# voichek/kmersGWAS

Hardware: AMD Instinct MI355X
Metric: k-mers x permutations scored/sec (higher is better)
Workload: dtype fp4 x fp6/fp4 block-scaled filter + f32/f64 exact re-score

## Files before the change

### kmersgwas_amd/csrc/aux_kernels.hip

```cpp
#include "score_common.h"
#include "synth.h"

namespace kgwas {

static hipError_t ensure_dyn_lds(const void* fn, size_t bytes) {
    if (bytes > 64 * 1024) return hipFuncSetAttribute(fn, hipFuncAttributeMaxDynamicSharedMemorySize, (int)bytes);
    return hipSuccess;
}

__global__ void __launch_bounds__(256) squeeze_kernel(const uint64_t* file_rows, uint64_t file_stride_w,
                                                      uint64_t n_rows, const uint32_t* colmap, uint32_t W_m,
                                                      uint32_t W_f, uint32_t* out) {
    extern __shared__ uint32_t lds_u32[];
    const uint32_t in_dw = 2u * W_f, in_ld = in_dw + 1u;
    const uint32_t out_dw = 2u * W_m, out_ld = out_dw + 1u;
    uint32_t* lin = lds_u32;
    uint32_t* lout = lds_u32 + 64u * in_ld;
    const uint64_t row0 = (uint64_t)blockIdx.x * 64u;
    const uint32_t* fr = reinterpret_cast<const uint32_t*>(file_rows);

    for (uint32_t e = threadIdx.x; e < 64u * in_dw; e += 256u) {
        const uint32_t rr = e / in_dw, dw = e - rr * in_dw;
        const uint64_t gr = row0 + rr;
        lin[rr * in_ld + dw] = (gr < n_rows) ? fr[gr * file_stride_w * 2u + 2u + dw] : 0u;
// ... 171 lines not shown
    }
    for (int o = 32; o > 0; o >>= 1) kcnt += __shfl_xor(kcnt, o);
    if (lane == 0 && kcnt) atomicAdd(&kept_s, kcnt);
    if (__ballot(bad != 0u) && lane == 0) atomicOr(&nan_s, 1u);
    __syncthreads();
    const uint32_t kept = kept_s;
    if (p == 0 && t == 0) info[0] = kept;
    if (t == 0 && nan_s) atomicOr(&info[1], 1u);
    const unsigned long long N = topn[p];
    if (kept < N || nan_s) return;
    if (t == 0) {
        prefix_s = 0;
        need_s = N;
    }
#pragma unroll 1
    for (int byte = 7; byte >= 0; byte--) {
        if (t < 256u) hist[t] = 0;
        __syncthreads();
        const unsigned long long prefix = prefix_s;
#pragma unroll
        for (int i = 0; i < DSEL_KPT; i++) {
            const bool act = ((valid >> i) & 1u) && (byte == 7 || (key[i] >> (8 * (byte + 1))) == prefix);
            const unsigned long long m = __ballot(act);
            if (!m) continue;
            const uint32_t bin = (uint32_t)(key[i] >> (8 * byte)) & 255u;
            const int first = __ffsll((long long)m) - 1;
            const uint32_t b0 = (uint32_t)__shfl((int)bin, first);
            if (__ballot(act && bin == b0) == m) {
                if ((int)lane == first) atomicAdd(&hist[b0], (uint32_t)__popcll(m));
            } else if (act) {
                atomicAdd(&hist[bin], 1u);
            }
        }
        __syncthreads();
        if (t < 64u) pick_bin_from_top(hist, prefix, &need_s, &prefix_s);
        __syncthreads();
    }
    if (t == 0) {
        const unsigned long long k = prefix_s;
        const unsigned long long b = (k >> 63) ? (k & 0x7FFFFFFFFFFFFFFFull) : ~k;
        const double v = __longlong_as_double((long long)b);
        thr_a[p] = v;
        thr_b[p] = v;
        thr_host_copy[p] = v;
    }
}

hipError_t launch_dense_select(const double* dense, const uint32_t* n1, uint32_t n_rows, uint32_t n_pheno, uint32_t S, uint32_t min_count,
                               const uint64_t* topn, double* thr_a, double* thr_b, double* thr_host_copy, uint32_t* info, hipStream_t st) {
    hipError_t e = hipMemsetAsync(info, 0, 2 * sizeof(uint32_t), st);
    if (e != hipSuccess) return e;
    static const bool reg_ok = !(exp_int("KGWAS_DSEL_REG", 1) == 0);
    if (reg_ok && n_rows <= (uint32_t)DSEL_KPT * 1024u)
        hipLaunchKernelGGL(dense_select_reg_kernel, dim3(n_pheno), dim3(1024), 0, st, dense, n1, n_rows, S, min_count, topn, thr_a, thr_b,
                           thr_host_copy, info);
    else
        hipLaunchKernelGGL(dense_select_kernel, dim3(n_pheno), dim3(256), 0, st, dense, n1, n_rows, S, min_count, topn, thr_a, thr_b,
                           thr_host_copy, info);
    return hipGetLastError();
}

__global__ void __launch_bounds__(256) records_to_host_kernel(const unsigned long long* __restrict__ sc, const unsigned long long* __restrict__ km,
                                                              const uint32_t* __restrict__ rw, uint32_t n, unsigned long long* __restrict__ h_sc,
                                                              unsigned long long* __restrict__ h_km, uint32_t* __restrict__ h_rw) {
    const uint32_t step = gridDim.x * blockDim.x;
    for (uint32_t i = blockIdx.x * blockDim.x + threadIdx.x; i < n; i += step) {
        h_sc[i] = sc[i];
        h_km[i] = km[i];
        h_rw[i] = rw[i];
    }
}

__global__ void __launch_bounds__(256) chunk_tail_kernel(const uint32_t* __restrict__ meta, uint32_t n_meta, uint32_t* __restrict__ h_meta,
                                                         const unsigned long long* __restrict__ tested, uint32_t n_tested,
                                                         unsigned long long* __restrict__ h_tested, const double* __restrict__ thr, uint32_t n_thr,
                                                         double* __restrict__ h_thr) {
    for (uint32_t i = threadIdx.x; i < n_meta; i += 256u) h_meta[i] = meta[i];
    for (uint32_t i = threadIdx.x; i < n_tested; i += 256u) h_tested[i] = tested[i];
    for (uint32_t i = threadIdx.x; i < n_thr; i += 256u) h_thr[i] = thr[i];
}

hipError_t launch_chunk_tail(const uint32_t* meta, uint32_t n_meta, uint32_t* h_meta, const unsigned long long* tested, uint32_t n_tested,
                             unsigned long long* h_tested, const double* thr, uint32_t n_thr, double* h_thr, hipStream_t st) {
    launch_last(chunk_tail_kernel, dim3(1), dim3(256), 0, st, meta, n_meta, h_meta, tested, n_tested, h_tested, thr, n_thr, h_thr);
    return hipGetLastError();
}

__global__ void __launch_bounds__(256) thr_tail_kernel(const uint32_t* hist, const uint32_t* hist_base, uint32_t bins, const uint64_t* topn,
                                                       const double* thr_host, double* thr, const uint32_t* __restrict__ meta, uint32_t n_meta,
                                                       uint32_t* __restrict__ h_meta, const unsigned long long* __restrict__ tested, uint32_t n_tested,
                                                       unsigned long long* __restrict__ h_tested, double* __restrict__ h_thr) {
    thr_update_block(hist, hist_base, bins, topn, thr_host, thr, blockIdx.x);
    if (h_thr && threadIdx.x == 0) h_thr[blockIdx.x] = thr[blockIdx.x];
    if (blockIdx.x == 0) {
        for (uint32_t i = threadIdx.x; i < n_meta; i += 256u) h_meta[i] = meta[i];
        for (uint32_t i = threadIdx.x; i < n_tested; i += 256u) h_tested[i] = tested[i];
    }
}

hipError_t launch_thr_tail(const uint32_t* hist, const uint32_t* hist_base, uint32_t bins, const uint64_t* topn, const double* thr_host, double* thr,
                           uint32_t n_pheno, const uint32_t* meta, uint32_t n_meta, uint32_t* h_meta, const unsigned long long* tested,
                           uint32_t n_tested, unsigned long long* h_tested, double* h_thr, hipStream_t st) {
    if (n_pheno == 0 || bins % 256u) return hipErrorInvalidValue;
    launch_last(thr_tail_kernel, dim3(n_pheno), dim3(256), 0, st, hist, hist_base, bins, topn, thr_host, thr, meta, n_meta, h_meta, tested,
                n_tested, h_tested, h_thr);
    return hipGetLastError();
}

hipError_t launch_records_to_host(const double* sc, const uint64_t* km, const uint32_t* rw, uint32_t n, double* h_sc, uint64_t* h_km, uint32_t* h_rw,
                                  hipStream_t st) {
    if (!n) return hipSuccess;
    static const uint32_t max_blocks = (uint64_t)exp_int("KGWAS_RECORD_BLOCKS", 64u);
    const uint32_t blocks = std::min<uint32_t>((n + 255u) / 256u, std::max(1u, max_blocks));
    hipLaunchKernelGGL(records_to_host_kernel, dim3(blocks), dim3(256), 0, st, reinterpret_cast<const unsigned long long*>(sc),
                       reinterpret_cast<const unsigned long long*>(km), rw, n, reinterpret_cast<unsigned long long*>(h_sc),
                       reinterpret_cast<unsigned long long*>(h_km), h_rw);
    return hipGetLastError();
}

hipError_t launch_thr_update(const uint32_t* hist, const uint32_t* hist_base, uint32_t bins, const uint64_t* topn,
                             const double* thr_host, double* thr, uint32_t n_pheno, hipStream_t st) {
    if (n_pheno == 0 || bins % 256u) return hipErrorInvalidValue;
    hipLaunchKernelGGL(thr_update_kernel, dim3(n_pheno), dim3(256), 0, st, hist, hist_base, bins, topn, thr_host, thr);
    return hipGetLastError();
}

hipError_t launch_squeeze(const uint64_t* file_rows, uint64_t file_stride_w, uint64_t n_rows, const uint32_t* colmap,
                          uint32_t W_m, uint32_t W_f, uint32_t* out, hipStream_t st) {
    if (n_rows == 0) return hipSuccess;
    const size_t lds = (size_t)64u * ((2u * W_f + 1u) + (2u * W_m + 1u)) * 4u;
    if (lds > 160u * 1024u) return hipErrorInvalidValue;
    hipError_t e = ensure_dyn_lds((const void*)squeeze_kernel, lds);
    if (e != hipSuccess) return e;
    hipLaunchKernelGGL(squeeze_kernel, dim3((uint32_t)((n_rows + 63) / 64)), dim3(256), lds, st, file_rows,
                       file_stride_w, n_rows, colmap, W_m, W_f, out);
    return hipGetLastError();
}

hipError_t launch_synth(uint64_t* rows, uint64_t first_row, uint64_t n_rows, uint64_t n_acc, uint64_t seed,
                        hipStream_t st) {
    if (n_rows == 0) return hipSuccess;
    const uint64_t total = n_rows * (1 + (n_acc + 63) / 64);
    uint64_t blocks = (total + 255) / 256;
    if (blocks > 256ull * 32ull) blocks = 256ull * 32ull;
    hipLaunchKernelGGL(synth_kernel, dim3((uint32_t)blocks), dim3(256), 0, st, rows, first_row, n_rows, n_acc, seed);
    return hipGetLastError();
}

__global__ void __launch_bounds__(256) copy_to_host_kernel(const uint4* __restrict__ src, uint4* __restrict__ dst, size_t n16, uint32_t tail_words) {
    const size_t step = (size_t)gridDim.x * blockDim.x;
    for (size_t i = (size_t)blockIdx.x * blockDim.x + threadIdx.x; i < n16; i += step) dst[i] = src[i];
    if (blockIdx.x == 0 && threadIdx.x < tail_words)
        reinterpret_cast<uint32_t*>(dst + n16)[threadIdx.x] = reinterpret_cast<const uint32_t*>(src + n16)[threadIdx.x];
}

hipError_t launch_copy_to_host(const void* src, void* dst_dev, size_t bytes, hipStream_t st) {
    if (!bytes) return hipSuccess;
    if (bytes % 4 || ((uintptr_t)src | (uintptr_t)dst_dev) % 16) return hipErrorInvalidValue;
    const size_t n16 = bytes / 16;
    const uint32_t blocks = (uint32_t)std::min<size_t>(std::max<size_t>((n16 + 255) / 256, 1), 256);
    hipLaunchKernelGGL(copy_to_host_kernel, dim3(blocks), dim3(256), 0, st, reinterpret_cast<const uint4*>(src), reinterpret_cast<uint4*>(dst_dev), n16,
                       (uint32_t)((bytes % 16) / 4));
    return hipGetLastError();
}

}
```

### kmersgwas_amd/csrc/kernels.h

```cpp
#pragma once
#include <hip/hip_runtime.h>
#include <stdint.h>

#include "env.h"
#include "launch.h"

namespace kgwas {

struct Cand {
    uint64_t kmer;
    double score;
    uint64_t row;
};

struct RowSrc {
    const uint32_t* base;
    uint64_t stride_dw;
    uint32_t off_dw;
    uint32_t avail_dw;
};

constexpr uint32_t TESTED_SHARDS = 256;

struct ScoreArgs {
    RowSrc src;
    const uint32_t* dmask;
    const uint64_t* file_rows;
    uint64_t file_stride_w;
    uint64_t n_rows;
    uint64_t first_row;
    uint32_t S;
    uint32_t W_m;
    uint32_t n_pheno;
    uint32_t min_count;
    const float* Yperm;
    const float* Ymfma;
    const float* sums;
    const double* thr;
    double* dense;
    uint32_t* n1_out;
    uint64_t* kmer_out;
    Cand* cand;
    uint32_t* cand_cnt;
    uint32_t cap;
    unsigned long long* tested;
    uint32_t* hist;
    const uint32_t* hist_base;
    uint32_t hist_bins;
    double* so_score;
    uint64_t* so_kmer;
    uint32_t* so_row;
};

constexpr int HIST_SHIFT = 44;
constexpr uint32_t HIST_BINS = 16384;

hipError_t launch_copy_to_host(const void* src, void* dst_dev, size_t bytes, hipStream_t st);
hipError_t launch_chunk_tail(const uint32_t* meta, uint32_t n_meta, uint32_t* h_meta, const unsigned long long* tested, uint32_t n_tested,
                             unsigned long long* h_tested, const double* thr, uint32_t n_thr, double* h_thr, hipStream_t st);
hipError_t launch_thr_tail(const uint32_t* hist, const uint32_t* hist_base, uint32_t bins, const uint64_t* topn, const double* thr_host, double* thr,
                           uint32_t n_pheno, const uint32_t* meta, uint32_t n_meta, uint32_t* h_meta, const unsigned long long* tested,
                           uint32_t n_tested, unsigned long long* h_tested, double* h_thr, hipStream_t st);
hipError_t launch_records_to_host(const double* sc, const uint64_t* km, const uint32_t* rw, uint32_t n, double* h_sc, uint64_t* h_km, uint32_t* h_rw,
                                  hipStream_t st);
hipError_t launch_thr_update(const uint32_t* hist, const uint32_t* hist_base, uint32_t bins, const uint64_t* topn,
                             const double* thr_host, double* thr, uint32_t n_pheno, hipStream_t st);

hipError_t launch_dense_select(const double* dense, const uint32_t* n1, uint32_t n_rows, uint32_t n_pheno, uint32_t S, uint32_t min_count,
                               const uint64_t* topn, double* thr_a, double* thr_b, double* thr_host_copy, uint32_t* info, hipStream_t st);

hipError_t launch_score_valu(const ScoreArgs& a, hipStream_t st);
hipError_t launch_score_mfma(const ScoreArgs& a, uint32_t rows_per_block, uint32_t nb_full, hipStream_t st);
size_t mfma_lds_bytes(uint32_t W_m);

struct CoarseCol {
    double kalpha;
    float iu;
    int32_t pheno;
};
struct CoarseArgs {
    RowSrc src;
    uint64_t n_rows;
    uint32_t S, n_pheno, min_count;
    uint32_t n_kgroups;
    uint32_t n_lgroups;
    uint32_t n_slices;
    const int8_t* Bq;
    const CoarseCol* cols;
    const double* thr;
    unsigned long long* bitmap;
    uint64_t words_per_col;
    unsigned long long* tested;
    float eg_max, rall_max, rmax_max;
};
size_t coarse_lds_bytes(uint32_t n_kgroups, uint32_t T);
hipError_t launch_coarse(const CoarseArgs& a, uint32_t T, uint32_t rows_per_block, hipStream_t st);
struct MxArgs {
    RowSrc src;
    uint64_t n_rows;
    uint32_t S, n_pheno, min_count;
    uint32_t n_full, n_quarter;
    uint32_t n_lgroups;
    uint32_t n_slices;
    uint32_t s1_fp6;
    uint32_t scale0;
    const uint8_t* Bq;
    const CoarseCol* cols;
    const double* thr;
    unsigned long long* bitmap;
    uint64_t words_per_col;
    unsigned long long* tested;
    float eg_max, rall_max, rmax_max;
};
size_t mx_lds_bytes(uint32_t n_steps, uint32_t CT, uint32_t n_slices, uint32_t s1_fp6);
uint32_t mx_step_bytes_rt(uint32_t n_slices, uint32_t s1_fp6);
uint32_t mx_row_tiles(uint32_t CT);
hipError_t launch_mx(const MxArgs& a, uint32_t CT, uint32_t rows_per_block, hipStream_t st);
bool mxs_supported(uint32_t CT, uint32_t NG, uint32_t n_slices, uint32_t s1_fp6);
size_t mxs_lds_bytes(uint32_t CT, uint32_t NG);
hipError_t launch_mxs(const MxArgs& a, uint32_t CT, uint32_t NG, uint32_t form, uint32_t rows_per_block, hipStream_t st);
hipError_t launch_rescore(const ScoreArgs& a, const uint32_t* keys, const uint32_t* surv_off, const uint32_t* surv_cnt,
                          uint32_t row_bits, uint32_t* tile_pref, uint32_t* tile_cnt, double* tmp_score,
                          const uint32_t* key_count, uint32_t* meta, hipStream_t st);
hipError_t launch_rescore_direct(const ScoreArgs& a, const uint32_t* keys, const uint32_t* surv_off, const uint32_t* surv_cnt,
                                 uint32_t row_bits, const uint32_t* tile_pref, hipStream_t st);
struct PrepThr {
    const uint32_t* hist;
    const uint32_t* hist_base;
    uint32_t bins;
    const uint64_t* topn;
    const double* thr_host;
    double* thr;
};
hipError_t launch_chunk_prep(uint32_t* cand_cnt, uint32_t n_pheno, unsigned long long* tested, uint32_t* key_count,
                             unsigned long long* bitmap, uint64_t bitmap_words, uint32_t* seg_cnt, uint32_t n_seg_words, const PrepThr& tu,
                             hipStream_t st);

constexpr int NARROW_SLICES = 3;
constexpr uint32_t NARROW_MAX_COLS = 4;
struct NarrowCol {
    double w[NARROW_SLICES];
    double t1;
    double eg, rall, rmax;
    double pad;
    float wf[3];
    float slackf;
};
struct NarrowArgs {
    RowSrc src;
    uint64_t n_rows;
    uint32_t S, n_pheno, min_count;
    uint32_t n_kgroups;
    const uint8_t* Bn;
    const NarrowCol* cols;
    const double* thr;
    unsigned long long* bitmap;
    uint64_t words_per_col;
    unsigned long long* tested;
    uint32_t row_off;
    uint32_t* seg_cnt;
    uint32_t n_segs;
    uint64_t slack_rows;
    uint32_t pack1;
};
hipError_t launch_bitmap_keys(unsigned long long* bitmap, uint64_t words_per_col, uint64_t n_rows, uint32_t n_pheno, uint32_t* blk_scratch,
                              unsigned long long* blk_mask, uint32_t* keys_sorted, uint32_t key_cap, uint32_t row_bits, uint32_t* surv_off,
                              uint32_t* surv_cnt, uint32_t* key_count, uint32_t* tile_pref, bool nibble_transposed, hipStream_t st);
hipError_t launch_narrow_keys(const unsigned long long* bitmap, uint64_t words_per_col, uint64_t n_rows, uint32_t n_pheno, const uint32_t* seg_cnt,
                              uint32_t* keys_sorted, uint32_t key_cap, uint32_t row_bits, uint32_t* surv_off, uint32_t* surv_cnt,
                              uint32_t* key_count, uint32_t* tile_pref, uint32_t* meta, const unsigned long long* tested_shards, hipStream_t st);
size_t narrow_lds_bytes(uint32_t n_kgroups);
hipError_t launch_narrow(const NarrowArgs& a, uint32_t rows_per_block, hipStream_t st);

hipError_t launch_pattern_hash(const RowSrc& src, const uint32_t* dmask, uint64_t n_rows, uint32_t S, uint32_t W_m,
                               uint32_t min_count, uint64_t* out, unsigned long long* out_count, hipStream_t st);
hipError_t count_distinct_u64(uint64_t* keys, uint64_t n, uint64_t* result, hipStream_t st);

hipError_t launch_bed_rowinfo(const uint32_t* sq, uint64_t n_rows, uint32_t W_m, uint32_t* n1_out, uint64_t* hash_out,
                              hipStream_t st);
hipError_t launch_bed_bytes(const uint32_t* sq, uint64_t n_rows, uint32_t W_m, uint32_t bytes_per_row, uint8_t* out,
                            hipStream_t st);

hipError_t launch_snp_planes(const uint8_t* bed, uint64_t n_snps, uint32_t bytes_per_snp, const uint32_t* byte_idx,
                             const uint32_t* shift, uint32_t S, uint32_t ndw, uint32_t* planes, hipStream_t st);
hipError_t launch_snp_score(const uint32_t* planes, uint64_t n_snps, uint32_t ndw, const float* Yperm, uint32_t L, uint32_t n_pheno,
                            double mac, double* scores, hipStream_t st);

uint32_t snpkin_vals_stride(uint32_t S);
size_t snpkin_vals_bytes(uint32_t S, uint32_t chunk_snps);
size_t snpkin_params_bytes(uint32_t chunk_snps);
hipError_t launch_snpkin_prep(const uint8_t* bed, uint32_t n_snps, uint32_t bytes_per_snp, uint32_t S, void* params, void* vals,
                              unsigned long long* n_used, hipStream_t st);
hipError_t launch_snpkin_accumulate(int rows_per_wave, const uint8_t* bed, uint32_t n_snps, uint32_t bytes_per_snp, uint32_t S,
                                    const void* params, const void* vals, const uint2* tiles, uint32_t n_tiles, double* sums,
                                    hipStream_t st);

constexpr uint32_t FK_SPLITTERS = 4096;
hipError_t launch_fk_match(const uint64_t* rows, uint64_t stride, uint32_t n_rows, const uint64_t* L, uint64_t n,
                           const uint64_t* spl, uint32_t ns, uint64_t B, uint64_t carry_key, bool has_prev, uint64_t* lb,
                           uint64_t* cnt, uint32_t* head, uint32_t* first_desc, hipStream_t st);
size_t fk_scan_temp_bytes(uint32_t max_rows);
hipError_t launch_fk_select(const uint64_t* rows, uint64_t stride, uint32_t n_rows, const uint64_t* cnt, const uint32_t* head,
                            uint32_t* run_start, uint64_t carry_run, const uint32_t* first_desc, uint8_t* emit, uint32_t* sel,
                            uint32_t* n_sel, uint64_t* info, void* temp, size_t temp_bytes, hipStream_t st);
hipError_t launch_fk_keys(const uint64_t* rows, uint64_t stride, uint32_t r0, uint32_t n_rows, uint64_t* keys, hipStream_t st);
hipError_t launch_fk_gather(const uint64_t* rows, uint64_t stride, const uint32_t* sel, uint32_t m, uint64_t* out, hipStream_t st);
hipError_t launch_fk_format(const uint64_t* rows, uint64_t stride, const uint32_t* sel, uint32_t m, uint32_t k, uint32_t S_f,
                            void* text, hipStream_t st);

hipError_t launch_bt_init(uint64_t* A, uint64_t n, uint64_t stride, uint64_t* rows, hipStream_t st);
hipError_t launch_bt_match(const uint64_t* A, uint64_t n, const uint64_t* spl, uint32_t ns, uint64_t B, const uint64_t* slice,
                           uint32_t m, uint64_t carry_key, bool has_prev, uint64_t* rows, uint64_t stride, uint64_t accession,
                           uint32_t* descends, hipStream_t st);

constexpr uint32_t LL_MAX_SLOTS = 4096;
constexpr uint32_t LL_NEED_NONE = 0xFFFFFFFFu;
struct ListArgs {
    const uint64_t* words;
    const uint32_t* seg_off;
    const uint32_t* seg_len;
    uint32_t n_seg;
    const uint64_t* sample;
    uint32_t m, nb, slots;
    uint64_t N, mac;
    const uint32_t* need;
    uint64_t* stage_pass;
    uint64_t* stage_np_key;
    uint64_t* stage_np_cnt;
    uint32_t* bk_base;
    uint32_t* bk_pass;
    uint32_t* bk_np;
    unsigned long long* stats;
    uint32_t* flags;
    unsigned long long* err_key;
};
hipError_t launch_ll_check(const uint64_t* words, uint32_t m, uint64_t carry_key, bool has_prev, uint32_t file, uint32_t* flags,
                           hipStream_t st);
size_t ll_temp_bytes(uint32_t max_sample, uint32_t max_buckets);
hipError_t launch_ll_splitters(const uint64_t* words, uint64_t total, uint32_t m, uint64_t* sample_raw, uint64_t* sample, void* temp,
                               size_t temp_bytes, hipStream_t st);
size_t ll_count_lds_bytes(uint32_t slots);
hipError_t launch_ll_count(const ListArgs& a, hipStream_t st);
hipError_t launch_ll_gather(const ListArgs& a, uint32_t* off_pass, uint32_t* off_np, uint64_t* out_pass, uint64_t* out_np_key,
                            uint64_t* out_np_cnt, void* temp, size_t temp_bytes, hipStream_t st);
hipError_t launch_ll_commit(unsigned long long* total, unsigned long long* piece, uint64_t n, hipStream_t st);

constexpr uint64_t CK_MAX_PASS_WORDS = 1ull << 30;
uint32_t ck_blocks(uint64_t max_words);
size_t ck_temp_bytes(uint64_t max_words, uint32_t max_sample, uint32_t kmer_len);
// ... 28 lines not shown
```

### kmersgwas_amd/csrc/launch.h

```cpp
#pragma once
#include <hip/hip_runtime.h>

#include <tuple>
#include <utility>

extern "C" hipError_t hipExtLaunchKernel(const void* function_address, dim3 numBlocks, dim3 dimBlocks, void** args, size_t sharedMemBytes,
                                         hipStream_t stream, hipEvent_t startEvent, hipEvent_t stopEvent, int flags);

namespace kgwas {

extern thread_local hipEvent_t g_bound_stop;

template <class... KA, size_t... I>
inline hipError_t launch_bound_impl(void (*kernel)(KA...), dim3 grid, dim3 block, size_t lds, hipStream_t st, hipEvent_t stop, std::tuple<KA...>& vals,
                                    std::index_sequence<I...>) {
    void* ptrs[] = {const_cast<void*>(static_cast<const void*>(&std::get<I>(vals)))..., nullptr};
    return hipExtLaunchKernel(reinterpret_cast<const void*>(kernel), grid, block, ptrs, lds, st, nullptr, stop, 0);
}

template <class... KA, class... A>
inline void launch_last(void (*kernel)(KA...), dim3 grid, dim3 block, size_t lds, hipStream_t st, A&&... args) {
    static_assert(sizeof...(KA) == sizeof...(A), "one argument per kernel parameter");
    const hipEvent_t stop = g_bound_stop;
    g_bound_stop = nullptr;
    if (!stop) {
        hipLaunchKernelGGL(kernel, grid, block, lds, st, static_cast<KA>(args)...);
        return;
    }
    std::tuple<KA...> vals(static_cast<KA>(args)...);
    (void)launch_bound_impl(kernel, grid, block, lds, st, stop, vals, std::index_sequence_for<KA...>{});
}

template <class F>
inline hipError_t bind_stop(hipEvent_t ev, hipStream_t st, F&& launcher) {
    g_bound_stop = ev;
    const hipError_t e = launcher();
    if (g_bound_stop) {
        g_bound_stop = nullptr;
        if (e == hipSuccess) return hipEventRecord(ev, st);
    }
    return e;
}

}
```

### kmersgwas_amd/csrc/scan_create.cpp

```cpp
#include "scan_internal.h"
#include <chrono>

struct CreateTrace {
    const bool on = opt_set("KGWAS_TRACE");
    const std::chrono::steady_clock::time_point t0 = std::chrono::steady_clock::now();
    void operator()(const char* what) const {
        if (on)
            fprintf(stderr, "[kgwas] scan_create +%.1f ms: %s\n", std::chrono::duration<double, std::milli>(std::chrono::steady_clock::now() - t0).count(), what);
    }
};

static std::unique_ptr<kgwas_scan> new_session(const kgwas_scan_params* p, ScanShape& sh) {
    if (p->struct_size != sizeof(kgwas_scan_params)) throw Error(KGWAS_ERR_ARG, "kgwas_scan_params: size mismatch");
    if (!p->col || !p->Y || !p->topn || p->n_acc == 0 || p->n_pheno == 0 || p->n_acc_file == 0)
        throw Error(KGWAS_ERR_ARG, "kgwas_scan_create: empty problem");
    if (p->n_acc > p->n_acc_file) throw Error(KGWAS_ERR_ARG, "more phenotyped accessions than table columns");
    if (p->n_acc_file >= (1ull << 31)) throw Error(KGWAS_ERR_ARG, "too many accessions");
    require_heap_emulation();
    check_device(p->device);
    KGWAS_HIP(hipSetDevice(p->device));
    std::unique_ptr<kgwas_scan> s(new kgwas_scan);
    s->device = p->device;
    s->S_f = p->n_acc_file;
    s->S = p->n_acc;
// ... 74 lines not shown
    KGWAS_HIP(hipStreamSynchronize(nullptr));
    s->d_topn.alloc(P);
    s->d_sel.alloc(P);
    s->h_sel.alloc(P);
    s->d_sel_info.alloc(2);
    s->h_sel_info.alloc(2);
    KGWAS_HIP(hipMemcpy(s->d_topn.p, s->topn.data(), P * 8, hipMemcpyHostToDevice));
    KGWAS_HIP(hipMemcpy(s->d_dmask.p, ex.dmask.data(), ex.dmask.size() * 4, hipMemcpyHostToDevice));
    KGWAS_HIP(hipMemcpy(s->d_colmap.p, ex.colmap.data(), ex.colmap.size() * 4, hipMemcpyHostToDevice));
    KGWAS_HIP(hipMemcpy(s->d_sums.p, ex.sums.data(), P * 4, hipMemcpyHostToDevice));
    if (s->kernel_used == KGWAS_KERNEL_MFMA) {
        s->d_Ymfma.alloc(ex.Ymfma.size());
        KGWAS_HIP(hipMemcpy(s->d_Ymfma.p, ex.Ymfma.data(), ex.Ymfma.size() * 4, hipMemcpyHostToDevice));
    }
    if (s->kernel_used != KGWAS_KERNEL_MFMA || s->coarse) {
        s->d_Yperm.alloc(ex.Yperm.size());
        KGWAS_HIP(hipMemcpy(s->d_Yperm.p, ex.Yperm.data(), ex.Yperm.size() * 4, hipMemcpyHostToDevice));
    }
    tcreate("small device buffers allocated and uploaded");
    return std::move(ex.sums);
}

static void upload_filters(kgwas_scan* s, const ScanPlan& pl, const ScanShape& sh, const std::vector<float>& sums) {
    if (pl.narrow) {
        const NarrowOperands op = narrow_operands(sh, pl, s->Y, sums, s->dbg_keep_resid ? s->dbg_resid[2].data() : nullptr);
        s->d_Bn.alloc(op.Bn.size());
        s->d_ncols.alloc(sh.P);
        KGWAS_HIP(hipMemcpy(s->d_Bn.p, op.Bn.data(), op.Bn.size(), hipMemcpyHostToDevice));
        KGWAS_HIP(hipMemcpy(s->d_ncols.p, op.ncols.data(), sh.P * sizeof(NarrowCol), hipMemcpyHostToDevice));
    }
    for (int mi = 0; mi < 2; mi++) {
        const FilterSet& fs = pl.set[mi];
        if (!fs.slices) continue;
        kgwas_scan::CoarseMode& M = s->cmode[mi];
        M.mx = fs.mx;
        M.mx_full = fs.n_full;
        M.mx_quarter = fs.n_quarter;
        M.mx_s1_fp6 = fs.s1_fp6;
        if (fs.mx) M.mx_scale0 = 0x01010101u * (uint32_t)(0x7F + (fs.slices == 1 ? 0 : 5));
        M.slices = fs.slices;
        M.n_parts = (uint32_t)fs.parts.size();
        M.tile_slices = fs.tile_slices;
        M.tile_slices_eq = fs.tile_slices_eq;
        uint32_t groups_all = 0;
        for (size_t pi = 0; pi < fs.parts.size(); pi++) {
            const FilterPart& fp = fs.parts[pi];
            kgwas_scan::CoarsePart& Pt = M.part[pi];
            Pt.T = fp.T;
            Pt.n_lgroups = (uint32_t)(fp.groups / fp.ng);
            Pt.stream = fp.stream;
            Pt.ng = fp.ng;
            if (fp.stream) s->st.coarse_mx_stream = fp.stream;
            groups_all += Pt.n_lgroups;
            double* resid = s->dbg_keep_resid ? s->dbg_resid[mi].data() : nullptr;
            const PartOperands op = fs.mx ? block_scaled_operands(sh, fs, fp, s->Y, sums, resid)
                                          : int8_operands(sh, pl.n_kgroups, fs, fp, s->Y, sums, resid);
            M.eg_max = std::max(M.eg_max, op.eg_max);
            M.rall_max = std::max(M.rall_max, op.rall_max);
            M.rmax_max = std::max(M.rmax_max, op.rmax_max);
            Pt.d_Bq.alloc(op.Bq.size());
            Pt.d_cols.alloc(op.cols.size());
            KGWAS_HIP(hipMemcpy(Pt.d_Bq.p, op.Bq.data(), op.Bq.size(), hipMemcpyHostToDevice));
            KGWAS_HIP(hipMemcpy(Pt.d_cols.p, op.cols.data(), op.cols.size() * sizeof(CoarseCol), hipMemcpyHostToDevice));
        }
        s->st.coarse_mode_tiles[mi] = M.part[0].T;
        s->st.coarse_mode_lgroups[mi] = groups_all;
        s->st.coarse_mode_tile_slices[mi] = M.tile_slices;
        if (fs.mx) {
            if (pl.use_mx) s->st.coarse_mx = 1;
            s->st.coarse_mx_s1_fp6 = fs.s1_fp6;
            s->st.coarse_mx_steps = fs.n_steps;
        }
        M.ready = true;
    }
}

static void alloc_filter_buffers(kgwas_scan* s) {
    const uint64_t P = s->n_pheno;
    s->key_slots = (uint32_t)std::min<uint64_t>((uint64_t)s->cap * P, 0x7FFFFFFFull);
    s->d_surv_sorted.alloc(s->key_slots);
    s->bitmap_words = (s->chunk_max + 63) / 64;
    s->d_bitmap.alloc(P * s->bitmap_words);
    s->d_bm_blocks.alloc(P * ((s->bitmap_words + 1023) / 1024 + 1) + 4);
    if (!s->narrow) s->d_bm_mask.alloc(P * ((s->bitmap_words + 1023) / 1024) * 4 + 4);
    s->bitmap_clean = false;
    s->d_surv_cnt.alloc(P);
    s->d_surv_off.alloc(P);
    s->d_key_count.alloc(2);
    s->d_tile_pref.alloc(P + 1);
    s->d_tile_cnt.alloc((size_t)s->key_slots / 256 + P + 2);
    s->d_tmp_score.alloc(s->key_slots);
    int least = 0, greatest = 0;
    KGWAS_HIP(hipDeviceGetStreamPriorityRange(&least, &greatest));
    const bool hi = !(exp_int("KGWAS_COPY_PRIO", 1) == 0);
    KGWAS_HIP(hipStreamCreateWithPriority(&s->copy_stream, hipStreamNonBlocking, hi ? greatest : least));
    s->row_key_bits = 1;
    while (s->row_key_bits < 32 && (1ull << s->row_key_bits) < s->chunk_max) s->row_key_bits++;
}

static void alloc_slots(kgwas_scan* s, const CreateTrace& tcreate) {
    const uint64_t P = s->n_pheno;
    if (!s->direct) s->d_sq.alloc(s->chunk_max * 2 * s->W_m);
    if (s->coarse) {
        const uint64_t slot_bytes = (uint64_t)s->key_slots * 20;
        s->n_slots = (int)std::min<uint64_t>(MAX_SLOTS, std::max<uint64_t>(4, (4ull << 30) / std::max<uint64_t>(slot_bytes, 1)));
        s->ring_size = (size_t)std::max<uint64_t>(std::min<uint64_t>(1ull << 30, std::min<uint64_t>((uint64_t)s->n_slots * slot_bytes, std::max<uint64_t>(64ull << 20, 8 * slot_bytes))),
                                                  2 * slot_bytes + 4096);
        if (opt_str("KGWAS_RING_BYTES"))
            s->ring_size = (size_t)std::max<uint64_t>(strtoull(opt_str("KGWAS_RING_BYTES"), nullptr, 10), slot_bytes + 4096);
        tcreate("device buffers and slots allocated");
        s->ring.alloc(s->ring_size);
        s->ring_dev = s->ring.dev();
        tcreate("pinned record ring allocated");
    } else {
        const uint64_t slot_bytes = (uint64_t)s->cap * P * sizeof(Cand);
        s->n_slots = (int)std::min<uint64_t>(16, std::max<uint64_t>(4, (1ull << 30) / std::max<uint64_t>(slot_bytes, 1)));
    }
    for (int si = 0; si < s->n_slots + (s->coarse ? 1 : 0); si++) {
        const bool is_redo = si == s->n_slots;
        Slot& sl = is_redo ? s->redo : s->slot[si];
        if (s->coarse && !is_redo) {
            sl.d_so_score.alloc(s->key_slots);
            sl.d_so_kmer.alloc(s->key_slots);
            sl.d_so_row.alloc(s->key_slots);
            sl.d_meta.alloc(2 * P + 4);
            sl.h_meta.alloc(2 * P + 4);
            sl.h_thr.alloc(P);
            memset(sl.h_thr.p, 0, P * sizeof(double));
            memset(sl.h_meta.p, 0, (2 * P + 4) * sizeof(uint32_t));
            sl.h_meta_dev = sl.h_meta.dev();
            sl.h_thr_dev = sl.h_thr.dev();
            KGWAS_HIP(hipEventCreateWithFlags(&sl.ev_counts, hipEventBlockingSync));
        } else {
            sl.cand.alloc((uint64_t)s->cap * P);
            sl.d_cand = sl.cand.dev();
        }
        sl.d_cnt.alloc(P);
        sl.h_cnt.alloc(P);
        sl.d_tested.alloc(TESTED_SHARDS);
        sl.h_tested.alloc(TESTED_SHARDS);
        sl.h_tested_dev = sl.h_tested.dev();
        KGWAS_HIP(hipEventCreate(&sl.ev_sq0));
        KGWAS_HIP(hipEventCreate(&sl.ev_k0));
        KGWAS_HIP(hipEventCreate(&sl.ev_k1));
        KGWAS_HIP(hipEventCreateWithFlags(&sl.ev_done, hipEventBlockingSync));
        KGWAS_HIP(hipEventCreate(&sl.ev_mid));
    }
    s->d_dense.alloc(P * s->dense_rows);
    s->h_dense.alloc(P * s->dense_rows);
    s->d_n1.alloc(s->dense_rows);
    s->h_n1.alloc(s->dense_rows);
    s->d_kmer.alloc(s->dense_rows);
    s->h_kmer.alloc(s->dense_rows);
    s->h_dense_dev = s->h_dense.dev();
    s->h_n1_dev = s->h_n1.dev();
    s->h_kmer_dev = s->h_kmer.dev();
    s->d_tested_dense.alloc(TESTED_SHARDS);
}

static void make_heaps_and_select(kgwas_scan* s) {
    make_heaps(s);
    const char* fr = opt_str("KGWAS_FULL_REPLAY");
    s->lazy_enabled = s->coarse && !s->record_history && !(fr && atoi(fr) != 0);
    s->lazy_log_mode = s->lazy_enabled && s->history_ring != 0;
    lazy_reset(s);
    s->hist.resize(s->n_pheno);
    s->keys.resize(s->n_pheno);
// ... 104 lines not shown
```

### kmersgwas_amd/csrc/scan_gpu.cpp

```cpp
#include "scan_internal.h"

namespace kgwas {


void fill_args(kgwas_scan* s, ScoreArgs& a, const uint64_t* d_rows, uint64_t n_rows, uint64_t first_row,
               bool squeezed) {
    memset(&a, 0, sizeof(a));
    if (squeezed) {
        a.src.base = s->d_sq.p;
        a.src.stride_dw = 2 * s->W_m;
        a.src.off_dw = 0;
        a.src.avail_dw = (uint32_t)(2 * s->W_m);
    } else {
        a.src.base = reinterpret_cast<const uint32_t*>(d_rows);
        a.src.stride_dw = 2 * (1 + s->W_f);
        a.src.off_dw = 2;
        a.src.avail_dw = (uint32_t)(2 * s->W_f);
    }
    a.dmask = s->d_dmask.p;
    a.file_rows = d_rows;
    a.file_stride_w = 1 + s->W_f;
    a.n_rows = n_rows;
    a.first_row = first_row;
    a.S = (uint32_t)s->S;
// ... 228 lines not shown
    if (!s->cmode[1].ready) return 0;
    const double cand_row = (double)s->sum_topn / (double)std::max<uint64_t>(s->rows_submitted, 1);
    auto eq = [](const kgwas_scan::CoarseMode& M) { return M.tile_slices_eq > 0 ? M.tile_slices_eq : (double)M.tile_slices; };
    const double tiles0 = eq(s->cmode[0]), tiles1 = eq(s->cmode[1]);
    return cand_row * std::max(0.0, s->infl_obs[0] - s->infl_obs[1]) < s->mode_k * (tiles1 - tiles0) ? 0 : 1;
}

static void dbg_log_thresholds(kgwas_scan* s, const double* d_thr, uint64_t n_rows, uint64_t first_row, uint32_t set) {
    kgwas_scan::DbgChunk ch;
    ch.first_row = first_row;
    ch.n_rows = n_rows;
    ch.set = set;
    ch.thr.resize(s->n_pheno);
    KGWAS_HIP(hipMemcpyAsync(ch.thr.data(), d_thr, s->n_pheno * sizeof(double), hipMemcpyDeviceToHost, s->stream));
    KGWAS_HIP(hipStreamSynchronize(s->stream));
    s->dbg_chunks.push_back(std::move(ch));
}

static void dbg_log_survivors(kgwas_scan* s) {
    kgwas_scan::DbgChunk& ch = s->dbg_chunks.back();
    const uint64_t P = s->n_pheno;
    std::vector<uint32_t> off(P), cnt(P);
    uint32_t total = 0;
    KGWAS_HIP(hipMemcpyAsync(off.data(), s->d_surv_off.p, P * sizeof(uint32_t), hipMemcpyDeviceToHost, s->stream));
    KGWAS_HIP(hipMemcpyAsync(cnt.data(), s->d_surv_cnt.p, P * sizeof(uint32_t), hipMemcpyDeviceToHost, s->stream));
    KGWAS_HIP(hipMemcpyAsync(&total, s->d_key_count.p, sizeof(uint32_t), hipMemcpyDeviceToHost, s->stream));
    KGWAS_HIP(hipStreamSynchronize(s->stream));
    ch.overflow = total > s->key_slots ? 1u : 0u;
    if (ch.overflow || !total) return;
    std::vector<uint32_t> keys(total);
    KGWAS_HIP(hipMemcpyAsync(keys.data(), s->d_surv_sorted.p, (size_t)total * sizeof(uint32_t), hipMemcpyDeviceToHost, s->stream));
    KGWAS_HIP(hipStreamSynchronize(s->stream));
    const uint32_t row_mask = s->row_key_bits >= 32 ? 0xFFFFFFFFu : (1u << s->row_key_bits) - 1u;
    for (uint64_t p = 0; p < P; p++) {
        if ((uint64_t)off[p] + cnt[p] > total) throw Error(KGWAS_ERR_STATE, "survivor log: a column's key range leaves the list");
        for (uint32_t i = 0; i < cnt[p]; i++) {
            const uint32_t key = keys[off[p] + i];
            ch.pairs.push_back(s->row_key_bits >= 32 ? 0u : key >> s->row_key_bits);
            ch.pairs.push_back(key & row_mask);
        }
    }
}

void submit_sparse(kgwas_scan* s, Slot& sl, const uint64_t* d_rows, uint64_t n_rows, uint64_t first_row,
                   bool count_hist) {
    ScoreArgs a;
    fill_args(s, a, d_rows, n_rows, first_row, !s->direct);
    a.cand = sl.d_cand;
    a.cand_cnt = sl.d_cnt.p;
    a.cap = s->cap;
    a.tested = sl.d_tested.p;
    if (count_hist) {
        if (!s->hist_ready) start_histograms(s);
        a.hist = s->d_hist.p;
        a.hist_base = s->d_hist_base.p;
        a.hist_bins = HIST_BINS;
    } else {
        for (uint64_t j = 0; j < s->n_pheno; j++) s->h_thr_redo.p[j] = s->lazy[j].on ? s->lazy[j].bound() : s->heaps[j].lowest();
        KGWAS_HIP(hipMemcpyAsync(s->d_thr_redo.p, s->h_thr_redo.p, s->n_pheno * sizeof(double), hipMemcpyHostToDevice,
                                 s->stream));
        a.thr = s->d_thr_redo.p;
    }
    const bool use_coarse = s->coarse && count_hist;
    if (!s->direct) {
        KGWAS_HIP(hipEventRecord(sl.ev_sq0, s->stream));
        maybe_squeeze(s, d_rows, n_rows);
        KGWAS_HIP(hipEventRecord(sl.ev_k0, s->stream));
    }
    {
        const uint64_t n_words = (n_rows + 63) / 64;
        const uint32_t n_segs = (uint32_t)((n_words + 1023) / 1024);
        PrepThr tu;
        memset(&tu, 0, sizeof(tu));
        if (use_coarse && s->narrow && s->hist_ready) {
            tu.hist = s->d_hist.p;
            tu.hist_base = s->d_hist_base.p;
            tu.bins = HIST_BINS;
            tu.topn = s->d_topn.p;
            tu.thr_host = s->d_thr_host.p;
            tu.thr = s->d_thr.p;
        }
        const bool zero_bitmap = use_coarse && (s->narrow || !s->bitmap_clean);
        const uint64_t zero_words = !zero_bitmap ? 0 : (s->narrow ? s->n_pheno * n_words : s->d_bitmap.n);
        const auto prep = [&] {
            return launch_chunk_prep(sl.d_cnt.p, (uint32_t)s->n_pheno, sl.d_tested.p, use_coarse ? s->d_key_count.p : nullptr,
                                     zero_bitmap ? s->d_bitmap.p : nullptr, zero_words,
                                     (use_coarse && s->narrow) ? s->d_bm_blocks.p : nullptr, (use_coarse && s->narrow) ? (uint32_t)s->n_pheno * n_segs : 0u,
                                     tu, s->stream);
        };
        if (s->direct) KGWAS_HIP(bind_stop(sl.ev_k0, s->stream, prep));
        else KGWAS_HIP(prep());
    }
    sl.used_coarse = use_coarse;
    if (use_coarse) {
        CoarseArgs c;
        memset(&c, 0, sizeof(c));
        c.src = a.src;
        c.n_rows = n_rows;
        c.S = a.S;
        c.n_pheno = a.n_pheno;
        c.min_count = a.min_count;
        c.n_kgroups = s->n_kgroups;
        const int cm = s->narrow ? 0 : pick_coarse_mode(s);
        if (s->dbg_keep_surv) dbg_log_thresholds(s, a.thr, n_rows, first_row, s->narrow ? 2u : (uint32_t)cm);
        const kgwas_scan::CoarseMode& M = s->cmode[cm];
        sl.coarse_mode = cm;
        sl.cand_est = (double)s->sum_topn * (double)n_rows / (double)std::max<uint64_t>(s->rows_submitted, 1);
        c.n_slices = M.slices;
        c.eg_max = M.eg_max;
        c.rall_max = M.rall_max;
        c.rmax_max = M.rmax_max;
        c.thr = a.thr;
        c.tested = a.tested;
        static const uint32_t rpb_env = (uint64_t)exp_int("KGWAS_COARSE_RPB", 0u);
        const uint64_t n_words = (n_rows + 63) / 64;
        if (s->narrow) {
            NarrowArgs na;
            memset(&na, 0, sizeof(na));
            na.src = a.src;
            na.n_rows = n_rows;
            na.S = a.S;
            na.n_pheno = a.n_pheno;
            na.min_count = a.min_count;
            na.n_kgroups = s->n_kgroups;
            na.Bn = s->d_Bn.p;
            na.cols = s->d_ncols.p;
            na.thr = a.thr;
            na.bitmap = s->d_bitmap.p;
            na.words_per_col = n_words;
            na.tested = a.tested;
            na.pack1 = s->narrow_pack1 ? 1u : 0u;
            na.seg_cnt = s->d_bm_blocks.p;
            na.n_segs = (uint32_t)((n_words + 1023) / 1024);
            na.slack_rows = s->direct ? s->slack_rows : 0;
            KGWAS_HIP(bind_stop(sl.ev_mid, s->stream, [&] { return launch_narrow(na, rpb_env ? rpb_env : (n_rows >= (1u << 24) ? 1280u : n_rows >= (1u << 18) ? 768u : 256u), s->stream); }));
        } else {
            s->bitmap_clean = false;
            c.bitmap = s->d_bitmap.p;
            c.words_per_col = n_words;
            for (uint32_t pi = 0; pi < M.n_parts; pi++) {
                const kgwas_scan::CoarsePart& Pt = M.part[pi];
                c.n_lgroups = Pt.n_lgroups;
                c.Bq = Pt.d_Bq.p;
                c.cols = Pt.d_cols.p;
                c.tested = pi == 0 ? a.tested : nullptr;
                const bool last_part = pi + 1u == M.n_parts;
                const uint32_t rpb = rpb_env ? rpb_env : (n_rows >= (1u << 22) ? 4096u : n_rows >= (1u << 20) ? 2048u : 512u);
                if (M.mx) {
                    MxArgs x;
                    memset(&x, 0, sizeof(x));
                    x.src = c.src;
                    x.n_rows = n_rows;
                    x.S = c.S;
                    x.n_pheno = c.n_pheno;
                    x.min_count = c.min_count;
                    x.n_full = M.mx_full;
                    x.n_quarter = M.mx_quarter;
                    x.n_lgroups = Pt.n_lgroups;
                    x.n_slices = M.slices;
                    x.s1_fp6 = M.mx_s1_fp6;
                    x.scale0 = M.mx_scale0;
                    x.Bq = reinterpret_cast<const uint8_t*>(Pt.d_Bq.p);
                    x.cols = Pt.d_cols.p;
                    x.thr = c.thr;
                    x.bitmap = c.bitmap;
                    x.words_per_col = c.words_per_col;
                    x.tested = c.tested;
                    x.eg_max = c.eg_max;
                    x.rall_max = c.rall_max;
                    x.rmax_max = c.rmax_max;
                    const auto filt = [&] {
                        return Pt.stream ? launch_mxs(x, Pt.T, Pt.ng, Pt.stream - 1u, rpb, s->stream) : launch_mx(x, Pt.T, rpb, s->stream);
                    };
                    if (last_part) KGWAS_HIP(bind_stop(sl.ev_mid, s->stream, filt));
                    else KGWAS_HIP(filt());
                } else {
                    const auto filt = [&] { return launch_coarse(c, Pt.T, rpb, s->stream); };
                    if (last_part) KGWAS_HIP(bind_stop(sl.ev_mid, s->stream, filt));
                    else KGWAS_HIP(filt());
                }
            }
            if (!M.n_parts) KGWAS_HIP(hipEventRecord(sl.ev_mid, s->stream));
        }
        a.tested = nullptr;
        a.so_score = sl.d_so_score.p;
        a.so_kmer = sl.d_so_kmer.p;
        a.so_row = sl.d_so_row.p;
        if (s->narrow) {
            KGWAS_HIP(launch_narrow_keys(s->d_bitmap.p, n_words, n_rows, (uint32_t)s->n_pheno, s->d_bm_blocks.p, s->d_surv_sorted.p, s->key_slots,
                                         s->row_key_bits, s->d_surv_off.p, s->d_surv_cnt.p, s->d_key_count.p, s->d_tile_pref.p, sl.d_meta.p, sl.d_tested.p, s->stream));
            if (s->dbg_keep_surv) dbg_log_survivors(s);
            KGWAS_HIP(bind_stop(sl.ev_k1, s->stream, [&] { return launch_rescore_direct(a, s->d_surv_sorted.p, s->d_surv_off.p, s->d_surv_cnt.p, s->row_key_bits, s->d_tile_pref.p, s->stream); }));
        } else {
        KGWAS_HIP(launch_bitmap_keys(s->d_bitmap.p, n_words, n_rows, (uint32_t)s->n_pheno, s->d_bm_blocks.p, s->d_bm_mask.p, s->d_surv_sorted.p, s->key_slots,
                                     s->row_key_bits, s->d_surv_off.p, s->d_surv_cnt.p, s->d_key_count.p, s->d_tile_pref.p, !s->narrow, s->stream));
        s->bitmap_clean = true;
        if (s->dbg_keep_surv) dbg_log_survivors(s);
        a.so_score = sl.d_so_score.p;
        a.so_kmer = sl.d_so_kmer.p;
        a.so_row = sl.d_so_row.p;
        KGWAS_HIP(bind_stop(sl.ev_k1, s->stream, [&] {
            return launch_rescore(a, s->d_surv_sorted.p, s->d_surv_off.p, s->d_surv_cnt.p, s->row_key_bits, s->d_tile_pref.p,
                                  s->d_tile_cnt.p, s->d_tmp_score.p, s->d_key_count.p, sl.d_meta.p, s->stream);
        }));
        }
        s->st.score_launches++;
    } else {
        if (s->direct) KGWAS_HIP(hipEventRecord(sl.ev_k0, s->stream));
        launch_score(s, a);
        KGWAS_HIP(hipEventRecord(sl.ev_k1, s->stream));
    }
    const bool fused_tail = use_coarse && s->narrow;
    static const bool tail_kernel = !(exp_int("KGWAS_TAIL_KERNEL", 1) == 0);
    const bool one_launch = use_coarse && tail_kernel && sl.h_meta_dev;
    const bool thr_and_tail = one_launch && s->hist_ready && !fused_tail;
    if (s->hist_ready && !fused_tail && !thr_and_tail)
        KGWAS_HIP(launch_thr_update(s->d_hist.p, s->d_hist_base.p, HIST_BINS, s->d_topn.p, s->d_thr_host.p, s->d_thr.p,
                                    (uint32_t)s->n_pheno, s->stream));
    if (!fused_tail && !one_launch)
        KGWAS_HIP(hipMemcpyAsync(sl.h_tested.p, sl.d_tested.p, TESTED_SHARDS * sizeof(unsigned long long), hipMemcpyDeviceToHost,
                                 s->stream));
    sl.tested_in_meta = fused_tail;
    if (thr_and_tail) {
        const bool thr_too = s->lazy_any.load(std::memory_order_relaxed);
        KGWAS_HIP(bind_stop(sl.ev_counts, s->stream, [&] {
            return launch_thr_tail(s->d_hist.p, s->d_hist_base.p, HIST_BINS, s->d_topn.p, s->d_thr_host.p, s->d_thr.p, (uint32_t)s->n_pheno, sl.d_meta.p,
                                   (uint32_t)(2 * s->n_pheno + 4), sl.h_meta_dev, sl.d_tested.p, (uint32_t)TESTED_SHARDS, sl.h_tested_dev,
                                   thr_too ? sl.h_thr_dev : nullptr, s->stream);
        }));
    } else if (one_launch) {
        const bool thr_too = s->lazy_any.load(std::memory_order_relaxed);
        KGWAS_HIP(bind_stop(sl.ev_counts, s->stream, [&] {
            return launch_chunk_tail(sl.d_meta.p, (uint32_t)(2 * s->n_pheno + 4), sl.h_meta_dev, sl.d_tested.p, fused_tail ? 0u : (uint32_t)TESTED_SHARDS,
                                     sl.h_tested_dev, s->d_thr.p, thr_too ? (uint32_t)s->n_pheno : 0u, sl.h_thr_dev, s->stream);
        }));
    } else if (use_coarse) {
        KGWAS_HIP(hipMemcpyAsync(sl.h_meta.p, sl.d_meta.p, (2 * s->n_pheno + 4) * sizeof(uint32_t), hipMemcpyDeviceToHost, s->stream));
        if (s->lazy_any.load(std::memory_order_relaxed))
            KGWAS_HIP(hipMemcpyAsync(sl.h_thr.p, s->d_thr.p, s->n_pheno * sizeof(double), hipMemcpyDeviceToHost, s->stream));
        KGWAS_HIP(hipEventRecord(sl.ev_counts, s->stream));
    } else {
        KGWAS_HIP(hipMemcpyAsync(sl.h_cnt.p, sl.d_cnt.p, s->n_pheno * sizeof(uint32_t), hipMemcpyDeviceToHost, s->stream));
        KGWAS_HIP(hipEventRecord(sl.ev_done, s->stream));
    }
    sl.rows = d_rows;
    sl.first_row = first_row;
    sl.n_rows = n_rows;
    sl.busy = true;
    s->st.chunks++;
}

bool chunk_complete(kgwas_scan* s, Slot& sl) {
    sl.busy = false;
    float ms = 0;
    KGWAS_HIP(hipEventElapsedTime(&ms, sl.ev_k0, sl.ev_k1));
    s->st.score_kernel_ms += ms;
    if (sl.used_coarse) {
        float mc = 0;
        KGWAS_HIP(hipEventElapsedTime(&mc, sl.ev_k0, sl.ev_mid));
        s->st.coarse_kernel_ms += mc;
        s->st.coarse_launches++;
        s->st.coarse_mode_ms[sl.coarse_mode] += mc;
        s->st.coarse_mode_launches[sl.coarse_mode]++;
        s->st.coarse_mode_rows[sl.coarse_mode] += sl.n_rows;
    }
    if (!s->direct) {
        float mq = 0;
        KGWAS_HIP(hipEventElapsedTime(&mq, sl.ev_sq0, sl.ev_k0));
        s->st.squeeze_kernel_ms += mq;
    }
    bool over = false;
    if (sl.used_coarse) {
        over = sl.h_meta.p[2 * s->n_pheno + 1] > s->key_slots;
    } else {
        for (uint64_t j = 0; j < s->n_pheno && !over; j++) over = sl.h_cnt.p[j] > s->cap;
    }
    if (s->trace) {
        uint64_t tot = 0, mx = 0;
        for (uint64_t q = 0; q < s->n_pheno; q++) {
            const uint64_t v = sl.used_coarse ? sl.h_meta.p[q] : sl.h_cnt.p[q];
            tot += v;
            mx = std::max<uint64_t>(mx, v);
        }
        fprintf(stderr, "[kgwas] chunk rows=%llu first=%llu kernel=%.3fms records %llu (max per column %llu)%s%s\n",
                (unsigned long long)sl.n_rows, (unsigned long long)sl.first_row, ms, (unsigned long long)tot,
                (unsigned long long)mx, sl.used_coarse ? (" survivors " + std::to_string(sl.h_meta.p[2 * s->n_pheno + 1])).c_str() : "",
                over ? " OVERFLOW" : "");
    }
    if (over) return false;
    if (sl.tested_in_meta)
        s->st.rows_tested += (uint64_t)sl.h_meta.p[2 * s->n_pheno + 2] | ((uint64_t)sl.h_meta.p[2 * s->n_pheno + 3] << 32);
    else
        for (uint32_t i = 0; i < TESTED_SHARDS; i++) s->st.rows_tested += sl.h_tested.p[i];
    return true;
}

uint64_t next_sparse_chunk(const kgwas_scan* s) {
    const double m = (double)std::max<uint64_t>(s->rows_submitted, 1);
    static const double fill_env = exp_num("KGWAS_FILL", 0.0);
    const double fill = fill_env > 0.0 ? fill_env : (s->narrow ? (s->lazy_any.load(std::memory_order_relaxed) ? 0.15 : 0.05) : 0.4);
    double c;
    if (s->coarse) {
        const double infl = s->narrow ? 1.0 : std::max(1.0, s->infl_obs[pick_coarse_mode(s)]);
        c = fill * m * (double)s->key_slots / (infl * (double)std::max<uint64_t>(s->sum_topn, 1));
    } else {
        c = m * (double)s->cap / (3.0 * (double)std::max<uint64_t>(s->max_topn, 1));
    }
    uint64_t ci = (uint64_t)std::min<double>(c, (double)s->chunk_max);
    ci = std::max<uint64_t>(ci, std::min<uint64_t>(s->dense_rows, s->chunk_max));
    ci = std::min<uint64_t>(ci, s->chunk_max);
    return (ci + 127) / 128 * 128;
}

void wait_event(kgwas_scan* s, hipEvent_t ev) {
    auto w0 = std::chrono::steady_clock::now();
    bool done = false;
    static const int polls = (int)exp_int("KGWAS_WAIT_POLLS", 400);
    for (int i = 0; i < polls && !done; i++) {
        const hipError_t q = hipEventQuery(ev);
        if (q == hipSuccess) done = true;
        else if (q != hipErrorNotReady) KGWAS_HIP(q);
        else
            for (int k = 0; k < 20; k++) __builtin_ia32_pause();
    }
    if (!done) KGWAS_HIP(hipEventSynchronize(ev));
    s->st.gpu_wait_ms += std::chrono::duration<double, std::milli>(std::chrono::steady_clock::now() - w0).count();
}

void ring_to_recycling(kgwas_scan* s, uint64_t replayed) {
    for (uint64_t j = 0; j < s->n_pheno; j++)
        if (s->lazy[j].on) s->lazy[j].detach();
    s->ring_keep.store(false, std::memory_order_release);
    s->ring_tail = replayed ? s->slot[(size_t)((replayed - 1) % (uint64_t)s->n_slots)].ring_end : s->ring_feed_start;
    s->ring_freed = replayed;
    if (s->trace) fprintf(stderr, "[kgwas t=%.3f] record ring full: logs detached, ring recycles from %zu (head %zu of %zu)\n", s->t_ms(), s->ring_tail, s->ring_head, s->ring_size);
}

bool fetch_records(kgwas_scan* s, Slot& sl, uint64_t seq) {
// ... 60 lines not shown
```

### kmersgwas_amd/csrc/scan_host.cpp

```cpp
#include "scan_internal.h"
#include <sched.h>

namespace kgwas {

thread_local hipEvent_t g_bound_stop = nullptr;


std::vector<int> parse_cpulist(const char* path) {
    std::vector<int> out;
    FILE* f = fopen(path, "r");
    if (!f) return out;
    char buf[4096];
    if (fgets(buf, sizeof(buf), f)) {
        for (char* tok = strtok(buf, ",\n"); tok; tok = strtok(nullptr, ",\n")) {
            int a = 0, b = 0;
            const int k = sscanf(tok, "%d-%d", &a, &b);
            if (k == 1) b = a;
            if (k >= 1)
                for (int c = a; c <= b; c++) out.push_back(c);
        }
    }
    fclose(f);
    return out;
}

std::vector<std::vector<int>> pick_replay_cpus(unsigned n, int device) {
    std::vector<std::vector<int>> none;
    int mode = 1;
    const char* e = opt_str("KGWAS_PIN_THREADS");
    if (e) mode = atoi(e);
    if (mode == 0) return none;
    cpu_set_t allowed;
    CPU_ZERO(&allowed);
    if (sched_getaffinity(0, sizeof(allowed), &allowed) != 0) return none;
    if (!e && usable_cpus() < (unsigned)CPU_COUNT(&allowed)) {
        if (opt_str("KGWAS_TRACE")) fprintf(stderr, "[kgwas] replay workers not pinned: a quota of %u CPUs on a set of %d\n", usable_cpus(), CPU_COUNT(&allowed));
        return none;
    }
    int node = -1;
    char bus[64] = {0};
    if (hipDeviceGetPCIBusId(bus, (int)sizeof(bus), device) == hipSuccess) {
        for (char* c = bus; *c; c++) *c = (char)tolower(*c);
        char path[256];
        snprintf(path, sizeof(path), "/sys/bus/pci/devices/%s/numa_node", bus);
        if (FILE* f = fopen(path, "r")) {
            if (fscanf(f, "%d", &node) != 1) node = -1;
            fclose(f);
        }
    }
    std::vector<int> cand;
    if (node >= 0) {
        char path[256];
        snprintf(path, sizeof(path), "/sys/devices/system/node/node%d/cpulist", node);
        cand = parse_cpulist(path);
    }
    if (cand.empty())
        for (int c = 0; c < CPU_SETSIZE; c++)
            if (CPU_ISSET(c, &allowed)) cand.push_back(c);
    std::vector<int> cores;
    for (int c : cand) {
        if (c < 0 || c >= CPU_SETSIZE || !CPU_ISSET(c, &allowed)) continue;
        char path[256];
        snprintf(path, sizeof(path), "/sys/devices/system/cpu/cpu%d/topology/thread_siblings_list", c);
        const std::vector<int> sib = parse_cpulist(path);
        if (sib.empty() || sib[0] == c) cores.push_back(c);
    }
    size_t n_gpus = 1, ordinal = 0;
    if (node >= 0 && bus[0]) {
        std::vector<std::string> gpus;
        if (DIR* d = opendir("/sys/bus/pci/devices")) {
            while (struct dirent* de = readdir(d)) {
                if (de->d_name[0] == '.') continue;
                char path[512];
                unsigned vendor = 0, cls = 0;
                int nn = -2;
                snprintf(path, sizeof(path), "/sys/bus/pci/devices/%s/vendor", de->d_name);
                if (FILE* f = fopen(path, "r")) {
                    if (fscanf(f, "%x", &vendor) != 1) vendor = 0;
                    fclose(f);
                }
                if (vendor != 0x1002) continue;
                snprintf(path, sizeof(path), "/sys/bus/pci/devices/%s/class", de->d_name);
                if (FILE* f = fopen(path, "r")) {
                    if (fscanf(f, "%x", &cls) != 1) cls = 0;
                    fclose(f);
                }
                if ((cls >> 8) != 0x0380 && (cls >> 8) != 0x1200 && (cls >> 8) != 0x0300) continue;
                snprintf(path, sizeof(path), "/sys/bus/pci/devices/%s/numa_node", de->d_name);
// ... 133 lines not shown
```

### kmersgwas_amd/csrc/scan_internal.h

```cpp
#pragma once
#include <algorithm>
#include <atomic>
#include <chrono>
#include <cmath>
#include <condition_variable>
#include <deque>
#include <limits>
#include <cstdio>
#include <cstdlib>
#include <cstring>
#include <functional>
#include <memory>
#include <mutex>
#include <string>
#include <thread>
#include <vector>

#include <dirent.h>
#include <immintrin.h>
#include <pthread.h>
#include <sched.h>
#include <sys/mman.h>

#include "common.h"
// ... 240 lines not shown
        }
        return *this;
    }
    ~LazyCol() { release_log(); }
    void release_log() {
        free(l_sc);
        free(l_km);
        free(l_rw);
        l_sc = nullptr, l_km = nullptr, l_rw = nullptr;
        l_n = l_cap = 0;
        segs.clear();
        scan_seg = 0, scan_off = 0, unscanned = 0;
    }
    void reserve_log(size_t need);
    void reset(bool enable, uint64_t topn_);
    void compact();
    void prune(uint64_t thr_bits);
    bool select(std::vector<uint64_t>& kmer, std::vector<double>& score, std::vector<uint64_t>& row);
    bool ties_now();
    void take_chunk(const double* sc, const uint64_t* km, const uint32_t* rw, uint32_t n, uint64_t row0, uint64_t thr_bits, bool by_ref);
    inline bool full() const { return n_logged >= topn; }
    inline double bound() const {
        double v = 0.0;
        if (have_bound) memcpy(&v, &bound_bits, 8);
        return v;
    }
    inline void add(uint64_t kmer, double score, uint64_t row) {
        uint64_t b;
        memcpy(&b, &score, 8);
        if (b == NEG_INF) return;
        if (l_n == l_cap) reserve_log(l_n + 1);
        l_sc[l_n] = score;
        l_km[l_n] = kmer;
        l_rw[l_n] = row;
        l_n++;
        owned_appended(1);
        n_logged++;
        if (++unscanned >= 4 * topn + 1024) scan_pending();
    }
    void scan_pending();
    size_t scan_seg = 0;
    uint32_t scan_off = 0;
    uint64_t unscanned = 0;
};

inline size_t ring_size(size_t forced, uint64_t topn) {
    if (forced > 1) return forced;
    const double r = 16.0 * std::sqrt(2.0 * (double)topn);
    return (size_t)std::min<double>(std::max<double>(r, 256.0), 1048576.0);
}

constexpr int MAX_SLOTS = 48;

struct ReplayAcc {
    uint64_t pushes = 0, cands = 0, busy_ns = 0, units = 0;
};

struct Slot {
    PinBuf<Cand> cand;
    Cand* d_cand = nullptr;
    DevBuf<uint32_t> d_cnt;
    PinBuf<uint32_t> h_cnt;
    bool copies_ordered = false;
    double* so_score = nullptr;
    uint64_t* so_kmer = nullptr;
    uint32_t* so_row = nullptr;
    size_t ring_end = 0;
    DevBuf<double> d_so_score;
    DevBuf<uint64_t> d_so_kmer;
    DevBuf<uint32_t> d_so_row;
    DevBuf<uint32_t> d_meta;
    PinBuf<uint32_t> h_meta;
    uint32_t* h_meta_dev = nullptr;
    double* h_thr_dev = nullptr;
    unsigned long long* h_tested_dev = nullptr;
    PinBuf<double> h_thr;
    bool tie_check = false;
    bool tested_in_meta = false;
    hipEvent_t ev_counts = nullptr;
    DevBuf<unsigned long long> d_tested;
    PinBuf<unsigned long long> h_tested;
    hipEvent_t ev_sq0 = nullptr, ev_k0 = nullptr, ev_k1 = nullptr, ev_done = nullptr, ev_mid = nullptr;
    bool used_coarse = false;
    int coarse_mode = 0;
    double cand_est = 0;
    const uint64_t* rows = nullptr;
    uint64_t first_row = 0, n_rows = 0;
    bool squeezed = false, busy = false;
};

}

using namespace kgwas;

struct kgwas_scan {
    int device = 0;
    uint64_t S_f = 0, S = 0, W_f = 0, W_m = 0, L = 0, n_pheno = 0, min_count = 0;
    std::vector<uint64_t> col, topn;
    std::vector<float> Y;
    bool direct = false;
    uint32_t kernel_used = 0;
    bool record_history = false;
    size_t history_ring = 0;
    uint64_t chunk_max = 0, dense_rows = 0, dense_chunk = 0;
    uint32_t cap = 0;
    uint64_t max_topn = 0;
    uint32_t nb_full = 0;

    hipStream_t stream = nullptr, copy_stream = nullptr;
    hipEvent_t ev_user = nullptr, ev_ds = nullptr, ev_d0 = nullptr, ev_d1 = nullptr;
    hipEvent_t ev_dcopy = nullptr;
    bool dense_copy_pending = false;
    DevBuf<uint32_t> d_dmask, d_colmap, d_sq;
    DevBuf<float> d_Yperm, d_Ymfma, d_sums;
    DevBuf<double> d_thr;
    PinBuf<double> h_thr;
    uint32_t thr_flip = 0;
    DevBuf<uint32_t> d_hist, d_hist_base;
    PinBuf<uint32_t> h_hist_base;
    DevBuf<uint64_t> d_topn;
    DevBuf<double> d_thr_host, d_thr_redo;
    PinBuf<double> h_thr_redo;
    bool hist_ready = false;
    uint64_t rows_submitted = 0;
    bool coarse = false;
    uint32_t n_kgroups = 0;
    struct CoarsePart {
        uint32_t T = 0, n_lgroups = 0;
        uint32_t stream = 0;
        uint32_t ng = 1;
        DevBuf<int8_t> d_Bq;
        DevBuf<CoarseCol> d_cols;
    };
    struct CoarseMode {
        bool ready = false;
        bool mx = false;
        uint32_t mx_full = 0, mx_quarter = 0, mx_s1_fp6 = 0, mx_scale0 = 0;
        uint32_t slices = 0, n_parts = 0;
        uint32_t tile_slices = 0;
        double tile_slices_eq = 0;
        float eg_max = 0, rall_max = 0, rmax_max = 0;
        CoarsePart part[2];
    } cmode[2];
    DevBuf<double> d_sel;
    PinBuf<double> h_sel;
    DevBuf<uint32_t> d_sel_info;
    PinBuf<uint32_t> h_sel_info;
    bool sel_valid = false;
    double infl_obs[2] = {4.0, 1.1};
    double mode_k = 0;
    std::chrono::steady_clock::time_point t_feed0;
    double t_ms() const { return std::chrono::duration<double, std::milli>(std::chrono::steady_clock::now() - t_feed0).count(); }
    uint64_t sum_topn = 0;
    bool narrow = false;
    bool narrow_pack1 = false;
    DevBuf<uint8_t> d_Bn;
    DevBuf<NarrowCol> d_ncols;
    DevBuf<unsigned long long> d_bitmap;
    uint64_t bitmap_words = 0;
    DevBuf<uint32_t> d_bm_blocks;
    DevBuf<unsigned long long> d_bm_mask;
    bool bitmap_clean = false;
    uint64_t slack_rows = 0;
    DevBuf<uint32_t> d_surv_sorted, d_surv_cnt, d_surv_off, d_key_count;
    DevBuf<uint32_t> d_tile_pref, d_tile_cnt;
    DevBuf<double> d_tmp_score;
    uint32_t key_slots = 0;
    uint32_t row_key_bits = 32;
    bool count_patterns = false;
    DevBuf<uint64_t> d_pat;
    DevBuf<unsigned long long> d_pat_cnt;
    uint64_t pat_upper = 0;
    Slot slot[MAX_SLOTS];
    PinBuf<uint8_t> ring;
    uint8_t* ring_dev = nullptr;
    bool streamed_feed = false;
    double* h_dense_dev = nullptr;
    uint32_t* h_n1_dev = nullptr;
    uint64_t* h_kmer_dev = nullptr;
    size_t ring_size = 0, ring_head = 0, ring_tail = 0;
    std::atomic<bool> ring_keep{false};
    size_t ring_feed_start = 0;
    uint64_t ring_freed = 0;
    Slot redo;
    int n_slots = MAX_SLOTS;
    DevBuf<double> d_dense;
    DevBuf<uint32_t> d_n1;
    DevBuf<uint64_t> d_kmer;
    PinBuf<double> h_dense;
    PinBuf<uint32_t> h_n1;
    PinBuf<uint64_t> h_kmer;
    DevBuf<unsigned long long> d_tested_dense;
    DevBuf<uint64_t> d_stage;
    Ingest ingest;

    struct HugeArena {
        void* p = nullptr;
        size_t bytes = 0;
        ~HugeArena() { free(p); }
    } heap_arena;
    std::unique_ptr<std::pmr::monotonic_buffer_resource> heap_mr;
    std::vector<BestHeap> heaps;
    bool lazy_enabled = false;
    bool dbg_keep_resid = false;
    std::vector<double> dbg_resid[3];
    struct DbgChunk {
        uint64_t first_row = 0, n_rows = 0;
        uint32_t set = 0, overflow = 0;
        std::vector<double> thr;
        std::vector<uint32_t> pairs;
    };
    bool dbg_keep_surv = false;
    std::vector<DbgChunk> dbg_chunks;
    bool lazy_log_mode = false;
    std::vector<LazyCol> lazy;
    std::atomic<bool> lazy_any{false};
    std::atomic<uint64_t> n_selected{0}, n_unselected{0}, lazy_pushes{0};
    uint64_t tie_check_rows = 0;
    std::vector<History> hist;
    std::vector<uint64_t> exp_kmer, exp_row;
    std::vector<double> exp_score;
    std::vector<std::vector<uint64_t>> keys;
    bool trace = false;
    std::vector<double> col_ms;
    bool all_full = false;
    uint64_t rows_done = 0;
    std::unique_ptr<Pool> pool;
    struct alignas(64) GroupState {
        std::atomic<uint64_t> done{0};
        std::atomic<uint32_t> busy{0};
    };
    std::atomic<size_t> n_groups{1};
    size_t n_groups0 = 1;
    std::vector<std::vector<uint32_t>> grp_cols;
    std::vector<std::vector<uint32_t>> grp_cols0;
    std::vector<int> grp_home;
    std::unique_ptr<std::atomic<int>[]> grp_owner;
    std::unique_ptr<GroupState[]> gstate;
    std::unique_ptr<std::atomic<uint32_t>[]> slot_left;
    std::atomic<int> rp_hungry{0};
    std::atomic<bool> rp_all_published{false};
    std::atomic<uint64_t> rp_final_pub{0};
    std::atomic<bool> final_feed{false};
    bool final_feed_next = false;
// ... 140 lines not shown
```

### kmersgwas_amd/csrc/score_coarse.hip

```cpp
#include <algorithm>
#include <type_traits>

#include "score_common.h"

#ifndef KGWAS_COARSE_PHASES
#define KGWAS_COARSE_PHASES 1
#endif
#ifndef KGWAS_COARSE_ABLATE
#define KGWAS_COARSE_ABLATE 0
#endif
#ifndef KGWAS_RESCORE_HALVES
#define KGWAS_RESCORE_HALVES 0
#endif
#ifndef KGWAS_RESCORE_FMA
#define KGWAS_RESCORE_FMA 1
#endif

namespace kgwas {

typedef int i32x4 __attribute__((ext_vector_type(4)));

#ifdef KGWAS_COARSE_TIMELINE
__device__ unsigned long long g_coarse_tl[2 * 16 * 64];
#define TL_STAMP(idx)                                                                       \
// ... 156 lines not shown
                }
                __builtin_amdgcn_wave_barrier();
                const uint32_t n1r = (uint32_t)n1s[lane];
                const uint64_t left = a.n_rows - rbase;
                const uint32_t rows_here = left < 64u ? (uint32_t)left : 64u;
                const bool mac_any = a.S >= 2u * a.min_count;
                const uint32_t span = a.S - 2u * a.min_count;
                const bool ok = mac_any & ((m >> 2) * 16u + kg * 4u + (m & 3u) < rows_here) & ((n1r - a.min_count) <= span);
                if (lg == 0) tested_local += ok ? 1u : 0u;
                const float f = (float)n1r;
                const float sq = __builtin_amdgcn_sqrtf(f * (Nf - f)) * 0.99999905f;
                float2 tm;
                tm.x = ok ? sq : __builtin_huge_valf();
                tm.y = (a.eg_max + fminf(a.rall_max, f * a.rmax_max)) * 1.000001f;
                if (KGWAS_COARSE_ABLATE & 16) tm = make_float2(1000.0f + m, 1.0f);
                trm[lane] = tm;
                __builtin_amdgcn_wave_barrier();
#pragma unroll
                for (int i = 0; i < RT * 4; i += 2) {
                    const float4 v = *reinterpret_cast<const float4*>(trm + kg * 16u + i);
                    sqd[i] = v.x;
                    er[i] = v.y;
                    sqd[i + 1] = v.z;
                    er[i + 1] = v.w;
                }
                __builtin_amdgcn_wave_barrier();
            }
            TL_STAMP(51);
            auto pair_margin = [&](int i, int g, float al) {
                int dc = acc[i >> 2][NS * g][i & 3];
                if (NS == 2) dc = __mul24(dc, 254) + acc[i >> 2][NS * g + NS - 1][i & 3];
                return fmaf(-al, sqd[i], fabsf((float)dc));
            };
            float alc[PG];
#pragma unroll
            for (int g = 0; g < PG; g++) alc[g] = colc[g * 16 + m];
            uint64_t hit[RT * 4];
            if (!(KGWAS_COARSE_ABLATE & 1)) {
                float mx[RT * 4];
#pragma unroll
                for (int i = 0; i < RT * 4; i++) mx[i] = -__builtin_huge_valf();
#pragma unroll
                for (int g = 0; g < PG; g++)
#pragma unroll
                    for (int i = 0; i < RT * 4; i++) mx[i] = fmaxf(mx[i], pair_margin(i, g, alc[g]));
#pragma unroll
                for (int i = 0; i < RT * 4; i++) hit[i] = __ballot(mx[i] + er[i] >= 0.0f);
            } else {
#pragma unroll
                for (int i = 0; i < RT * 4; i++) hit[i] = 0;
                int x = 0;
#pragma unroll
                for (int i = 0; i < RT * 4; i++)
#pragma unroll
                    for (int t = 0; t < T; t++) x ^= acc[i >> 2][t][i & 3];
                hit[0] = __ballot(x == 0x7fffffff);
            }
            TL_STAMP(52);
            uint64_t hit_any = 0;
#pragma unroll
            for (int i = 0; i < RT * 4; i++) hit_any |= hit[i];
            if ((KGWAS_COARSE_ABLATE & 32) && hit_any) {
                if (lane == 0) atomicAdd(&a.tested[0], 0ull);
                hit_any = 0;
            }
            uint32_t mb[PG];
#pragma unroll
            for (int g = 0; g < PG; g++) mb[g] = 0;
            if (hit_any) {
#pragma unroll
                for (int i = 0; i < RT * 4; i++) {
                    if (hit[i]) {
#pragma unroll
                        for (int g = 0; g < PG; g++) {
                            float al = alc[g];
                            asm volatile("" : "+v"(al));
                            mb[g] |= (pair_margin(i, g, al) + er[i] >= 0.0f) ? (1u << i) : 0u;
                        }
                    }
                }
            }
            if (hit_any) {
                unsigned short* bm16 = reinterpret_cast<unsigned short*>(a.bitmap) + (rbase >> 6) * 4u + kg;
#pragma unroll
                for (int g = 0; g < PG; g++)
                    if (mb[g]) bm16[(uint64_t)colp[g * 16 + m] * a.words_per_col * 4u] = (unsigned short)mb[g];
            }
            TL_STAMP(53);
        }
    }
    if (a.tested) {
        uint32_t v = tested_local;
#pragma unroll
        for (int d = 1; d < 64; d <<= 1) v += __shfl_xor(v, d);
        if (lane == 0u && v) atomicAdd(&a.tested[blockIdx.x % TESTED_SHARDS], (unsigned long long)v);
    }
}

__device__ __forceinline__ uint32_t tile_column(const uint32_t* tile_pref, uint32_t n_pheno, uint32_t t) {
    uint32_t lo = 0, hi = n_pheno;
    while (hi - lo > 1u) {
        const uint32_t mid = (lo + hi) >> 1;
        if (tile_pref[mid] <= t) lo = mid; else hi = mid;
    }
    return lo;
}

typedef __attribute__((address_space(4))) const float* kconst_f32p;
template <bool YLDS, int NS = 1>
__device__ __forceinline__ void rescore_block(const uint32_t (&w)[NS][4], const float* yb, float (&acc)[NS][4]) {
    kconst_f32p yc = (kconst_f32p)yb;
    const float4* yl = reinterpret_cast<const float4*>(yb);
    (void)yc;
    (void)yl;
#if KGWAS_RESCORE_FMA
    typedef float f32x2 __attribute__((ext_vector_type(2)));
#if KGWAS_RESCORE_HALVES
    if (NS == 1 && YLDS) {
        const float2* yh = reinterpret_cast<const float2*>(yb);
#pragma unroll
        for (int half = 0; half < 2; half++) {
            uint32_t eh[2][8];
#pragma unroll
            for (int l = 0; l < 2; l++)
#pragma unroll
                for (int j = 0; j < 8; j++) eh[l][j] = (w[0][2 * half + l] >> j) & 0x01010101u;
            f32x2 ah = {acc[0][2 * half], acc[0][2 * half + 1]};
#pragma unroll
            for (int s = 0; s < 32; s++) {
                const int b = 31 - s, j = b & 7, k = b >> 3;
                const float2 yv = yh[2 * s + half];
                const f32x2 yy = {yv.x, yv.y};
                auto byte_f32 = [&](uint32_t x) {
                    float f;
                    if (k == 0) asm("v_cvt_f32_ubyte0 %0, %1" : "=v"(f) : "v"(x));
                    if (k == 1) asm("v_cvt_f32_ubyte1 %0, %1" : "=v"(f) : "v"(x));
                    if (k == 2) asm("v_cvt_f32_ubyte2 %0, %1" : "=v"(f) : "v"(x));
                    if (k == 3) asm("v_cvt_f32_ubyte3 %0, %1" : "=v"(f) : "v"(x));
                    return f;
                };
                const f32x2 g = {byte_f32(eh[0][j]), byte_f32(eh[1][j])};
                ah = __builtin_elementwise_fma(g, yy, ah);
            }
            acc[0][2 * half] = ah.x;
            acc[0][2 * half + 1] = ah.y;
        }
        return;
    }
#endif
    uint32_t e[NS][4][8];
#pragma unroll
    for (int v = 0; v < NS; v++)
#pragma unroll
        for (int l = 0; l < 4; l++)
#pragma unroll
            for (int j = 0; j < 8; j++) e[v][l][j] = (w[v][l] >> j) & 0x01010101u;
    f32x2 a01[NS], a23[NS];
#pragma unroll
    for (int v = 0; v < NS; v++) {
        a01[v] = (f32x2){acc[v][0], acc[v][1]};
        a23[v] = (f32x2){acc[v][2], acc[v][3]};
    }
#pragma unroll
    for (int s = 0; s < 32; s++) {
        const int b = 31 - s, j = b & 7, k = b >> 3;
        f32x2 y01, y23;
        if (YLDS) {
            const float4 yv = yl[s];
            y01 = (f32x2){yv.x, yv.y};
// ... 98 lines not shown
        }
        if (YLDS) {
            const float4* ysrc = reinterpret_cast<const float4*>(a.Yperm + (size_t)p * L);
            for (uint32_t k = threadIdx.x; k < L / 4u; k += 256u) ytile[k] = ysrc[k];
            __syncthreads();
        }
        uint2 nx[NS][2];
        auto fetch = [&](uint32_t b) {
#pragma unroll
            for (int v = 0; v < NS; v++)
#pragma unroll
                for (int h = 0; h < 2; h++) {
                    nx[v][h] = make_uint2(0u, 0u);
                    if (4u * b + 2u * h + 1u < a.src.avail_dw) nx[v][h] = *reinterpret_cast<const uint2*>(rp[v] + 4u * b + 2u * h);
                }
        };
        if (nblk) fetch(0);
        for (uint32_t b = 0; b < nblk; b++) {
            uint32_t w[NS][4];
#pragma unroll
            for (int v = 0; v < NS; v++) {
#pragma unroll
                for (int h = 0; h < 2; h++) {
                    w[v][2 * h] = nx[v][h].x & a.dmask[4 * b + 2 * h];
                    w[v][2 * h + 1] = nx[v][h].y & a.dmask[4 * b + 2 * h + 1];
                }
                n1[v] += __popc(w[v][0]) + __popc(w[v][1]) + __popc(w[v][2]) + __popc(w[v][3]);
            }
            if (b + 1u < nblk) fetch(b + 1u);
            if (YLDS)
                rescore_block<true, NS>(w, reinterpret_cast<const float*>(ytile) + 128u * b, acc);
            else
                rescore_block<false, NS>(w, a.Yperm + (size_t)p * L + 128u * b, acc);
        }
        if (DIRECT) {
#pragma unroll
            for (int v = 0; v < NS; v++) {
                const float yf = ((acc[v][0] + acc[v][1]) + acc[v][2]) + acc[v][3];
                double q, d, sc, out = -__builtin_huge_val();
                score_terms(a, yf, n1[v], a.sums[p], q, d);
                if (valid[v] && mac_pass(a, n1[v]) && candidate_score(a, p, q, d, a.thr[p], sc)) out = sc;
                if (valid[v]) {
                    a.so_score[gi[v]] = out;
                    a.so_kmer[gi[v]] = a.file_rows[r[v] * a.file_stride_w];
                    a.so_row[gi[v]] = (uint32_t)r[v];
                }
            }
            if (YLDS) __syncthreads();
        } else {
#pragma unroll
            for (int v = 0; v < NS; v++)
                if ((uint32_t)v < nv) rescore_finish(a, p, valid[v], gi[v], acc[v], n1[v], tmp_score, tile_cnt, t0 + (uint32_t)v, wcnt);
        }
    };
    for (uint32_t t = (uint32_t)NS * blockIdx.x;; t += (uint32_t)NS * gridDim.x) {
        if (ticket) {
            if (threadIdx.x == 0) next_tile = atomicAdd(ticket, (uint32_t)NS);
            __syncthreads();
            t = next_tile;
            __syncthreads();
        }
        if (t >= n_tiles) break;
        const uint32_t p = __builtin_amdgcn_readfirstlane(tile_column(tile_pref, a.n_pheno, t));
        if (NS == 1) {
            run(t, p, 1u);
        } else {
            const bool two = t + 1u < n_tiles && t + 1u < tile_pref[p + 1u];
            run(t, p, two ? 2u : 1u);
            if (!two && t + 1u < n_tiles) run(t + 1u, __builtin_amdgcn_readfirstlane(tile_column(tile_pref, a.n_pheno, t + 1u)), 1u);
        }
    }
}

__device__ __forceinline__ uint32_t block_sum_256(uint32_t v, uint32_t* red) {
    const uint32_t lane = threadIdx.x & 63u, wave = threadIdx.x >> 6;
#pragma unroll
    for (int d = 1; d < 64; d <<= 1) v += __shfl_xor(v, d);
    __syncthreads();
    if (lane == 0u) red[wave] = v;
    __syncthreads();
    return red[0] + red[1] + red[2] + red[3];
}

__global__ void __launch_bounds__(256) compact_kernel(ScoreArgs a, const uint32_t* keys, const uint32_t* surv_off,
                                                      const uint32_t* surv_cnt, const uint32_t* tile_pref, uint32_t row_mask,
                                                      const double* tmp_score, const uint32_t* tile_cnt, const uint32_t* key_count,
                                                      uint32_t* meta) {
    __shared__ uint32_t wcnt[4];
    __shared__ uint32_t red[4];
    __shared__ uint32_t cpre[257];
    const uint32_t n_tiles = tile_pref[a.n_pheno];
    const uint32_t lane = threadIdx.x & 63u, wave = threadIdx.x >> 6;
    const uint32_t n_workers = gridDim.x - 1u;
    if (blockIdx.x == n_workers) {
        const uint32_t per = (n_tiles + 255u) / 256u;
        const uint32_t lo = threadIdx.x * per < n_tiles ? threadIdx.x * per : n_tiles;
        const uint32_t hi = lo + per < n_tiles ? lo + per : n_tiles;
        uint32_t sm = 0;
        for (uint32_t i = lo; i < hi; i++) sm += tile_cnt[i];
        cpre[threadIdx.x + 1u] = sm;
        if (threadIdx.x == 0u) cpre[0] = 0u;
        __syncthreads();
        for (uint32_t d = 1; d < 256u; d <<= 1) {
            const uint32_t x = threadIdx.x + 1u > d ? cpre[threadIdx.x + 1u - d] : 0u;
            __syncthreads();
            cpre[threadIdx.x + 1u] += x;
            __syncthreads();
        }
        auto prefix_at = [&](uint32_t x) {
            if (x >= n_tiles) return cpre[256];
            const uint32_t seg = per ? x / per : 0u;
            uint32_t v = cpre[seg];
            for (uint32_t i = seg * per; i < x; i++) v += tile_cnt[i];
            return v;
        };
        for (uint32_t p = threadIdx.x; p < a.n_pheno; p += 256u) {
            const uint32_t o0 = prefix_at(tile_pref[p]), o1 = prefix_at(tile_pref[p + 1u]);
            meta[p] = o1 - o0;
            meta[a.n_pheno + p] = o0;
        }
        if (threadIdx.x == 0u) {
            meta[2u * a.n_pheno] = cpre[256];
            meta[2u * a.n_pheno + 1u] = *key_count;
        }
        return;
    }
    uint32_t base = 0, done = 0;
    for (uint32_t t = blockIdx.x; t < n_tiles; t += n_workers) {
        uint32_t part = 0;
        for (uint32_t i = done + threadIdx.x; i < t; i += 256u) part += tile_cnt[i];
        base += block_sum_256(part, red);
        done = t;
        if (tile_cnt[t] == 0u) continue;
        const uint32_t p = __builtin_amdgcn_readfirstlane(tile_column(tile_pref, a.n_pheno, t));
        const uint32_t i = (t - tile_pref[p]) * 256u + threadIdx.x;
        const bool valid = i < surv_cnt[p];
        const uint32_t gi = surv_off[p] + (valid ? i : 0u);
        const double sc = valid ? tmp_score[gi] : -__builtin_huge_val();
        const bool is_cand = sc != -__builtin_huge_val();
        const unsigned long long bal = __ballot(is_cand);
        if (lane == 0) wcnt[wave] = __popcll(bal);
        __syncthreads();
        uint32_t before = __popcll(bal & ((1ull << lane) - 1ull));
        for (uint32_t w = 0; w < wave; w++) before += wcnt[w];
        if (is_cand) {
            const uint32_t r = keys[gi] & row_mask;
            const uint32_t o = base + before;
            a.so_score[o] = sc;
            a.so_kmer[o] = a.file_rows[(uint64_t)r * a.file_stride_w];
            a.so_row[o] = r;
        }
        __syncthreads();
    }
}

__global__ void __launch_bounds__(256) chunk_prep_kernel(uint32_t* cand_cnt, uint32_t n_pheno, unsigned long long* tested, uint32_t* key_count,
                                                         unsigned long long* bitmap, uint64_t bitmap_words, uint32_t* seg_cnt, uint32_t n_seg_words,
                                                         PrepThr tu) {
    const uint32_t i = blockIdx.x * blockDim.x + threadIdx.x;
    if (i < n_pheno) cand_cnt[i] = 0u;
    if (i < TESTED_SHARDS) tested[i] = 0ull;
    if (i == 0 && key_count) key_count[0] = 0u, key_count[1] = 0u;
    if (i < n_seg_words) seg_cnt[i] = 0u;
    ulonglong2* b2 = reinterpret_cast<ulonglong2*>(bitmap);
    const uint64_t pairs = bitmap_words / 2u;
    for (uint64_t k = i; k < pairs; k += (uint64_t)gridDim.x * blockDim.x) b2[k] = make_ulonglong2(0ull, 0ull);
    if (i == 0 && (bitmap_words & 1u)) bitmap[bitmap_words - 1u] = 0ull;
    if (tu.hist)
        for (uint32_t p = blockIdx.x; p < n_pheno; p += gridDim.x) thr_update_block(tu.hist, tu.hist_base, tu.bins, tu.topn, tu.thr_host, tu.thr, p);
}

hipError_t launch_chunk_prep(uint32_t* cand_cnt, uint32_t n_pheno, unsigned long long* tested, uint32_t* key_count,
                             unsigned long long* bitmap, uint64_t bitmap_words, uint32_t* seg_cnt, uint32_t n_seg_words, const PrepThr& tu,
                             hipStream_t st) {
    uint64_t n = n_pheno > TESTED_SHARDS ? n_pheno : TESTED_SHARDS;
    if (n_seg_words > n) n = n_seg_words;
    if (bitmap_words / 8u > n) n = bitmap_words / 8u;
    const uint64_t blocks = std::min<uint64_t>((n + 255u) / 256u, 8192u);
    if (blocks * 256u < std::max<uint64_t>(std::max<uint64_t>(n_pheno, TESTED_SHARDS), n_seg_words)) return hipErrorInvalidValue;
    if (tu.hist && (tu.bins % 1024u || tu.bins / 256u > 64u)) return hipErrorInvalidValue;
    launch_last(chunk_prep_kernel, dim3((uint32_t)blocks), dim3(256), 0, st, cand_cnt, n_pheno, tested, key_count, bitmap, bitmap_words,
                       seg_cnt, n_seg_words, tu);
    return hipGetLastError();
}

size_t coarse_lds_bytes(uint32_t n_kgroups, uint32_t T) { return (size_t)n_kgroups * 8u * T * 1024u + 1536u + 8u * 768u; }

template <int T, int NS, int TH = 512>
static hipError_t launch_coarse_t(const CoarseArgs& a, uint32_t rows_per_block, uint32_t n_rowblocks, size_t lds,
                                  hipStream_t st) {
    lds += (size_t)(TH / 64 - 8) * 768u;
    if (lds > 64 * 1024) {
        hipError_t e = hipFuncSetAttribute((const void*)coarse_kernel<T, NS, TH>, hipFuncAttributeMaxDynamicSharedMemorySize,
                                           (int)lds);
        if (e != hipSuccess) return e;
    }
    static const int grid_env = (int)exp_int("KGWAS_COARSE_GRIDLG", -1);
    const uint32_t grid_lg = (grid_env >= 0 ? grid_env != 0 : true) && a.n_lgroups > 1 ? 1u : 0u;
    const uint32_t grid = grid_lg ? (n_rowblocks + 7u) / 8u * 8u * a.n_lgroups : n_rowblocks;
    launch_last(coarse_kernel<T, NS, TH>, dim3(grid), dim3(TH), lds, st, a, rows_per_block, n_rowblocks, grid_lg);
    return hipGetLastError();
}

hipError_t launch_coarse(const CoarseArgs& a, uint32_t T, uint32_t rows_per_block, hipStream_t st) {
    if (a.n_rows == 0) return hipSuccess;
    const size_t lds = coarse_lds_bytes(a.n_kgroups, T);
    if (lds > 160u * 1024u) return hipErrorInvalidValue;
    static const int th_env = (int)exp_int("KGWAS_COARSE_TH", 768);
    const bool wide_block = th_env == 768 && a.n_slices == 1 && T <= 4 && lds + 4u * 768u <= 160u * 1024u;
    const uint32_t threads = wide_block ? 768 : 512;
    if ((a.n_rows * a.src.stride_dw + a.src.off_dw + a.src.avail_dw) * 4ull >= (1ull << 32)) return hipErrorInvalidValue;
    const uint32_t rpp = (threads >> 6) * 64u;
    rows_per_block = (rows_per_block + rpp - 1) / rpp * rpp;
    const uint32_t n_rowblocks = (uint32_t)((a.n_rows + rows_per_block - 1) / rows_per_block);
#ifdef KGWAS_COARSE_BENCH_ONLY
    if (a.n_slices == 1 && T == 7) return launch_coarse_t<7, 1>(a, rows_per_block, n_rowblocks, lds, st);
    if (a.n_slices == 2 && T == 8) return launch_coarse_t<8, 2>(a, rows_per_block, n_rowblocks, lds, st);
    return hipErrorInvalidValue;
#else
    if (wide_block) {
        switch (T) {
            case 1: return launch_coarse_t<1, 1, 768>(a, rows_per_block, n_rowblocks, lds, st);
            case 2: return launch_coarse_t<2, 1, 768>(a, rows_per_block, n_rowblocks, lds, st);
            case 3: return launch_coarse_t<3, 1, 768>(a, rows_per_block, n_rowblocks, lds, st);
            case 4: return launch_coarse_t<4, 1, 768>(a, rows_per_block, n_rowblocks, lds, st);
        }
    }
    if (a.n_slices == 1) {
        switch (T) {
            case 1: return launch_coarse_t<1, 1>(a, rows_per_block, n_rowblocks, lds, st);
            case 2: return launch_coarse_t<2, 1>(a, rows_per_block, n_rowblocks, lds, st);
            case 3: return launch_coarse_t<3, 1>(a, rows_per_block, n_rowblocks, lds, st);
            case 4: return launch_coarse_t<4, 1>(a, rows_per_block, n_rowblocks, lds, st);
            case 5: return launch_coarse_t<5, 1>(a, rows_per_block, n_rowblocks, lds, st);
            case 6: return launch_coarse_t<6, 1>(a, rows_per_block, n_rowblocks, lds, st);
            case 7: return launch_coarse_t<7, 1>(a, rows_per_block, n_rowblocks, lds, st);
            case 8: return launch_coarse_t<8, 1>(a, rows_per_block, n_rowblocks, lds, st);
        }
    } else if (a.n_slices == 2) {
        switch (T) {
            case 2: return launch_coarse_t<2, 2>(a, rows_per_block, n_rowblocks, lds, st);
            case 4: return launch_coarse_t<4, 2>(a, rows_per_block, n_rowblocks, lds, st);
            case 6: return launch_coarse_t<6, 2>(a, rows_per_block, n_rowblocks, lds, st);
            case 8: return launch_coarse_t<8, 2>(a, rows_per_block, n_rowblocks, lds, st);
        }
    }
    return hipErrorInvalidValue;
#endif
}

#ifdef KGWAS_COARSE_TIMELINE
extern "C" int kgwas_debug_coarse_timeline(unsigned long long* out, unsigned long long n) {
    if (n > 2 * 16 * 64) n = 2 * 16 * 64;
    return (int)hipMemcpyFromSymbol(out, HIP_SYMBOL(g_coarse_tl), n * sizeof(unsigned long long), 0, hipMemcpyDeviceToHost);
}
#endif

hipError_t launch_rescore(const ScoreArgs& a, const uint32_t* keys, const uint32_t* surv_off, const uint32_t* surv_cnt,
                          uint32_t row_bits, uint32_t* tile_pref, uint32_t* tile_cnt, double* tmp_score,
                          const uint32_t* key_count, uint32_t* meta, hipStream_t st) {
    if (a.n_pheno == 0) return hipSuccess;
    const uint32_t row_mask = row_bits >= 32 ? 0xFFFFFFFFu : ((1u << row_bits) - 1u);
    const size_t ybytes = 64u * (size_t)a.W_m * sizeof(float);
    static const bool ylds_ok = exp_str("KGWAS_RESCORE_YLDS") ? atoi(exp_str("KGWAS_RESCORE_YLDS")) != 0 : true;
    [[maybe_unused]] static const int ns_env = (int)exp_int("KGWAS_RESCORE_NS", 1);
    static const bool dyn = exp_int("KGWAS_RESCORE_DYN", 0) != 0;
    static const uint32_t grid = (uint64_t)exp_int("KGWAS_RESCORE_GRID", 2048u);
    uint32_t* ticket = dyn ? const_cast<uint32_t*>(key_count) + 1 : nullptr;
#ifdef KGWAS_EXPERIMENTS
    if (ylds_ok && ybytes <= 16384u && ns_env == 2)
        hipLaunchKernelGGL((rescore_kernel<true, false, 2>), dim3(grid), dim3(256), ybytes, st, a, keys, surv_off, surv_cnt, tile_pref, row_mask,
                           tmp_score, tile_cnt, ticket);
    else
#endif
    if (ylds_ok && ybytes <= 16384u)
        hipLaunchKernelGGL(rescore_kernel<true>, dim3(grid), dim3(256), ybytes, st, a, keys, surv_off, surv_cnt, tile_pref, row_mask,
                           tmp_score, tile_cnt, ticket);
    else
        hipLaunchKernelGGL(rescore_kernel<false>, dim3(grid), dim3(256), 0, st, a, keys, surv_off, surv_cnt, tile_pref, row_mask,
                           tmp_score, tile_cnt, ticket);
    launch_last(compact_kernel, dim3(2048 + 1), dim3(256), 0, st, a, keys, surv_off, surv_cnt, tile_pref, row_mask, tmp_score,
                       tile_cnt, key_count, meta);
    return hipGetLastError();
}

hipError_t launch_rescore_direct(const ScoreArgs& a, const uint32_t* keys, const uint32_t* surv_off, const uint32_t* surv_cnt,
                                 uint32_t row_bits, const uint32_t* tile_pref, hipStream_t st) {
    if (a.n_pheno == 0) return hipSuccess;
    const uint32_t row_mask = row_bits >= 32 ? 0xFFFFFFFFu : ((1u << row_bits) - 1u);
    const size_t ybytes = 64u * (size_t)a.W_m * sizeof(float);
    if (ybytes <= 16384u)
        launch_last(rescore_kernel<true, true>, dim3(512), dim3(256), ybytes, st, a, keys, surv_off, surv_cnt, tile_pref, row_mask,
                           (double*)nullptr, (uint32_t*)nullptr, (uint32_t*)nullptr);
    else
        launch_last(rescore_kernel<false, true>, dim3(512), dim3(256), 0, st, a, keys, surv_off, surv_cnt, tile_pref, row_mask,
                           (double*)nullptr, (uint32_t*)nullptr, (uint32_t*)nullptr);
    return hipGetLastError();
}

}
```

### kmersgwas_amd/csrc/score_mx.hip

```cpp
#include <stdlib.h>

#include <algorithm>

#include "score_common.h"

#ifndef KGWAS_MX_ABLATE
#define KGWAS_MX_ABLATE 0
#endif

#ifndef KGWAS_MX_NT
#define KGWAS_MX_NT 0
#endif

#ifndef KGWAS_MX_WARM
#define KGWAS_MX_WARM 0
#endif
#ifndef KGWAS_MX_PERSIST
#define KGWAS_MX_PERSIST 1
#endif

namespace kgwas {

typedef int mxv8i __attribute__((ext_vector_type(8)));
typedef float mxv4f __attribute__((ext_vector_type(4)));
// ... 301 lines not shown
                    const float sq = __builtin_amdgcn_sqrtf(f * (Nf - f)) * 0.99999905f;
                    float2 tm;
                    tm.x = ok ? sq : __builtin_huge_valf();
                    tm.y = (a.eg_max + fminf(a.rall_max, f * a.rmax_max)) * 1.000001f;
                    trm[e] = tm;
                }
                __builtin_amdgcn_wave_barrier();
            }

            float alc[CT];
            float al_min = __builtin_huge_valf();
#pragma unroll
            for (int t = 0; t < CT; t++) {
                alc[t] = colc[t * 16 + m];
                al_min = fminf(al_min, alc[t]);
            }
            const bool ones_lane = m == 15u;
#pragma unroll
            for (int w = 0; w < NW; w++) {
                float sqd[16], er[16];
#pragma unroll
                for (int i = 0; i < 16; i += 2) {
                    const float4 v = *reinterpret_cast<const float4*>(trm + kb * (RT * 4u) + 16 * w + i);
                    sqd[i] = v.x;
                    er[i] = v.y;
                    sqd[i + 1] = v.z;
                    er[i + 1] = v.w;
                }
                auto pair_margin = [&](int i, int t, float al) {
                    const int gi = 16 * w + i;
                    return fmaf(-al, sqd[i], fabsf(acc[gi >> 2][t][gi & 3]));
                };
                uint64_t hit[16];
                if (!(KGWAS_MX_ABLATE & 1)) {
                    float mx[16];
#pragma unroll
                    for (int i = 0; i < 16; i++) {
                        const int gi = 16 * w + i;
                        const float v = acc[gi >> 2][CT - 1][gi & 3];
                        mx[i] = ones_lane ? 0.0f : fabsf(v);
                    }
#pragma unroll
                    for (int t = 0; t + 1 < CT; t++)
#pragma unroll
                        for (int i = 0; i < 16; i++) {
                            const int gi = 16 * w + i;
                            mx[i] = fmaxf(mx[i], fabsf(acc[gi >> 2][t][gi & 3]));
                        }
#pragma unroll
                    for (int i = 0; i < 16; i++) hit[i] = __ballot(fmaf(-al_min, sqd[i], mx[i]) + er[i] >= 0.0f);
                } else {
#pragma unroll
                    for (int i = 0; i < 16; i++) hit[i] = 0;
                    int x = 0;
#pragma unroll
                    for (int i = 0; i < 16; i++)
#pragma unroll
                        for (int t = 0; t < CT; t++) x ^= __float_as_int(acc[(16 * w + i) >> 2][t][i & 3]);
                    hit[0] = __ballot(x == 0x7fffffff);
                }
                uint64_t hit_any = 0;
#pragma unroll
                for (int i = 0; i < 16; i++) hit_any |= hit[i];
                if ((KGWAS_MX_ABLATE & 32) && hit_any) {
                    if (lane == 0) atomicAdd(&a.tested[0], 0ull);
                    hit_any = 0;
                }
                if (hit_any) {
                    uint32_t mb[CT];
#pragma unroll
                    for (int t = 0; t < CT; t++) mb[t] = 0;
#pragma unroll
                    for (int i = 0; i < 16; i++) {
                        if (hit[i]) {
#pragma unroll
                            for (int t = 0; t < CT; t++) {
                                float al = alc[t];
                                asm volatile("" : "+v"(al));
                                mb[t] |= (pair_margin(i, t, al) + er[i] >= 0.0f) ? (1u << i) : 0u;
                            }
                        }
                    }
                    unsigned short* bm16 = reinterpret_cast<unsigned short*>(a.bitmap) + ((rbase >> 6) + w) * 4u + kb;
#pragma unroll
                    for (int t = 0; t < CT; t++)
                        if (mb[t]) bm16[(uint64_t)colp[t * 16 + m] * a.words_per_col * 4u] = (unsigned short)mb[t];
                }
            }
            __builtin_amdgcn_wave_barrier();
#pragma unroll
            for (int rt = 0; rt < RT; rt++) ro[rt] = ro_next[rt];
        }
    }
#if KGWAS_MX_WARM
    asm volatile("s_waitcnt vmcnt(0)" ::: "memory");
#endif
    if (a.tested) {
        uint32_t v = tested_local;
#pragma unroll
        for (int d = 1; d < 64; d <<= 1) v += __shfl_xor(v, d);
        if (lane == 0u && v) atomicAdd(&a.tested[blockIdx.x % TESTED_SHARDS], (unsigned long long)v);
    }
}

size_t mx_lds_bytes(uint32_t n_steps, uint32_t CT, uint32_t n_slices, uint32_t s1_fp6) {
    const uint32_t sb = n_slices == 1 ? MX_PART0 : (s1_fp6 ? 2u * MX_PART0 : MX_PART0 + 1024u);
    return (size_t)n_steps * CT * sb + 3u * 112u * 4u + 12u * 768u + 256u;
}
uint32_t mx_step_bytes_rt(uint32_t n_slices, uint32_t s1_fp6) { return n_slices == 1 ? MX_PART0 : (s1_fp6 ? 2u * MX_PART0 : MX_PART0 + 1024u); }
uint32_t mx_row_tiles(uint32_t CT) { return 4u; }

template <int CT, int RT, int NS, int S1F, int TH = 512>
static hipError_t launch_mx_t(const MxArgs& a, uint32_t rows_per_block, size_t lds, hipStream_t st) {
    const uint32_t rpp = (TH / 64) * RT * 16u;
    rows_per_block = (rows_per_block + rpp - 1) / rpp * rpp;
    const uint32_t n_rowblocks = (uint32_t)((a.n_rows + rows_per_block - 1) / rows_per_block);
    if (lds > 64 * 1024) {
        hipError_t e = hipFuncSetAttribute((const void*)mx_kernel<CT, RT, NS, S1F, TH>, hipFuncAttributeMaxDynamicSharedMemorySize, (int)lds);
        if (e != hipSuccess) return e;
    }
    const uint32_t grid_lg = a.n_lgroups > 1 ? 1u : 0u;
    uint32_t grid = grid_lg ? (n_rowblocks + 7u) / 8u * 8u * a.n_lgroups : n_rowblocks;
    if (KGWAS_MX_PERSIST && !grid_lg) {
        static int n_cu = 0;
        if (!n_cu) {
            int dev = 0;
            hipDeviceProp_t pr;
            n_cu = (hipGetDevice(&dev) == hipSuccess && hipGetDeviceProperties(&pr, dev) == hipSuccess && pr.multiProcessorCount > 0) ? pr.multiProcessorCount : 256;
        }
        const uint64_t n_pass = (a.n_rows + rpp - 1) / rpp;
        grid = (uint32_t)std::min<uint64_t>(n_pass, (uint64_t)n_cu);
    }
    launch_last(mx_kernel<CT, RT, NS, S1F, TH>, dim3(grid), dim3(TH), lds, st, a, rows_per_block, n_rowblocks, grid_lg);
    return hipGetLastError();
}

template <int NS, int S1F>
static hipError_t launch_mx_ct(const MxArgs& a, uint32_t CT, uint32_t rows_per_block, size_t lds, hipStream_t st) {
    switch (CT) {
        case 1: return launch_mx_t<1, 4, NS, S1F, 768>(a, rows_per_block, lds, st);
        case 2: return launch_mx_t<2, 4, NS, S1F, 768>(a, rows_per_block, lds, st);
        case 3: return launch_mx_t<3, 4, NS, S1F, 768>(a, rows_per_block, lds, st);
        case 4: return launch_mx_t<4, 4, NS, S1F>(a, rows_per_block, lds, st);
        case 5: return launch_mx_t<5, 4, NS, S1F>(a, rows_per_block, lds, st);
        case 6: return launch_mx_t<6, 4, NS, S1F>(a, rows_per_block, lds, st);
        case 7: return launch_mx_t<7, 4, NS, S1F>(a, rows_per_block, lds, st);
    }
    return hipErrorInvalidValue;
}

hipError_t launch_mx(const MxArgs& a, uint32_t CT, uint32_t rows_per_block, hipStream_t st) {
    if (a.n_rows == 0) return hipSuccess;
    const size_t lds = mx_lds_bytes(4u * a.n_full + a.n_quarter, CT, a.n_slices, a.s1_fp6);
    if (lds > 160u * 1024u) return hipErrorInvalidValue;
    if ((a.n_rows * a.src.stride_dw + a.src.off_dw + a.src.avail_dw) * 4ull >= (1ull << 32)) return hipErrorInvalidValue;
#ifdef KGWAS_MX_BENCH_ONLY
    if (a.n_slices == 2 && !a.s1_fp6 && CT == 7) return launch_mx_t<7, 4, 2, 4>(a, rows_per_block, lds, st);
    return hipErrorInvalidValue;
#else
    if (a.n_slices == 1) return launch_mx_ct<1, 4>(a, CT, rows_per_block, lds, st);
    if (a.n_slices == 2 && !a.s1_fp6) return launch_mx_ct<2, 4>(a, CT, rows_per_block, lds, st);
    if (a.n_slices == 2 && a.s1_fp6) return launch_mx_ct<2, 2>(a, CT, rows_per_block, lds, st);
    return hipErrorInvalidValue;
#endif
}

}
```

### kmersgwas_amd/csrc/score_mxs.hip

```cpp
#include <stdlib.h>

#include <algorithm>
#include <type_traits>

#include "score_common.h"

#ifndef KGWAS_MXS_DEPHASE
#define KGWAS_MXS_DEPHASE 0
#endif
#ifndef KGWAS_MXS_ROWS_NT
#define KGWAS_MXS_ROWS_NT 0
#endif
#ifndef KGWAS_MXS_ABLATE
#define KGWAS_MXS_ABLATE 0
#endif

#ifndef KGWAS_MXS_PROF
#define KGWAS_MXS_PROF 0
#endif

namespace kgwas {

#if KGWAS_MXS_PROF
__device__ unsigned long long mxs_prof[8];
// ... 332 lines not shown
                for (int rt = 0; rt < RT; rt++) *reinterpret_cast<mxsv4f*>(n1s + kb * NSL + rt * 4) = acc[rt][CT - 1];
            }
            __builtin_amdgcn_wave_barrier();
            const uint64_t left = rbase < a.n_rows ? a.n_rows - rbase : 0;
            const uint32_t rows_here = left < RT * 16u ? (uint32_t)left : RT * 16u;
            const bool mac_any = a.S >= 2u * a.min_count;
            const uint32_t span = a.S - 2u * a.min_count;
            if (lane < RT * 16u) {
                const uint32_t e = lane;
                const uint32_t kbe = e / NSL, ie = e % NSL;
                const uint32_t row = 16u * (ie >> 2) + 4u * kbe + (ie & 3u);
                const float f = n1s[e];
                const uint32_t n1r = (uint32_t)f;
                const bool ok = mac_any & (row < rows_here) & ((n1r - a.min_count) <= span);
                if (lg == 0 && grp == 0) tested_local += ok ? 1u : 0u;
                const float sq = __builtin_amdgcn_sqrtf(f * (Nf - f)) * 0.99999905f;
                float2 tm;
                tm.x = ok ? sq : __builtin_huge_valf();
                tm.y = (a.eg_max + fminf(a.rall_max, f * a.rmax_max)) * 1.000001f;
                trm[e] = tm;
            }
            __builtin_amdgcn_wave_barrier();
        }
        float alc[CT];
        float al_min = __builtin_huge_valf();
#pragma unroll
        for (int t = 0; t < CT; t++) {
            alc[t] = colc[grp * SLOTS + t * 16 + m];
            al_min = fminf(al_min, alc[t]);
        }
        const bool ones_lane = m == 15u;
        {
            float sqd[NSL], er[NSL];
#pragma unroll
            for (int i = 0; i < NSL; i += 2) {
                const float4 v = *reinterpret_cast<const float4*>(trm + kb * NSL + i);
                sqd[i] = v.x;
                er[i] = v.y;
                sqd[i + 1] = v.z;
                er[i + 1] = v.w;
            }
            uint64_t hit[NSL];
            if (!(KGWAS_MXS_ABLATE & 1)) {
                float mx[NSL];
#pragma unroll
                for (int i = 0; i < NSL; i++) {
                    const float v = acc[i >> 2][CT - 1][i & 3];
                    mx[i] = ones_lane ? 0.0f : fabsf(v);
                }
#pragma unroll
                for (int t = 0; t + 1 < CT; t++)
#pragma unroll
                    for (int i = 0; i < NSL; i++) mx[i] = fmaxf(mx[i], fabsf(acc[i >> 2][t][i & 3]));
#pragma unroll
                for (int i = 0; i < NSL; i++) hit[i] = __ballot(fmaf(-al_min, sqd[i], mx[i]) + er[i] >= 0.0f);
            } else {
#pragma unroll
                for (int i = 0; i < NSL; i++) hit[i] = 0;
                int x = 0;
#pragma unroll
                for (int i = 0; i < NSL; i++)
#pragma unroll
                    for (int t = 0; t < CT; t++) x ^= __float_as_int(acc[i >> 2][t][i & 3]);
                hit[0] = __ballot(x == 0x7fffffff);
            }
            uint64_t hit_any = 0;
#pragma unroll
            for (int i = 0; i < NSL; i++) hit_any |= hit[i];
            if (hit_any) {
                uint32_t mb[CT];
#pragma unroll
                for (int t = 0; t < CT; t++) mb[t] = 0;
#pragma unroll
                for (int i = 0; i < NSL; i++) {
                    if (hit[i]) {
#pragma unroll
                        for (int t = 0; t < CT; t++) {
                            float al = alc[t];
                            asm volatile("" : "+v"(al));
                            mb[t] |= (fmaf(-al, sqd[i], fabsf(acc[i >> 2][t][i & 3])) + er[i] >= 0.0f) ? (1u << i) : 0u;
                        }
                    }
                }
                if (RT == 4) {
                    unsigned short* bm16 = reinterpret_cast<unsigned short*>(a.bitmap) + (rbase >> 6) * 4u + kb;
#pragma unroll
                    for (int t = 0; t < CT; t++)
                        if (mb[t]) bm16[(uint64_t)colp[t * 16 + m] * a.words_per_col * 4u] = (unsigned short)mb[t];
                } else {
                    unsigned char* bm8 = reinterpret_cast<unsigned char*>(a.bitmap) + (rbase >> 6) * 8u + kb * 2u + ((rbase >> 5) & 1u);
#pragma unroll
                    for (int t = 0; t < CT; t++)
                        if (mb[t]) bm8[(uint64_t)colp[t * 16 + m] * a.words_per_col * 8u] = (unsigned char)mb[t];
                }
            }
        }
        __builtin_amdgcn_wave_barrier();
#if KGWAS_MXS_PROF
        pf_epi += __builtin_readcyclecounter() - te0;
#endif
    }
    if (!late)
        for (uint32_t i = 0; i < n_dummy; i++) dummy_step();
#if KGWAS_MXS_PROF
    if (threadIdx.x == 0) {
        atomicAdd(&mxs_prof[0], pf_sync);
        atomicAdd(&mxs_prof[1], pf_step);
        atomicAdd(&mxs_prof[2], pf_epi);
        atomicAdd(&mxs_prof[3], pf_nstep);
        atomicAdd(&mxs_prof[4], (unsigned long long)n_passes);
        atomicAdd(&mxs_prof[5], __builtin_readcyclecounter() - pf_k0);
        atomicAdd(&mxs_prof[6], pf_bar);
        atomicAdd(&mxs_prof[7], pf_issue);
    }
#endif
    asm volatile("s_waitcnt vmcnt(0)" ::: "memory");
    if (a.tested) {
        uint32_t v = tested_local;
#pragma unroll
        for (int d = 1; d < 64; d <<= 1) v += __shfl_xor(v, d);
        if (lane == 0u && v) atomicAdd(&a.tested[blockIdx.x % TESTED_SHARDS], (unsigned long long)v);
    }
}

static size_t mxs_lds_bytes_t(uint32_t cta, uint32_t rt, uint32_t ng, uint32_t th, uint32_t ring) {
    const uint32_t waves = th / 64u;
    return (size_t)ring * ((cta * MXS_SB + 1023u) / 1024u * 1024u) + 3u * cta * 16u * 4u + waves * (rt * 192u) + waves * 256u + (KGWAS_MXS_DEPHASE ? waves : waves / ng) * (rt * 1024u);
}

template <int CT, int RT, int NG, int TH>
static hipError_t launch_mxs_t(const MxArgs& a, uint32_t rows_per_block, hipStream_t st) {
    const uint32_t rpp = (TH / 64 / NG) * RT * 16u;
    rows_per_block = (rows_per_block + rpp - 1) / rpp * rpp;
    const uint32_t n_rowblocks = (uint32_t)((a.n_rows + rows_per_block - 1) / rows_per_block);
    const bool ring4 = mxs_lds_bytes_t(CT * NG, RT, NG, TH, 4) <= 160u * 1024u;
    const size_t lds = mxs_lds_bytes_t(CT * NG, RT, NG, TH, ring4 ? 4 : 3);
    if (lds > 160u * 1024u) return hipErrorInvalidValue;
    const void* fn = ring4 ? (const void*)mxs_kernel<CT, RT, NG, TH, 4> : (const void*)mxs_kernel<CT, RT, NG, TH, 3>;
    if (lds > 64 * 1024) {
        hipError_t e = hipFuncSetAttribute(fn, hipFuncAttributeMaxDynamicSharedMemorySize, (int)lds);
        if (e != hipSuccess) return e;
    }
    const uint32_t grid = a.n_lgroups > 1 ? (n_rowblocks + 7u) / 8u * 8u * a.n_lgroups : n_rowblocks;
    if (ring4)
        launch_last(mxs_kernel<CT, RT, NG, TH, 4>, dim3(grid), dim3(TH), lds, st, a, rows_per_block, n_rowblocks);
    else
        launch_last(mxs_kernel<CT, RT, NG, TH, 3>, dim3(grid), dim3(TH), lds, st, a, rows_per_block, n_rowblocks);
    return hipGetLastError();
}

bool mxs_supported(uint32_t CT, uint32_t NG, uint32_t n_slices, uint32_t s1_fp6) {
    return n_slices == 2 && !s1_fp6 && ((NG == 1 && CT >= 3 && CT <= 13) || (NG == 2 && CT >= 4 && CT <= 7));
}
size_t mxs_lds_bytes(uint32_t CT, uint32_t NG) {
    const uint32_t rt = (NG == 1 && CT > 7) ? 2u : 4u;
    const size_t b4 = mxs_lds_bytes_t(CT * NG, rt, NG, 512, 4);
    return b4 <= 160u * 1024u ? b4 : mxs_lds_bytes_t(CT * NG, rt, NG, 512, 3);
}

hipError_t launch_mxs(const MxArgs& a, uint32_t CT, uint32_t NG, uint32_t form, uint32_t rows_per_block, hipStream_t st) {
    if (a.n_rows == 0) return hipSuccess;
    if (!mxs_supported(CT, NG, a.n_slices, a.s1_fp6)) return hipErrorInvalidValue;
    if ((a.n_rows * a.src.stride_dw + a.src.off_dw + a.src.avail_dw) * 4ull >= (1ull << 32)) return hipErrorInvalidValue;
#ifdef KGWAS_MXS_BENCH_ONLY
    if (NG == 2 && CT == 7) return launch_mxs_t<7, 4, 2, 512>(a, rows_per_block, st);
    if (NG == 1 && CT == 13) return form == 2 ? launch_mxs_t<13, 4, 1, 256>(a, rows_per_block, st) : launch_mxs_t<13, 2, 1, 512>(a, rows_per_block, st);
    if (NG == 1 && CT == 7) return launch_mxs_t<7, 4, 1, 512>(a, rows_per_block, st);
    return hipErrorInvalidValue;
#else
    if (NG == 2) switch (CT) {
            case 4: return launch_mxs_t<4, 4, 2, 512>(a, rows_per_block, st);
            case 5: return launch_mxs_t<5, 4, 2, 512>(a, rows_per_block, st);
            case 6: return launch_mxs_t<6, 4, 2, 512>(a, rows_per_block, st);
            case 7: return launch_mxs_t<7, 4, 2, 512>(a, rows_per_block, st);
        }
    else switch (CT) {
            case 3: return launch_mxs_t<3, 4, 1, 512>(a, rows_per_block, st);
            case 4: return launch_mxs_t<4, 4, 1, 512>(a, rows_per_block, st);
            case 5: return launch_mxs_t<5, 4, 1, 512>(a, rows_per_block, st);
            case 6: return launch_mxs_t<6, 4, 1, 512>(a, rows_per_block, st);
            case 7: return launch_mxs_t<7, 4, 1, 512>(a, rows_per_block, st);
            case 8: return form == 2 ? launch_mxs_t<8, 4, 1, 256>(a, rows_per_block, st) : launch_mxs_t<8, 2, 1, 512>(a, rows_per_block, st);
            case 9: return form == 2 ? launch_mxs_t<9, 4, 1, 256>(a, rows_per_block, st) : launch_mxs_t<9, 2, 1, 512>(a, rows_per_block, st);
            case 10: return form == 2 ? launch_mxs_t<10, 4, 1, 256>(a, rows_per_block, st) : launch_mxs_t<10, 2, 1, 512>(a, rows_per_block, st);
            case 11: return form == 2 ? launch_mxs_t<11, 4, 1, 256>(a, rows_per_block, st) : launch_mxs_t<11, 2, 1, 512>(a, rows_per_block, st);
            case 12: return form == 2 ? launch_mxs_t<12, 4, 1, 256>(a, rows_per_block, st) : launch_mxs_t<12, 2, 1, 512>(a, rows_per_block, st);
            case 13: return form == 2 ? launch_mxs_t<13, 4, 1, 256>(a, rows_per_block, st) : launch_mxs_t<13, 2, 1, 512>(a, rows_per_block, st);
        }
    return hipErrorInvalidValue;
#endif
}

}
```

### kmersgwas_amd/csrc/score_narrow.hip

```cpp
#include <stdlib.h>

#include <algorithm>

#include "score_common.h"

#ifndef KGWAS_NARROW_ABLATE
#define KGWAS_NARROW_ABLATE 0
#endif

namespace kgwas {

typedef int nv8i __attribute__((ext_vector_type(8)));
typedef float nv4f __attribute__((ext_vector_type(4)));

namespace {
constexpr int NRT = 4;
}

__device__ __forceinline__ void narrow_group(const uint32_t (&piece)[NRT][4], const uint4* sg, nv4f (&acc)[NRT]) {
#pragma unroll
    for (int j = 0; j < 4; j++) {
        uint4 s0, s1;
        if (KGWAS_NARROW_ABLATE & 16) {
            s0 = make_uint4(j, 1, 2, 3);
// ... 268 lines not shown
        const char* fetch_ptr = rows_base + fb + 16u * lane;                                      \
        if (fb < total_b && ((q) * 4u + wave) * 64u < rows_per_block) {             \
            EACH(NARROW_LOAD)                                                                     \
        }                                                                                         \
    }
    NARROW_FETCH(NARROW_EACH, 0u)
#if KGWAS_NARROW_DEPTH == 2
    NARROW_FETCH(NARROW_EACH2, 1u)
#endif
    uint32_t pofs[NRT];
#pragma unroll
    for (int rt = 0; rt < NRT; rt++) pofs[rt] = (rt * 16u + m) * stride_b + off_b;
    auto process = [&](uint64_t rbase) {
        __builtin_amdgcn_wave_barrier();
        nv4f acc[NRT];
#pragma unroll
        for (int rt = 0; rt < NRT; rt++) acc[rt] = (nv4f){0.0f, 0.0f, 0.0f, 0.0f};
        for (uint32_t g = 0; g < a.n_kgroups; g++) {
            uint32_t b0 = 64u * g + 16u * kb, b1 = b0 + 8u;
            b0 = b0 + 8u <= avail_b ? b0 : avail_b - 8u;
            b1 = b1 + 8u <= avail_b ? b1 : avail_b - 8u;
            uint32_t piece[NRT][4];
#pragma unroll
            for (int rt = 0; rt < NRT; rt++) {
                const char* rp = stage + pofs[rt];
                uint2 lo, hi;
                if (KGWAS_NARROW_ABLATE & 8) {
                    lo = make_uint2(lane * 2654435761u + g, rt + b0);
                    hi = make_uint2(lane + b1, lane * 40503u);
                } else {
                    lo = *reinterpret_cast<const uint2*>(rp + b0);
                    hi = *reinterpret_cast<const uint2*>(rp + b1);
                }
                piece[rt][0] = lo.x;
                piece[rt][1] = lo.y;
                piece[rt][2] = hi.x;
                piece[rt][3] = hi.y;
            }
            narrow_group(piece, nlds + (size_t)g * 4u * 128u + lane * 2u, acc);
        }
        if (KGWAS_NARROW_ABLATE & 4) {
            float x = 0;
#pragma unroll
            for (int rt = 0; rt < NRT; rt++) x += acc[rt][0] + acc[rt][1] + acc[rt][2] + acc[rt][3];
            if (x == 12345.678f) tested_local++;
        } else {
            narrow_test(a, lcols, L, acc, lane, rbase, mac_any, span, tested_local);
        }
        __builtin_amdgcn_wave_barrier();
    };
#define NARROW_PASS(EACH, ps)                                                                                     \
    {                                                                                                             \
        EACH(NARROW_PUT)    \
        NARROW_FETCH(EACH, (ps) + KGWAS_NARROW_DEPTH)                                                             \
        process(pass_row0(ps));                                                                                   \
    }
#if KGWAS_NARROW_DEPTH == 2
    for (uint32_t ps = 0;; ps += 2u) {
        if (!pass_exists(ps)) break;
        NARROW_PASS(NARROW_EACH, ps)
        if (!pass_exists(ps + 1u)) break;
        NARROW_PASS(NARROW_EACH2, ps + 1u)
    }
#undef NARROW_EACH2
#else
    for (uint32_t ps = 0; pass_exists(ps); ps++) NARROW_PASS(NARROW_EACH, ps)
#endif
#undef NARROW_PASS
#undef NARROW_FETCH
#undef NARROW_EACH
#undef NARROW_LOAD
#undef NARROW_PUT
    __syncthreads();
    narrow_flush_counts(a, L);
    if (a.tested) {
        uint32_t v = tested_local;
#pragma unroll
        for (int dd = 1; dd < 64; dd <<= 1) v += __shfl_xor(v, dd);
        if (lane == 0u && v) atomicAdd(&a.tested[blockIdx.x % TESTED_SHARDS], (unsigned long long)v);
    }
}

constexpr uint32_t BM_WORDS = 1024;

__global__ void __launch_bounds__(256) bitmap_count_kernel(const unsigned long long* bm, uint64_t words_per_col, uint32_t n_words,
                                                           uint32_t n_blocks, uint32_t* blk_cnt, unsigned long long* blk_mask) {
    __shared__ uint32_t part[4];
    const uint32_t p = blockIdx.y, b = blockIdx.x;
    const unsigned long long* w = bm + (uint64_t)p * words_per_col;
    uint32_t c = 0;
#pragma unroll
    for (int i = 0; i < 4; i++) {
        const uint32_t x = b * BM_WORDS + threadIdx.x * 4u + i;
        if (x < n_words) c += __popcll(w[x]);
    }
    const unsigned long long m = __ballot(c != 0u);
    if ((threadIdx.x & 63u) == 0u) blk_mask[((uint64_t)p * n_blocks + b) * 4u + (threadIdx.x >> 6)] = m;
#pragma unroll
    for (int d = 1; d < 64; d <<= 1) c += __shfl_xor(c, d);
    if ((threadIdx.x & 63u) == 0u) part[threadIdx.x >> 6] = c;
    __syncthreads();
    if (threadIdx.x == 0) blk_cnt[p * n_blocks + b] = part[0] + part[1] + part[2] + part[3];
}

__global__ void __launch_bounds__(256) bitmap_scan_kernel(uint32_t* blk_cnt, uint32_t n_blocks, uint32_t* col_total) {
    __shared__ uint32_t part[256];
    __shared__ uint32_t carry;
    const uint32_t p = blockIdx.x;
    if (threadIdx.x == 0) carry = 0;
    __syncthreads();
    for (uint32_t b0 = 0; b0 < n_blocks; b0 += 256u) {
        const uint32_t b = b0 + threadIdx.x;
        const uint32_t v = b < n_blocks ? blk_cnt[p * n_blocks + b] : 0u;
        part[threadIdx.x] = v;
        __syncthreads();
        for (uint32_t d = 1; d < 256u; d <<= 1) {
            const uint32_t x = threadIdx.x >= d ? part[threadIdx.x - d] : 0u;
            __syncthreads();
            part[threadIdx.x] += x;
            __syncthreads();
        }
        if (b < n_blocks) blk_cnt[p * n_blocks + b] = carry + part[threadIdx.x] - v;
        __syncthreads();
        if (threadIdx.x == 255u) carry += part[255];
        __syncthreads();
    }
    if (threadIdx.x == 0) col_total[p] = carry;
}

__device__ __forceinline__ void bitmap_bases_block(const uint32_t* col_total, uint32_t n_pheno, uint32_t key_cap, uint32_t* surv_off,
                                                   uint32_t* surv_cnt, uint32_t* key_count, uint32_t* tile_pref) {
    __shared__ uint32_t part[256];
    __shared__ uint32_t carry;
    if (threadIdx.x == 0) carry = 0;
    __syncthreads();
    for (uint32_t p0 = 0; p0 < n_pheno; p0 += 256u) {
        const uint32_t p = p0 + threadIdx.x;
        const uint32_t v = p < n_pheno ? col_total[p] : 0u;
        part[threadIdx.x] = v;
        __syncthreads();
        for (uint32_t d = 1; d < 256u; d <<= 1) {
            const uint32_t x = threadIdx.x >= d ? part[threadIdx.x - d] : 0u;
            __syncthreads();
            part[threadIdx.x] += x;
            __syncthreads();
        }
        if (p < n_pheno) {
            surv_off[p] = carry + part[threadIdx.x] - v;
            surv_cnt[p] = v;
        }
        __syncthreads();
        if (threadIdx.x == 255u) carry += part[255];
        __syncthreads();
    }
    if (threadIdx.x == 0) *key_count = carry;
    const bool over = carry > key_cap;
    __syncthreads();
    if (over)
        for (uint32_t p = threadIdx.x; p < n_pheno; p += 256u) surv_cnt[p] = 0u;
    if (threadIdx.x == 0) carry = 0;
    __syncthreads();
    for (uint32_t p0 = 0; p0 < n_pheno; p0 += 256u) {
        const uint32_t p = p0 + threadIdx.x;
        const uint32_t v = (p < n_pheno && !over) ? (col_total[p] + 255u) / 256u : 0u;
        part[threadIdx.x] = v;
        __syncthreads();
        for (uint32_t d = 1; d < 256u; d <<= 1) {
            const uint32_t x = threadIdx.x >= d ? part[threadIdx.x - d] : 0u;
            __syncthreads();
            part[threadIdx.x] += x;
            __syncthreads();
        }
        if (p < n_pheno) tile_pref[p] = carry + part[threadIdx.x] - v;
        __syncthreads();
        if (threadIdx.x == 255u) carry += part[255];
        __syncthreads();
    }
    if (threadIdx.x == 0) tile_pref[n_pheno] = carry;
    __syncthreads();
}

__global__ void __launch_bounds__(256) bitmap_scatter_kernel(unsigned long long* bm, uint64_t words_per_col, uint32_t n_words,
                                                             uint32_t n_blocks, const uint32_t* blk_off, const uint32_t* col_total,
                                                             const unsigned long long* blk_mask, uint32_t n_pheno, uint32_t* surv_off,
                                                             uint32_t* surv_cnt, uint32_t* key_count, uint32_t* tile_pref, uint32_t* keys,
                                                             uint32_t key_cap, uint32_t row_bits, bool nibble_transposed) {
    __shared__ uint32_t part[4];
    __shared__ uint32_t basep[4];
    const uint32_t p = blockIdx.y, b = blockIdx.x;
    if (p == 0u && b == 0u) bitmap_bases_block(col_total, n_pheno, key_cap, surv_off, surv_cnt, key_count, tile_pref);
    const uint32_t my_off = blk_off[p * n_blocks + b];
    const uint32_t next_off = b + 1u < n_blocks ? blk_off[p * n_blocks + b + 1u] : col_total[p];
    if (next_off == my_off) return;
    const uint32_t lane = threadIdx.x & 63u, wave = threadIdx.x >> 6;
    uint32_t col_base;
    {
        uint32_t v = 0;
        for (uint32_t q = threadIdx.x; q < p; q += 256u) v += col_total[q];
#pragma unroll
        for (int d = 1; d < 64; d <<= 1) v += __shfl_xor(v, d);
        if (lane == 0u) basep[wave] = v;
        __syncthreads();
        col_base = basep[0] + basep[1] + basep[2] + basep[3];
    }
    const bool mine = (blk_mask[((uint64_t)p * n_blocks + b) * 4u + wave] >> lane) & 1ull;
    unsigned long long* w = bm + (uint64_t)p * words_per_col;
    unsigned long long x[4] = {0ull, 0ull, 0ull, 0ull};
    uint32_t c = 0;
    if (mine) {
#pragma unroll
        for (int i = 0; i < 4; i++) {
            const uint32_t idx = b * BM_WORDS + threadIdx.x * 4u + i;
            if (idx < n_words) {
                x[i] = w[idx];
                if (x[i]) w[idx] = 0ull;
            }
            c += __popcll(x[i]);
        }
        if (nibble_transposed) {
#pragma unroll
            for (int i = 0; i < 4; i++) {
                if (!x[i]) continue;
                unsigned long long y = 0;
#pragma unroll
                for (int kg = 0; kg < 4; kg++)
#pragma unroll
                    for (int rt = 0; rt < 4; rt++) y |= ((x[i] >> (4 * (4 * kg + rt))) & 0xFull) << (4 * (4 * rt + kg));
                x[i] = y;
            }
        }
    }
    uint32_t incl = c;
#pragma unroll
    for (int d = 1; d < 64; d <<= 1) {
        const uint32_t t = __shfl_up(incl, d);
        if ((int)lane >= d) incl += t;
    }
    if (lane == 63u) part[wave] = incl;
    __syncthreads();
    uint32_t o = col_base + my_off + incl - c;
    for (uint32_t k = 0; k < wave; k++) o += part[k];
#pragma unroll
    for (int i = 0; i < 4; i++) {
        unsigned long long v = x[i];
        const uint32_t row0 = (b * BM_WORDS + threadIdx.x * 4u + i) * 64u;
        while (v) {
            const uint32_t bit = __ffsll((long long)v) - 1u;
            v &= v - 1ull;
            if (o < key_cap) keys[o] = (p << row_bits) | (row0 + bit);
            o++;
        }
    }
}

hipError_t launch_bitmap_keys(unsigned long long* bitmap, uint64_t words_per_col, uint64_t n_rows, uint32_t n_pheno, uint32_t* blk_scratch,
                              unsigned long long* blk_mask, uint32_t* keys_sorted, uint32_t key_cap, uint32_t row_bits, uint32_t* surv_off,
                              uint32_t* surv_cnt, uint32_t* key_count, uint32_t* tile_pref, bool nibble_transposed, hipStream_t st) {
    const uint32_t n_words = (uint32_t)((n_rows + 63) / 64);
    const uint32_t n_blocks = (n_words + BM_WORDS - 1) / BM_WORDS;
    hipLaunchKernelGGL(bitmap_count_kernel, dim3(n_blocks, n_pheno), dim3(256), 0, st, bitmap, words_per_col, n_words, n_blocks, blk_scratch, blk_mask);
    uint32_t* col_total = blk_scratch + (size_t)n_pheno * n_blocks;
    hipLaunchKernelGGL(bitmap_scan_kernel, dim3(n_pheno), dim3(256), 0, st, blk_scratch, n_blocks, col_total);
    hipLaunchKernelGGL(bitmap_scatter_kernel, dim3(n_blocks, n_pheno), dim3(256), 0, st, bitmap, words_per_col, n_words, n_blocks, blk_scratch,
                       col_total, blk_mask, n_pheno, surv_off, surv_cnt, key_count, tile_pref, keys_sorted, key_cap, row_bits, nibble_transposed);
    return hipGetLastError();
}

__global__ void __launch_bounds__(256) narrow_keys_kernel(const unsigned long long* bm, uint64_t words_per_col, uint32_t n_words, uint32_t n_segs,
                                                          uint32_t n_pheno, const uint32_t* seg_cnt, uint32_t* keys, uint32_t key_cap,
                                                          uint32_t row_bits, uint32_t* surv_off, uint32_t* surv_cnt, uint32_t* key_count,
                                                          uint32_t* tile_pref, uint32_t* meta, const unsigned long long* tested_shards) {
    __shared__ uint32_t red[4][NARROW_MAX_COLS + 1];
    __shared__ uint32_t tot[NARROW_MAX_COLS + 1];
    __shared__ uint32_t part[4];
    const uint32_t p = blockIdx.y, b = blockIdx.x;
    const uint32_t lane = threadIdx.x & 63u, wave = threadIdx.x >> 6;
    uint32_t cs[NARROW_MAX_COLS] = {0u, 0u, 0u, 0u}, mine = 0;
    for (uint32_t q = 0; q < n_pheno; q++)
        for (uint32_t k = threadIdx.x; k < n_segs; k += 256u) {
            const uint32_t v = seg_cnt[q * n_segs + k];
            cs[q] += v;
            if (q == p && k < b) mine += v;
        }
#pragma unroll
    for (int d = 1; d < 64; d <<= 1) {
        mine += __shfl_xor(mine, d);
#pragma unroll
        for (int q = 0; q < (int)NARROW_MAX_COLS; q++) cs[q] += __shfl_xor(cs[q], d);
    }
    if (lane == 0u) {
#pragma unroll
        for (int q = 0; q < (int)NARROW_MAX_COLS; q++) red[wave][q] = cs[q];
        red[wave][NARROW_MAX_COLS] = mine;
    }
    __syncthreads();
    if (threadIdx.x <= NARROW_MAX_COLS) tot[threadIdx.x] = red[0][threadIdx.x] + red[1][threadIdx.x] + red[2][threadIdx.x] + red[3][threadIdx.x];
    __syncthreads();
    uint32_t total = 0, off_p = 0;
    for (uint32_t q = 0; q < n_pheno; q++) {
        if (q < p) off_p += tot[q];
        total += tot[q];
    }
    const bool over = total > key_cap;
    if (b == 0u && p == 0u) {
        __shared__ unsigned long long tsum[4];
        unsigned long long v = tested_shards[threadIdx.x];
#pragma unroll
        for (int d = 1; d < 64; d <<= 1) v += __shfl_xor(v, d);
        if (lane == 0u) tsum[wave] = v;
        __syncthreads();
        if (threadIdx.x == 0u) {
            const unsigned long long tt = tsum[0] + tsum[1] + tsum[2] + tsum[3];
            meta[2u * n_pheno + 2u] = (uint32_t)tt;
            meta[2u * n_pheno + 3u] = (uint32_t)(tt >> 32);
        }
    }
    if (b == 0u && p == 0u && threadIdx.x == 0u) {
        uint32_t o = 0, t = 0;
        for (uint32_t q = 0; q < n_pheno; q++) {
            const uint32_t c = over ? 0u : tot[q];
            surv_off[q] = o;
            surv_cnt[q] = c;
            tile_pref[q] = t;
            meta[q] = c;
            meta[n_pheno + q] = o;
            o += tot[q];
            t += (c + 255u) / 256u;
        }
        tile_pref[n_pheno] = t;
        *key_count = total;
        meta[2u * n_pheno] = over ? 0u : total;
        meta[2u * n_pheno + 1u] = total;
    }
    if (over || seg_cnt[p * n_segs + b] == 0u) return;
    const unsigned long long* w = bm + (uint64_t)p * words_per_col;
    unsigned long long x[4];
    uint32_t c = 0;
#pragma unroll
    for (int i = 0; i < 4; i++) {
        const uint32_t idx = b * BM_WORDS + threadIdx.x * 4u + i;
        x[i] = idx < n_words ? w[idx] : 0ull;
        c += __popcll(x[i]);
    }
    uint32_t incl = c;
#pragma unroll
    for (int d = 1; d < 64; d <<= 1) {
        const uint32_t t = __shfl_up(incl, d);
        if ((int)lane >= d) incl += t;
    }
    if (lane == 63u) part[wave] = incl;
    __syncthreads();
    uint32_t o = off_p + tot[NARROW_MAX_COLS] + incl - c;
    for (uint32_t k = 0; k < wave; k++) o += part[k];
#pragma unroll
    for (int i = 0; i < 4; i++) {
        unsigned long long v = x[i];
        const uint32_t row0 = (b * BM_WORDS + threadIdx.x * 4u + i) * 64u;
        while (v) {
            const uint32_t bit = __ffsll((long long)v) - 1u;
            v &= v - 1ull;
            if (o < key_cap) keys[o] = (p << row_bits) | (row0 + bit);
            o++;
        }
    }
}

hipError_t launch_narrow_keys(const unsigned long long* bitmap, uint64_t words_per_col, uint64_t n_rows, uint32_t n_pheno, const uint32_t* seg_cnt,
                              uint32_t* keys_sorted, uint32_t key_cap, uint32_t row_bits, uint32_t* surv_off, uint32_t* surv_cnt,
                              uint32_t* key_count, uint32_t* tile_pref, uint32_t* meta, const unsigned long long* tested_shards, hipStream_t st) {
    static_assert(TESTED_SHARDS == 256, "block (0, 0) sums one counter per thread");
    if (n_pheno < 1 || n_pheno > NARROW_MAX_COLS) return hipErrorInvalidValue;
    const uint32_t n_words = (uint32_t)((n_rows + 63) / 64);
    const uint32_t n_segs = (n_words + BM_WORDS - 1) / BM_WORDS;
    hipLaunchKernelGGL(narrow_keys_kernel, dim3(n_segs, n_pheno), dim3(256), 0, st, bitmap, words_per_col, n_words, n_segs, n_pheno, seg_cnt,
                       keys_sorted, key_cap, row_bits, surv_off, surv_cnt, key_count, tile_pref, meta, tested_shards);
    return hipGetLastError();
}

size_t narrow_lds_bytes(uint32_t n_kgroups) { return (size_t)n_kgroups * 4u * 2048u + 4u * sizeof(NarrowCol); }

template <int NP>
static hipError_t launch_staged_t(const NarrowArgs& a, uint32_t rows_per_block, uint32_t n_blocks, uint32_t stage_bytes, size_t lds,
                                  hipStream_t st, bool last) {
    if (lds > 64 * 1024) {
        hipError_t e = hipFuncSetAttribute((const void*)narrow_staged_kernel<NP>, hipFuncAttributeMaxDynamicSharedMemorySize, (int)lds);
        if (e != hipSuccess) return e;
    }
    if (last)
        launch_last(narrow_staged_kernel<NP>, dim3(n_blocks), dim3(256), lds, st, a, rows_per_block, stage_bytes);
    else
        hipLaunchKernelGGL((narrow_staged_kernel<NP>), dim3(n_blocks), dim3(256), lds, st, a, rows_per_block, stage_bytes);
    return hipGetLastError();
}

hipError_t launch_narrow(const NarrowArgs& a, uint32_t rows_per_block, hipStream_t st) {
    if (a.n_rows == 0) return hipSuccess;
    if (a.n_pheno < 1 || a.n_pheno > NARROW_MAX_COLS) return hipErrorInvalidValue;
    rows_per_block = (rows_per_block + 255u) / 256u * 256u;
    const uint32_t stride_b = (uint32_t)a.src.stride_dw * 4u;
    const int np = (int)((64u * stride_b + 1023u) / 1024u);
    const uint32_t stage_bytes = (uint32_t)np * 1024u;
    const size_t lds_staged = narrow_lds_bytes(a.n_kgroups) + 4u * (size_t)stage_bytes;
    static const bool no_stage = exp_int("KGWAS_NARROW_STAGED", 1) == 0;
    uint64_t n_staged = 0;
    if (!no_stage && lds_staged <= 53u * 1024u && np <= 12 && (reinterpret_cast<uintptr_t>(a.src.base) & 15u) == 0) {
        const uint64_t readable_b = (a.n_rows + a.slack_rows) * (uint64_t)stride_b;
        const uint64_t total_b = a.n_rows * (uint64_t)stride_b, over = (uint64_t)np * 1024u - 64ull * stride_b;
        if ((a.n_rows - 1u) / 64u * 64u * stride_b + (uint64_t)np * 1024u <= readable_b)
            n_staged = a.n_rows;
        else if (total_b > over)
            n_staged = (total_b - over) / (64ull * stride_b) * 64ull;
    }
    if (n_staged) {
        NarrowArgs s1 = a;
        s1.n_rows = n_staged;
        const uint32_t nb = (uint32_t)((n_staged + rows_per_block - 1) / rows_per_block);
        hipError_t e = hipSuccess;
        switch (np) {
            case 1: e = launch_staged_t<1>(s1, rows_per_block, nb, stage_bytes, lds_staged, st, n_staged == a.n_rows); break;
            case 2: e = launch_staged_t<2>(s1, rows_per_block, nb, stage_bytes, lds_staged, st, n_staged == a.n_rows); break;
            case 3: e = launch_staged_t<3>(s1, rows_per_block, nb, stage_bytes, lds_staged, st, n_staged == a.n_rows); break;
            case 4: e = launch_staged_t<4>(s1, rows_per_block, nb, stage_bytes, lds_staged, st, n_staged == a.n_rows); break;
            case 5: e = launch_staged_t<5>(s1, rows_per_block, nb, stage_bytes, lds_staged, st, n_staged == a.n_rows); break;
            case 6: e = launch_staged_t<6>(s1, rows_per_block, nb, stage_bytes, lds_staged, st, n_staged == a.n_rows); break;
            case 7: e = launch_staged_t<7>(s1, rows_per_block, nb, stage_bytes, lds_staged, st, n_staged == a.n_rows); break;
            case 8: e = launch_staged_t<8>(s1, rows_per_block, nb, stage_bytes, lds_staged, st, n_staged == a.n_rows); break;
            case 9: e = launch_staged_t<9>(s1, rows_per_block, nb, stage_bytes, lds_staged, st, n_staged == a.n_rows); break;
            case 10: e = launch_staged_t<10>(s1, rows_per_block, nb, stage_bytes, lds_staged, st, n_staged == a.n_rows); break;
            case 11: e = launch_staged_t<11>(s1, rows_per_block, nb, stage_bytes, lds_staged, st, n_staged == a.n_rows); break;
            default: e = launch_staged_t<12>(s1, rows_per_block, nb, stage_bytes, lds_staged, st, n_staged == a.n_rows); break;
        }
        if (e != hipSuccess || n_staged == a.n_rows) return e;
    }
    NarrowArgs a2 = a;
    a2.src.base = a.src.base + n_staged * a.src.stride_dw;
    a2.n_rows = a.n_rows - n_staged;
    a2.row_off = (uint32_t)n_staged;
    const uint32_t n_blocks2 = (uint32_t)((a2.n_rows + rows_per_block - 1) / rows_per_block);
    const size_t lds = narrow_lds_bytes(a.n_kgroups);
    if (lds > 160u * 1024u) return hipErrorInvalidValue;
    if (lds > 64 * 1024) {
        hipError_t e = hipFuncSetAttribute((const void*)narrow_kernel, hipFuncAttributeMaxDynamicSharedMemorySize, (int)lds);
        if (e != hipSuccess) return e;
    }
    launch_last(narrow_kernel, dim3(n_blocks2), dim3(256), lds, st, a2, rows_per_block);
    return hipGetLastError();
}

}
```

Before: 530.1 billion.

## Track dirty bitmap groups with byte marks and fuse chunk tail into rescore

Filter kernels now record a byte mark per group of bitmap words they set, so the count and scatter kernels only popcount and clear marked regions instead of scanning the whole bitmap. The count kernel handles several blocks per workgroup, and the scatter kernel clears marks and reads words before its early exit. The threshold-update and meta/tested host copy tail is folded into the rescore launch through a new ChunkEnd argument, which saves a kernel launch per chunk. Launch bookkeeping counters are added to check that the stop event binds to the last launch. The cost is extra mark writes in the filter kernels and more complex cross-kernel invariants.

```diff
diff --git a/kmersgwas_amd/csrc/aux_kernels.hip b/kmersgwas_amd/csrc/aux_kernels.hip
--- a/kmersgwas_amd/csrc/aux_kernels.hip
+++ b/kmersgwas_amd/csrc/aux_kernels.hip
@@ -277,8 +277,7 @@
 
 hipError_t launch_chunk_tail(const uint32_t* meta, uint32_t n_meta, uint32_t* h_meta, const unsigned long long* tested, uint32_t n_tested,
                              unsigned long long* h_tested, const double* thr, uint32_t n_thr, double* h_thr, hipStream_t st) {
-    launch_last(chunk_tail_kernel, dim3(1), dim3(256), 0, st, meta, n_meta, h_meta, tested, n_tested, h_tested, thr, n_thr, h_thr);
-    return hipGetLastError();
+    return launch_last(chunk_tail_kernel, dim3(1), dim3(256), 0, st, meta, n_meta, h_meta, tested, n_tested, h_tested, thr, n_thr, h_thr);
 }
 
 __global__ void __launch_bounds__(256) thr_tail_kernel(const uint32_t* hist, const uint32_t* hist_base, uint32_t bins, const uint64_t* topn,
@@ -297,9 +296,8 @@
                            uint32_t n_pheno, const uint32_t* meta, uint32_t n_meta, uint32_t* h_meta, const unsigned long long* tested,
                            uint32_t n_tested, unsigned long long* h_tested, double* h_thr, hipStream_t st) {
     if (n_pheno == 0 || bins % 256u) return hipErrorInvalidValue;
-    launch_last(thr_tail_kernel, dim3(n_pheno), dim3(256), 0, st, hist, hist_base, bins, topn, thr_host, thr, meta, n_meta, h_meta, tested,
-                n_tested, h_tested, h_thr);
-    return hipGetLastError();
+    return launch_last(thr_tail_kernel, dim3(n_pheno), dim3(256), 0, st, hist, hist_base, bins, topn, thr_host, thr, meta, n_meta, h_meta, tested,
+                       n_tested, h_tested, h_thr);
 }
 
 hipError_t launch_records_to_host(const double* sc, const uint64_t* km, const uint32_t* rw, uint32_t n, double* h_sc, uint64_t* h_km, uint32_t* h_rw,
diff --git a/kmersgwas_amd/csrc/kernels.h b/kmersgwas_amd/csrc/kernels.h
--- a/kmersgwas_amd/csrc/kernels.h
+++ b/kmersgwas_amd/csrc/kernels.h
@@ -90,6 +90,8 @@
     const double* thr;
     unsigned long long* bitmap;
     uint64_t words_per_col;
+    unsigned char* marks;
+    uint64_t marks_per_col;
     unsigned long long* tested;
     float eg_max, rall_max, rmax_max;
 };
@@ -109,6 +111,8 @@
     const double* thr;
     unsigned long long* bitmap;
     uint64_t words_per_col;
+    unsigned char* marks;
+    uint64_t marks_per_col;
     unsigned long long* tested;
     float eg_max, rall_max, rmax_max;
 };
@@ -119,9 +123,22 @@
 bool mxs_supported(uint32_t CT, uint32_t NG, uint32_t n_slices, uint32_t s1_fp6);
 size_t mxs_lds_bytes(uint32_t CT, uint32_t NG);
 hipError_t launch_mxs(const MxArgs& a, uint32_t CT, uint32_t NG, uint32_t form, uint32_t rows_per_block, hipStream_t st);
+struct ChunkEnd {
+    const uint32_t* hist;
+    const uint32_t* hist_base;
+    uint32_t bins;
+    const uint64_t* topn;
+    const double* thr_host;
+    double* thr;
+    uint32_t* h_meta;
+    const unsigned long long* tested;
+    uint32_t n_tested;
+    unsigned long long* h_tested;
+    double* h_thr;
+};
 hipError_t launch_rescore(const ScoreArgs& a, const uint32_t* keys, const uint32_t* surv_off, const uint32_t* surv_cnt,
                           uint32_t row_bits, uint32_t* tile_pref, uint32_t* tile_cnt, double* tmp_score,
-                          const uint32_t* key_count, uint32_t* meta, hipStream_t st);
+                          const uint32_t* key_count, uint32_t* meta, const ChunkEnd* end, hipStream_t st);
 hipError_t launch_rescore_direct(const ScoreArgs& a, const uint32_t* keys, const uint32_t* surv_off, const uint32_t* surv_cnt,
                                  uint32_t row_bits, const uint32_t* tile_pref, hipStream_t st);
 struct PrepThr {
@@ -133,8 +150,8 @@
     double* thr;
 };
 hipError_t launch_chunk_prep(uint32_t* cand_cnt, uint32_t n_pheno, unsigned long long* tested, uint32_t* key_count,
-                             unsigned long long* bitmap, uint64_t bitmap_words, uint32_t* seg_cnt, uint32_t n_seg_words, const PrepThr& tu,
-                             hipStream_t st);
+                             unsigned long long* bitmap, uint64_t bitmap_words, unsigned char* marks, uint64_t mark_bytes, uint32_t* seg_cnt,
+                             uint32_t n_seg_words, const PrepThr& tu, hipStream_t st);
 
 constexpr int NARROW_SLICES = 3;
 constexpr uint32_t NARROW_MAX_COLS = 4;
@@ -163,8 +180,9 @@
     uint64_t slack_rows;
     uint32_t pack1;
 };
+constexpr uint64_t bitmap_marks_per_col(uint64_t words_per_col) { return ((words_per_col + 3u) / 4u + 3u) / 4u * 4u; }
 hipError_t launch_bitmap_keys(unsigned long long* bitmap, uint64_t words_per_col, uint64_t n_rows, uint32_t n_pheno, uint32_t* blk_scratch,
-                              unsigned long long* blk_mask, uint32_t* keys_sorted, uint32_t key_cap, uint32_t row_bits, uint32_t* surv_off,
+                              unsigned char* marks, uint32_t* keys_sorted, uint32_t key_cap, uint32_t row_bits, uint32_t* surv_off,
                               uint32_t* surv_cnt, uint32_t* key_count, uint32_t* tile_pref, bool nibble_transposed, hipStream_t st);
 hipError_t launch_narrow_keys(const unsigned long long* bitmap, uint64_t words_per_col, uint64_t n_rows, uint32_t n_pheno, const uint32_t* seg_cnt,
                               uint32_t* keys_sorted, uint32_t key_cap, uint32_t row_bits, uint32_t* surv_off, uint32_t* surv_cnt,
diff --git a/kmersgwas_amd/csrc/launch.h b/kmersgwas_amd/csrc/launch.h
--- a/kmersgwas_amd/csrc/launch.h
+++ b/kmersgwas_amd/csrc/launch.h
@@ -10,6 +10,8 @@
 namespace kgwas {
 
 extern thread_local hipEvent_t g_bound_stop;
+extern thread_local unsigned long long g_launches;
+extern thread_local unsigned long long g_bound_taken;
 
 template <class... KA, size_t... I>
 inline hipError_t launch_bound_impl(void (*kernel)(KA...), dim3 grid, dim3 block, size_t lds, hipStream_t st, hipEvent_t stop, std::tuple<KA...>& vals,
@@ -19,16 +21,27 @@
 }
 
 template <class... KA, class... A>
-inline void launch_last(void (*kernel)(KA...), dim3 grid, dim3 block, size_t lds, hipStream_t st, A&&... args) {
+inline void launch_mid(void (*kernel)(KA...), dim3 grid, dim3 block, size_t lds, hipStream_t st, A&&... args) {
+    static_assert(sizeof...(KA) == sizeof...(A), "one argument per kernel parameter");
+    g_launches++;
+    hipLaunchKernelGGL(kernel, grid, block, lds, st, static_cast<KA>(args)...);
+}
+
+template <class... KA, class... A>
+inline hipError_t launch_last(void (*kernel)(KA...), dim3 grid, dim3 block, size_t lds, hipStream_t st, A&&... args) {
     static_assert(sizeof...(KA) == sizeof...(A), "one argument per kernel parameter");
     const hipEvent_t stop = g_bound_stop;
     g_bound_stop = nullptr;
+    g_launches++;
     if (!stop) {
         hipLaunchKernelGGL(kernel, grid, block, lds, st, static_cast<KA>(args)...);
-        return;
+        return hipGetLastError();
     }
+    g_bound_taken = g_launches;
     std::tuple<KA...> vals(static_cast<KA>(args)...);
-    (void)launch_bound_impl(kernel, grid, block, lds, st, stop, vals, std::index_sequence_for<KA...>{});
+    const hipError_t e = launch_bound_impl(kernel, grid, block, lds, st, stop, vals, std::index_sequence_for<KA...>{});
+    const hipError_t earlier = hipGetLastError();
+    return e != hipSuccess ? e : earlier;
 }
 
 template <class F>
@@ -38,6 +51,8 @@
     if (g_bound_stop) {
         g_bound_stop = nullptr;
         if (e == hipSuccess) return hipEventRecord(ev, st);
+    } else if (e == hipSuccess && g_launches != g_bound_taken) {
+        return hipErrorInvalidValue;
     }
     return e;
 }
diff --git a/kmersgwas_amd/csrc/scan_create.cpp b/kmersgwas_amd/csrc/scan_create.cpp
--- a/kmersgwas_amd/csrc/scan_create.cpp
+++ b/kmersgwas_amd/csrc/scan_create.cpp
@@ -180,7 +180,7 @@
     s->bitmap_words = (s->chunk_max + 63) / 64;
     s->d_bitmap.alloc(P * s->bitmap_words);
     s->d_bm_blocks.alloc(P * ((s->bitmap_words + 1023) / 1024 + 1) + 4);
-    if (!s->narrow) s->d_bm_mask.alloc(P * ((s->bitmap_words + 1023) / 1024) * 4 + 4);
+    if (!s->narrow) s->d_bm_marks.alloc(P * bitmap_marks_per_col(s->bitmap_words));
     s->bitmap_clean = false;
     s->d_surv_cnt.alloc(P);
     s->d_surv_off.alloc(P);
diff --git a/kmersgwas_amd/csrc/scan_gpu.cpp b/kmersgwas_amd/csrc/scan_gpu.cpp
--- a/kmersgwas_amd/csrc/scan_gpu.cpp
+++ b/kmersgwas_amd/csrc/scan_gpu.cpp
@@ -334,9 +334,11 @@
         }
         const bool zero_bitmap = use_coarse && (s->narrow || !s->bitmap_clean);
         const uint64_t zero_words = !zero_bitmap ? 0 : (s->narrow ? s->n_pheno * n_words : s->d_bitmap.n);
+        const bool zero_marks = zero_bitmap && !s->narrow;
         const auto prep = [&] {
             return launch_chunk_prep(sl.d_cnt.p, (uint32_t)s->n_pheno, sl.d_tested.p, use_coarse ? s->d_key_count.p : nullptr,
-                                     zero_bitmap ? s->d_bitmap.p : nullptr, zero_words,
+                                     zero_bitmap ? s->d_bitmap.p : nullptr, zero_words, zero_marks ? s->d_bm_marks.p : nullptr,
+                                     zero_marks ? s->d_bm_marks.n : 0,
                                      (use_coarse && s->narrow) ? s->d_bm_blocks.p : nullptr, (use_coarse && s->narrow) ? (uint32_t)s->n_pheno * n_segs : 0u,
                                      tu, s->stream);
         };
@@ -344,6 +346,9 @@
         else KGWAS_HIP(prep());
     }
     sl.used_coarse = use_coarse;
+    static const bool tail_kernel = !(exp_int("KGWAS_TAIL_KERNEL", 1) == 0);
+    static const bool chunk_end_ok = !(exp_int("KGWAS_CHUNK_END", 1) == 0);
+    bool ended = false;
     if (use_coarse) {
         CoarseArgs c;
         memset(&c, 0, sizeof(c));
@@ -390,6 +395,8 @@
             s->bitmap_clean = false;
             c.bitmap = s->d_bitmap.p;
             c.words_per_col = n_words;
+            c.marks = s->d_bm_marks.p;
+            c.marks_per_col = bitmap_marks_per_col(n_words);
             for (uint32_t pi = 0; pi < M.n_parts; pi++) {
                 const kgwas_scan::CoarsePart& Pt = M.part[pi];
                 c.n_lgroups = Pt.n_lgroups;
@@ -417,6 +424,8 @@
                     x.thr = c.thr;
                     x.bitmap = c.bitmap;
                     x.words_per_col = c.words_per_col;
+                    x.marks = c.marks;
+                    x.marks_per_col = c.marks_per_col;
                     x.tested = c.tested;
                     x.eg_max = c.eg_max;
                     x.rall_max = c.rall_max;
@@ -444,16 +453,32 @@
             if (s->dbg_keep_surv) dbg_log_survivors(s);
             KGWAS_HIP(bind_stop(sl.ev_k1, s->stream, [&] { return launch_rescore_direct(a, s->d_surv_sorted.p, s->d_surv_off.p, s->d_surv_cnt.p, s->row_key_bits, s->d_tile_pref.p, s->stream); }));
         } else {
-        KGWAS_HIP(launch_bitmap_keys(s->d_bitmap.p, n_words, n_rows, (uint32_t)s->n_pheno, s->d_bm_blocks.p, s->d_bm_mask.p, s->d_surv_sorted.p, s->key_slots,
+        KGWAS_HIP(launch_bitmap_keys(s->d_bitmap.p, n_words, n_rows, (uint32_t)s->n_pheno, s->d_bm_blocks.p, s->d_bm_marks.p, s->d_surv_sorted.p, s->key_slots,
                                      s->row_key_bits, s->d_surv_off.p, s->d_surv_cnt.p, s->d_key_count.p, s->d_tile_pref.p, !s->narrow, s->stream));
         s->bitmap_clean = true;
         if (s->dbg_keep_surv) dbg_log_survivors(s);
         a.so_score = sl.d_so_score.p;
         a.so_kmer = sl.d_so_kmer.p;
         a.so_row = sl.d_so_row.p;
-        KGWAS_HIP(bind_stop(sl.ev_k1, s->stream, [&] {
+        ChunkEnd ce;
+        memset(&ce, 0, sizeof(ce));
+        if (chunk_end_ok && tail_kernel && sl.h_meta_dev && s->hist_ready) {
+            ce.hist = s->d_hist.p;
+            ce.hist_base = s->d_hist_base.p;
+            ce.bins = HIST_BINS;
+            ce.topn = s->d_topn.p;
+            ce.thr_host = s->d_thr_host.p;
+            ce.thr = s->d_thr.p;
+            ce.h_meta = sl.h_meta_dev;
+            ce.tested = sl.d_tested.p;
+            ce.n_tested = (uint32_t)TESTED_SHARDS;
+            ce.h_tested = sl.h_tested_dev;
+            ce.h_thr = s->lazy_any.load(std::memory_order_relaxed) ? sl.h_thr_dev : nullptr;
+            ended = true;
+        }
+        KGWAS_HIP(bind_stop(ended ? sl.ev_counts : sl.ev_k1, s->stream, [&] {
             return launch_rescore(a, s->d_surv_sorted.p, s->d_surv_off.p, s->d_surv_cnt.p, s->row_key_bits, s->d_tile_pref.p,
-                                  s->d_tile_cnt.p, s->d_tmp_score.p, s->d_key_count.p, sl.d_meta.p, s->stream);
+                                  s->d_tile_cnt.p, s->d_tmp_score.p, s->d_key_count.p, sl.d_meta.p, ended ? &ce : nullptr, s->stream);
         }));
         }
         s->st.score_launches++;
@@ -463,37 +488,39 @@
         KGWAS_HIP(hipEventRecord(sl.ev_k1, s->stream));
     }
     const bool fused_tail = use_coarse && s->narrow;
-    static const bool tail_kernel = !(exp_int("KGWAS_TAIL_KERNEL", 1) == 0);
-    const bool one_launch = use_coarse && tail_kernel && sl.h_meta_dev;
-    const bool thr_and_tail = one_launch && s->hist_ready && !fused_tail;
-    if (s->hist_ready && !fused_tail && !thr_and_tail)
-        KGWAS_HIP(launch_thr_update(s->d_hist.p, s->d_hist_base.p, HIST_BINS, s->d_topn.p, s->d_thr_host.p, s->d_thr.p,
-                                    (uint32_t)s->n_pheno, s->stream));
-    if (!fused_tail && !one_launch)
-        KGWAS_HIP(hipMemcpyAsync(sl.h_tested.p, sl.d_tested.p, TESTED_SHARDS * sizeof(unsigned long long), hipMemcpyDeviceToHost,
-                                 s->stream));
+    sl.k1_is_counts = ended;
     sl.tested_in_meta = fused_tail;
-    if (thr_and_tail) {
-        const bool thr_too = s->lazy_any.load(std::memory_order_relaxed);
-        KGWAS_HIP(bind_stop(sl.ev_counts, s->stream, [&] {
-            return launch_thr_tail(s->d_hist.p, s->d_hist_base.p, HIST_BINS, s->d_topn.p, s->d_thr_host.p, s->d_thr.p, (uint32_t)s->n_pheno, sl.d_meta.p,
-                                   (uint32_t)(2 * s->n_pheno + 4), sl.h_meta_dev, sl.d_tested.p, (uint32_t)TESTED_SHARDS, sl.h_tested_dev,
-                                   thr_too ? sl.h_thr_dev : nullptr, s->stream);
-        }));
-    } else if (one_launch) {
-        const bool thr_too = s->lazy_any.load(std::memory_order_relaxed);
-        KGWAS_HIP(bind_stop(sl.ev_counts, s->stream, [&] {
-            return launch_chunk_tail(sl.d_meta.p, (uint32_t)(2 * s->n_pheno + 4), sl.h_meta_dev, sl.d_tested.p, fused_tail ? 0u : (uint32_t)TESTED_SHARDS,
-                                     sl.h_tested_dev, s->d_thr.p, thr_too ? (uint32_t)s->n_pheno : 0u, sl.h_thr_dev, s->stream);
-        }));
-    } else if (use_coarse) {
-        KGWAS_HIP(hipMemcpyAsync(sl.h_meta.p, sl.d_meta.p, (2 * s->n_pheno + 4) * sizeof(uint32_t), hipMemcpyDeviceToHost, s->stream));
-        if (s->lazy_any.load(std::memory_order_relaxed))
-            KGWAS_HIP(hipMemcpyAsync(sl.h_thr.p, s->d_thr.p, s->n_pheno * sizeof(double), hipMemcpyDeviceToHost, s->stream));
-        KGWAS_HIP(hipEventRecord(sl.ev_counts, s->stream));
-    } else {
-        KGWAS_HIP(hipMemcpyAsync(sl.h_cnt.p, sl.d_cnt.p, s->n_pheno * sizeof(uint32_t), hipMemcpyDeviceToHost, s->stream));
-        KGWAS_HIP(hipEventRecord(sl.ev_done, s->stream));
+    if (!ended) {
+        const bool one_launch = use_coarse && tail_kernel && sl.h_meta_dev;
+        const bool thr_and_tail = one_launch && s->hist_ready && !fused_tail;
+        if (s->hist_ready && !fused_tail && !thr_and_tail)
+            KGWAS_HIP(launch_thr_update(s->d_hist.p, s->d_hist_base.p, HIST_BINS, s->d_topn.p, s->d_thr_host.p, s->d_thr.p,
+                                        (uint32_t)s->n_pheno, s->stream));
+        if (!fused_tail && !one_launch)
+            KGWAS_HIP(hipMemcpyAsync(sl.h_tested.p, sl.d_tested.p, TESTED_SHARDS * sizeof(unsigned long long), hipMemcpyDeviceToHost,
+                                     s->stream));
+        if (thr_and_tail) {
+            const bool thr_too = s->lazy_any.load(std::memory_order_relaxed);
+            KGWAS_HIP(bind_stop(sl.ev_counts, s->stream, [&] {
+                return launch_thr_tail(s->d_hist.p, s->d_hist_base.p, HIST_BINS, s->d_topn.p, s->d_thr_host.p, s->d_thr.p, (uint32_t)s->n_pheno, sl.d_meta.p,
+                                       (uint32_t)(2 * s->n_pheno + 4), sl.h_meta_dev, sl.d_tested.p, (uint32_t)TESTED_SHARDS, sl.h_tested_dev,
+                                       thr_too ? sl.h_thr_dev : nullptr, s->stream);
+            }));
+        } else if (one_launch) {
+            const bool thr_too = s->lazy_any.load(std::memory_order_relaxed);
+            KGWAS_HIP(bind_stop(sl.ev_counts, s->stream, [&] {
+                return launch_chunk_tail(sl.d_meta.p, (uint32_t)(2 * s->n_pheno + 4), sl.h_meta_dev, sl.d_tested.p, fused_tail ? 0u : (uint32_t)TESTED_SHARDS,
+                                         sl.h_tested_dev, s->d_thr.p, thr_too ? (uint32_t)s->n_pheno : 0u, sl.h_thr_dev, s->stream);
+            }));
+        } else if (use_coarse) {
+            KGWAS_HIP(hipMemcpyAsync(sl.h_meta.p, sl.d_meta.p, (2 * s->n_pheno + 4) * sizeof(uint32_t), hipMemcpyDeviceToHost, s->stream));
+            if (s->lazy_any.load(std::memory_order_relaxed))
+                KGWAS_HIP(hipMemcpyAsync(sl.h_thr.p, s->d_thr.p, s->n_pheno * sizeof(double), hipMemcpyDeviceToHost, s->stream));
+            KGWAS_HIP(hipEventRecord(sl.ev_counts, s->stream));
+        } else {
+            KGWAS_HIP(hipMemcpyAsync(sl.h_cnt.p, sl.d_cnt.p, s->n_pheno * sizeof(uint32_t), hipMemcpyDeviceToHost, s->stream));
+            KGWAS_HIP(hipEventRecord(sl.ev_done, s->stream));
+        }
     }
     sl.rows = d_rows;
     sl.first_row = first_row;
@@ -505,7 +532,7 @@
 bool chunk_complete(kgwas_scan* s, Slot& sl) {
     sl.busy = false;
     float ms = 0;
-    KGWAS_HIP(hipEventElapsedTime(&ms, sl.ev_k0, sl.ev_k1));
+    KGWAS_HIP(hipEventElapsedTime(&ms, sl.ev_k0, sl.k1_is_counts ? sl.ev_counts : sl.ev_k1));
     s->st.score_kernel_ms += ms;
     if (sl.used_coarse) {
         float mc = 0;
diff --git a/kmersgwas_amd/csrc/scan_host.cpp b/kmersgwas_amd/csrc/scan_host.cpp
--- a/kmersgwas_amd/csrc/scan_host.cpp
+++ b/kmersgwas_amd/csrc/scan_host.cpp
@@ -4,6 +4,7 @@
 namespace kgwas {
 
 thread_local hipEvent_t g_bound_stop = nullptr;
+thread_local unsigned long long g_launches = 0, g_bound_taken = 0;
 
 
 std::vector<int> parse_cpulist(const char* path) {
diff --git a/kmersgwas_amd/csrc/scan_internal.h b/kmersgwas_amd/csrc/scan_internal.h
--- a/kmersgwas_amd/csrc/scan_internal.h
+++ b/kmersgwas_amd/csrc/scan_internal.h
@@ -346,6 +346,7 @@
     PinBuf<unsigned long long> h_tested;
     hipEvent_t ev_sq0 = nullptr, ev_k0 = nullptr, ev_k1 = nullptr, ev_done = nullptr, ev_mid = nullptr;
     bool used_coarse = false;
+    bool k1_is_counts = false;
     int coarse_mode = 0;
     double cand_est = 0;
     const uint64_t* rows = nullptr;
@@ -423,7 +424,7 @@
     DevBuf<unsigned long long> d_bitmap;
     uint64_t bitmap_words = 0;
     DevBuf<uint32_t> d_bm_blocks;
-    DevBuf<unsigned long long> d_bm_mask;
+    DevBuf<unsigned char> d_bm_marks;
     bool bitmap_clean = false;
     uint64_t slack_rows = 0;
     DevBuf<uint32_t> d_surv_sorted, d_surv_cnt, d_surv_off, d_key_count;
diff --git a/kmersgwas_amd/csrc/score_coarse.hip b/kmersgwas_amd/csrc/score_coarse.hip
--- a/kmersgwas_amd/csrc/score_coarse.hip
+++ b/kmersgwas_amd/csrc/score_coarse.hip
@@ -262,9 +262,14 @@
             }
             if (hit_any) {
                 unsigned short* bm16 = reinterpret_cast<unsigned short*>(a.bitmap) + (rbase >> 6) * 4u + kg;
+                unsigned char* mk = a.marks + (rbase >> 8);
 #pragma unroll
                 for (int g = 0; g < PG; g++)
-                    if (mb[g]) bm16[(uint64_t)colp[g * 16 + m] * a.words_per_col * 4u] = (unsigned short)mb[g];
+                    if (mb[g]) {
+                        const uint64_t col = (uint64_t)colp[g * 16 + m];
+                        bm16[col * a.words_per_col * 4u] = (unsigned short)mb[g];
+                        mk[col * a.marks_per_col] = 1;
+                    }
             }
             TL_STAMP(53);
         }
@@ -529,16 +534,14 @@
     return red[0] + red[1] + red[2] + red[3];
 }
 
-__global__ void __launch_bounds__(256) compact_kernel(ScoreArgs a, const uint32_t* keys, const uint32_t* surv_off,
-                                                      const uint32_t* surv_cnt, const uint32_t* tile_pref, uint32_t row_mask,
-                                                      const double* tmp_score, const uint32_t* tile_cnt, const uint32_t* key_count,
-                                                      uint32_t* meta) {
+__device__ __forceinline__ void compact_block(const ScoreArgs& a, const uint32_t* keys, const uint32_t* surv_off, const uint32_t* surv_cnt,
+                                              const uint32_t* tile_pref, uint32_t row_mask, const double* tmp_score, const uint32_t* tile_cnt,
+                                              const uint32_t* key_count, uint32_t* meta, uint32_t n_workers, const ChunkEnd* end) {
     __shared__ uint32_t wcnt[4];
     __shared__ uint32_t red[4];
     __shared__ uint32_t cpre[257];
     const uint32_t n_tiles = tile_pref[a.n_pheno];
     const uint32_t lane = threadIdx.x & 63u, wave = threadIdx.x >> 6;
-    const uint32_t n_workers = gridDim.x - 1u;
     if (blockIdx.x == n_workers) {
         const uint32_t per = (n_tiles + 255u) / 256u;
         const uint32_t lo = threadIdx.x * per < n_tiles ? threadIdx.x * per : n_tiles;
@@ -565,11 +568,22 @@
             const uint32_t o0 = prefix_at(tile_pref[p]), o1 = prefix_at(tile_pref[p + 1u]);
             meta[p] = o1 - o0;
             meta[a.n_pheno + p] = o0;
+            if (end) {
+                end->h_meta[p] = o1 - o0;
+                end->h_meta[a.n_pheno + p] = o0;
+            }
         }
         if (threadIdx.x == 0u) {
+            const uint32_t kc = *key_count;
             meta[2u * a.n_pheno] = cpre[256];
-            meta[2u * a.n_pheno + 1u] = *key_count;
-        }
+            meta[2u * a.n_pheno + 1u] = kc;
+            if (end) {
+                end->h_meta[2u * a.n_pheno] = cpre[256];
+                end->h_meta[2u * a.n_pheno + 1u] = kc;
+            }
+        }
+        if (end)
+            for (uint32_t i = threadIdx.x; i < end->n_tested; i += 256u) end->h_tested[i] = end->tested[i];
         return;
     }
     uint32_t base = 0, done = 0;
@@ -601,9 +615,30 @@
     }
 }
 
+__global__ void __launch_bounds__(256) compact_kernel(ScoreArgs a, const uint32_t* keys, const uint32_t* surv_off,
+                                                      const uint32_t* surv_cnt, const uint32_t* tile_pref, uint32_t row_mask,
+                                                      const double* tmp_score, const uint32_t* tile_cnt, const uint32_t* key_count,
+                                                      uint32_t* meta) {
+    compact_block(a, keys, surv_off, surv_cnt, tile_pref, row_mask, tmp_score, tile_cnt, key_count, meta, gridDim.x - 1u, nullptr);
+}
+
+__global__ void __launch_bounds__(256) chunk_end_kernel(ScoreArgs a, const uint32_t* keys, const uint32_t* surv_off,
+                                                        const uint32_t* surv_cnt, const uint32_t* tile_pref, uint32_t row_mask,
+                                                        const double* tmp_score, const uint32_t* tile_cnt, const uint32_t* key_count,
+                                                        uint32_t* meta, ChunkEnd end) {
+    const uint32_t n_workers = gridDim.x - 1u - a.n_pheno;
+    if (blockIdx.x > n_workers) {
+        const uint32_t p = blockIdx.x - n_workers - 1u;
+        thr_update_block(end.hist, end.hist_base, end.bins, end.topn, end.thr_host, end.thr, p);
+        if (end.h_thr && threadIdx.x == 0) end.h_thr[p] = end.thr[p];
+        return;
+    }
+    compact_block(a, keys, surv_off, surv_cnt, tile_pref, row_mask, tmp_score, tile_cnt, key_count, meta, n_workers, &end);
+}
+
 __global__ void __launch_bounds__(256) chunk_prep_kernel(uint32_t* cand_cnt, uint32_t n_pheno, unsigned long long* tested, uint32_t* key_count,
-                                                         unsigned long long* bitmap, uint64_t bitmap_words, uint32_t* seg_cnt, uint32_t n_seg_words,
-                                                         PrepThr tu) {
+                                                         unsigned long long* bitmap, uint64_t bitmap_words, uint32_t* marks, uint64_t mark_dwords,
+                                                         uint32_t* seg_cnt, uint32_t n_seg_words, PrepThr tu) {
     const uint32_t i = blockIdx.x * blockDim.x + threadIdx.x;
     if (i < n_pheno) cand_cnt[i] = 0u;
     if (i < TESTED_SHARDS) tested[i] = 0ull;
@@ -613,22 +648,23 @@
     const uint64_t pairs = bitmap_words / 2u;
     for (uint64_t k = i; k < pairs; k += (uint64_t)gridDim.x * blockDim.x) b2[k] = make_ulonglong2(0ull, 0ull);
     if (i == 0 && (bitmap_words & 1u)) bitmap[bitmap_words - 1u] = 0ull;
+    for (uint64_t k = i; k < mark_dwords; k += (uint64_t)gridDim.x * blockDim.x) marks[k] = 0u;
     if (tu.hist)
         for (uint32_t p = blockIdx.x; p < n_pheno; p += gridDim.x) thr_update_block(tu.hist, tu.hist_base, tu.bins, tu.topn, tu.thr_host, tu.thr, p);
 }
 
 hipError_t launch_chunk_prep(uint32_t* cand_cnt, uint32_t n_pheno, unsigned long long* tested, uint32_t* key_count,
-                             unsigned long long* bitmap, uint64_t bitmap_words, uint32_t* seg_cnt, uint32_t n_seg_words, const PrepThr& tu,
-                             hipStream_t st) {
+                             unsigned long long* bitmap, uint64_t bitmap_words, unsigned char* marks, uint64_t mark_bytes, uint32_t* seg_cnt,
+                             uint32_t n_seg_words, const PrepThr& tu, hipStream_t st) {
+    if (mark_bytes % 4u || (reinterpret_cast<uintptr_t>(marks) & 3u)) return hipErrorInvalidValue;
     uint64_t n = n_pheno > TESTED_SHARDS ? n_pheno : TESTED_SHARDS;
     if (n_seg_words > n) n = n_seg_words;
     if (bitmap_words / 8u > n) n = bitmap_words / 8u;
     const uint64_t blocks = std::min<uint64_t>((n + 255u) / 256u, 8192u);
     if (blocks * 256u < std::max<uint64_t>(std::max<uint64_t>(n_pheno, TESTED_SHARDS), n_seg_words)) return hipErrorInvalidValue;
     if (tu.hist && (tu.bins % 1024u || tu.bins / 256u > 64u)) return hipErrorInvalidValue;
-    launch_last(chunk_prep_kernel, dim3((uint32_t)blocks), dim3(256), 0, st, cand_cnt, n_pheno, tested, key_count, bitmap, bitmap_words,
-                       seg_cnt, n_seg_words, tu);
-    return hipGetLastError();
+    return launch_last(chunk_prep_kernel, dim3((uint32_t)blocks), dim3(256), 0, st, cand_cnt, n_pheno, tested, key_count, bitmap, bitmap_words,
+                       reinterpret_cast<uint32_t*>(marks), mark_bytes / 4u, seg_cnt, n_seg_words, tu);
 }
 
 size_t coarse_lds_bytes(uint32_t n_kgroups, uint32_t T) { return (size_t)n_kgroups * 8u * T * 1024u + 1536u + 8u * 768u; }
@@ -645,8 +681,7 @@
     static const int grid_env = (int)exp_int("KGWAS_COARSE_GRIDLG", -1);
     const uint32_t grid_lg = (grid_env >= 0 ? grid_env != 0 : true) && a.n_lgroups > 1 ? 1u : 0u;
     const uint32_t grid = grid_lg ? (n_rowblocks + 7u) / 8u * 8u * a.n_lgroups : n_rowblocks;
-    launch_last(coarse_kernel<T, NS, TH>, dim3(grid), dim3(TH), lds, st, a, rows_per_block, n_rowblocks, grid_lg);
-    return hipGetLastError();
+    return launch_last(coarse_kernel<T, NS, TH>, dim3(grid), dim3(TH), lds, st, a, rows_per_block, n_rowblocks, grid_lg);
 }
 
 hipError_t launch_coarse(const CoarseArgs& a, uint32_t T, uint32_t rows_per_block, hipStream_t st) {
@@ -705,8 +740,9 @@
 
 hipError_t launch_rescore(const ScoreArgs& a, const uint32_t* keys, const uint32_t* surv_off, const uint32_t* surv_cnt,
                           uint32_t row_bits, uint32_t* tile_pref, uint32_t* tile_cnt, double* tmp_score,
-                          const uint32_t* key_count, uint32_t* meta, hipStream_t st) {
+                          const uint32_t* key_count, uint32_t* meta, const ChunkEnd* end, hipStream_t st) {
     if (a.n_pheno == 0) return hipSuccess;
+    if (end && (end->bins % 256u || !end->h_meta || !end->h_tested)) return hipErrorInvalidValue;
     const uint32_t row_mask = row_bits >= 32 ? 0xFFFFFFFFu : ((1u << row_bits) - 1u);
     const size_t ybytes = 64u * (size_t)a.W_m * sizeof(float);
     static const bool ylds_ok = exp_str("KGWAS_RESCORE_YLDS") ? atoi(exp_str("KGWAS_RESCORE_YLDS")) != 0 : true;
@@ -716,19 +752,21 @@
     uint32_t* ticket = dyn ? const_cast<uint32_t*>(key_count) + 1 : nullptr;
 #ifdef KGWAS_EXPERIMENTS
     if (ylds_ok && ybytes <= 16384u && ns_env == 2)
-        hipLaunchKernelGGL((rescore_kernel<true, false, 2>), dim3(grid), dim3(256), ybytes, st, a, keys, surv_off, surv_cnt, tile_pref, row_mask,
-                           tmp_score, tile_cnt, ticket);
+        launch_mid(rescore_kernel<true, false, 2>, dim3(grid), dim3(256), ybytes, st, a, keys, surv_off, surv_cnt, tile_pref, row_mask, tmp_score,
+                   tile_cnt, ticket);
     else
 #endif
     if (ylds_ok && ybytes <= 16384u)
-        hipLaunchKernelGGL(rescore_kernel<true>, dim3(grid), dim3(256), ybytes, st, a, keys, surv_off, surv_cnt, tile_pref, row_mask,
-                           tmp_score, tile_cnt, ticket);
+        launch_mid(rescore_kernel<true, false, 1>, dim3(grid), dim3(256), ybytes, st, a, keys, surv_off, surv_cnt, tile_pref, row_mask, tmp_score,
+                   tile_cnt, ticket);
     else
-        hipLaunchKernelGGL(rescore_kernel<false>, dim3(grid), dim3(256), 0, st, a, keys, surv_off, surv_cnt, tile_pref, row_mask,
-                           tmp_score, tile_cnt, ticket);
-    launch_last(compact_kernel, dim3(2048 + 1), dim3(256), 0, st, a, keys, surv_off, surv_cnt, tile_pref, row_mask, tmp_score,
+        launch_mid(rescore_kernel<false, false, 1>, dim3(grid), dim3(256), 0, st, a, keys, surv_off, surv_cnt, tile_pref, row_mask, tmp_score,
+                   tile_cnt, ticket);
+    if (end)
+        return launch_last(chunk_end_kernel, dim3(2048 + 1 + a.n_pheno), dim3(256), 0, st, a, keys, surv_off, surv_cnt, tile_pref, row_mask,
+                           tmp_score, tile_cnt, key_count, meta, *end);
+    return launch_last(compact_kernel, dim3(2048 + 1), dim3(256), 0, st, a, keys, surv_off, surv_cnt, tile_pref, row_mask, tmp_score,
                        tile_cnt, key_count, meta);
-    return hipGetLastError();
 }
 
 hipError_t launch_rescore_direct(const ScoreArgs& a, const uint32_t* keys, const uint32_t* surv_off, const uint32_t* surv_cnt,
@@ -737,12 +775,10 @@
     const uint32_t row_mask = row_bits >= 32 ? 0xFFFFFFFFu : ((1u << row_bits) - 1u);
     const size_t ybytes = 64u * (size_t)a.W_m * sizeof(float);
     if (ybytes <= 16384u)
-        launch_last(rescore_kernel<true, true>, dim3(512), dim3(256), ybytes, st, a, keys, surv_off, surv_cnt, tile_pref, row_mask,
+        return launch_last(rescore_kernel<true, true>, dim3(512), dim3(256), ybytes, st, a, keys, surv_off, surv_cnt, tile_pref, row_mask,
                            (double*)nullptr, (uint32_t*)nullptr, (uint32_t*)nullptr);
-    else
-        launch_last(rescore_kernel<false, true>, dim3(512), dim3(256), 0, st, a, keys, surv_off, surv_cnt, tile_pref, row_mask,
-                           (double*)nullptr, (uint32_t*)nullptr, (uint32_t*)nullptr);
-    return hipGetLastError();
-}
-
-}
+    return launch_last(rescore_kernel<false, true>, dim3(512), dim3(256), 0, st, a, keys, surv_off, surv_cnt, tile_pref, row_mask,
+                       (double*)nullptr, (uint32_t*)nullptr, (uint32_t*)nullptr);
+}
+
+}
diff --git a/kmersgwas_amd/csrc/score_mx.hip b/kmersgwas_amd/csrc/score_mx.hip
--- a/kmersgwas_amd/csrc/score_mx.hip
+++ b/kmersgwas_amd/csrc/score_mx.hip
@@ -407,9 +407,14 @@
                         }
                     }
                     unsigned short* bm16 = reinterpret_cast<unsigned short*>(a.bitmap) + ((rbase >> 6) + w) * 4u + kb;
+                    unsigned char* mk = a.marks + (((rbase >> 6) + w) >> 2);
 #pragma unroll
                     for (int t = 0; t < CT; t++)
-                        if (mb[t]) bm16[(uint64_t)colp[t * 16 + m] * a.words_per_col * 4u] = (unsigned short)mb[t];
+                        if (mb[t]) {
+                            const uint64_t col = (uint64_t)colp[t * 16 + m];
+                            bm16[col * a.words_per_col * 4u] = (unsigned short)mb[t];
+                            mk[col * a.marks_per_col] = 1;
+                        }
                 }
             }
             __builtin_amdgcn_wave_barrier();
@@ -456,8 +461,7 @@
         const uint64_t n_pass = (a.n_rows + rpp - 1) / rpp;
         grid = (uint32_t)std::min<uint64_t>(n_pass, (uint64_t)n_cu);
     }
-    launch_last(mx_kernel<CT, RT, NS, S1F, TH>, dim3(grid), dim3(TH), lds, st, a, rows_per_block, n_rowblocks, grid_lg);
-    return hipGetLastError();
+    return launch_last(mx_kernel<CT, RT, NS, S1F, TH>, dim3(grid), dim3(TH), lds, st, a, rows_per_block, n_rowblocks, grid_lg);
 }
 
 template <int NS, int S1F>
diff --git a/kmersgwas_amd/csrc/score_mxs.hip b/kmersgwas_amd/csrc/score_mxs.hip
--- a/kmersgwas_amd/csrc/score_mxs.hip
+++ b/kmersgwas_amd/csrc/score_mxs.hip
@@ -438,16 +438,25 @@
                         }
                     }
                 }
+                unsigned char* mk = a.marks + (rbase >> 8);
                 if (RT == 4) {
                     unsigned short* bm16 = reinterpret_cast<unsigned short*>(a.bitmap) + (rbase >> 6) * 4u + kb;
 #pragma unroll
                     for (int t = 0; t < CT; t++)
-                        if (mb[t]) bm16[(uint64_t)colp[t * 16 + m] * a.words_per_col * 4u] = (unsigned short)mb[t];
+                        if (mb[t]) {
+                            const uint64_t col = (uint64_t)colp[t * 16 + m];
+                            bm16[col * a.words_per_col * 4u] = (unsigned short)mb[t];
+                            mk[col * a.marks_per_col] = 1;
+                        }
                 } else {
                     unsigned char* bm8 = reinterpret_cast<unsigned char*>(a.bitmap) + (rbase >> 6) * 8u + kb * 2u + ((rbase >> 5) & 1u);
 #pragma unroll
                     for (int t = 0; t < CT; t++)
-                        if (mb[t]) bm8[(uint64_t)colp[t * 16 + m] * a.words_per_col * 8u] = (unsigned char)mb[t];
+                        if (mb[t]) {
+                            const uint64_t col = (uint64_t)colp[t * 16 + m];
+                            bm8[col * a.words_per_col * 8u] = (unsigned char)mb[t];
+                            mk[col * a.marks_per_col] = 1;
+                        }
                 }
             }
         }
@@ -499,10 +508,8 @@
     }
     const uint32_t grid = a.n_lgroups > 1 ? (n_rowblocks + 7u) / 8u * 8u * a.n_lgroups : n_rowblocks;
     if (ring4)
-        launch_last(mxs_kernel<CT, RT, NG, TH, 4>, dim3(grid), dim3(TH), lds, st, a, rows_per_block, n_rowblocks);
-    else
-        launch_last(mxs_kernel<CT, RT, NG, TH, 3>, dim3(grid), dim3(TH), lds, st, a, rows_per_block, n_rowblocks);
-    return hipGetLastError();
+        return launch_last(mxs_kernel<CT, RT, NG, TH, 4>, dim3(grid), dim3(TH), lds, st, a, rows_per_block, n_rowblocks);
+    return launch_last(mxs_kernel<CT, RT, NG, TH, 3>, dim3(grid), dim3(TH), lds, st, a, rows_per_block, n_rowblocks);
 }
 
 bool mxs_supported(uint32_t CT, uint32_t NG, uint32_t n_slices, uint32_t s1_fp6) {
diff --git a/kmersgwas_amd/csrc/score_narrow.hip b/kmersgwas_amd/csrc/score_narrow.hip
--- a/kmersgwas_amd/csrc/score_narrow.hip
+++ b/kmersgwas_amd/csrc/score_narrow.hip
@@ -374,25 +374,40 @@
 }
 
 constexpr uint32_t BM_WORDS = 1024;
-
-__global__ void __launch_bounds__(256) bitmap_count_kernel(const unsigned long long* bm, uint64_t words_per_col, uint32_t n_words,
-                                                           uint32_t n_blocks, uint32_t* blk_cnt, unsigned long long* blk_mask) {
-    __shared__ uint32_t part[4];
-    const uint32_t p = blockIdx.y, b = blockIdx.x;
+constexpr uint32_t BM_COUNT_SUB = 8;
+
+__global__ void __launch_bounds__(256) bitmap_count_kernel(const unsigned long long* bm, const unsigned char* marks, uint64_t words_per_col,
+                                                           uint64_t marks_per_col, uint32_t n_words, uint32_t n_blocks, uint32_t* blk_cnt) {
+    __shared__ uint32_t part[BM_COUNT_SUB][4];
+    const uint32_t p = blockIdx.y, b0 = blockIdx.x * BM_COUNT_SUB;
     const unsigned long long* w = bm + (uint64_t)p * words_per_col;
-    uint32_t c = 0;
-#pragma unroll
-    for (int i = 0; i < 4; i++) {
-        const uint32_t x = b * BM_WORDS + threadIdx.x * 4u + i;
-        if (x < n_words) c += __popcll(w[x]);
-    }
-    const unsigned long long m = __ballot(c != 0u);
-    if ((threadIdx.x & 63u) == 0u) blk_mask[((uint64_t)p * n_blocks + b) * 4u + (threadIdx.x >> 6)] = m;
-#pragma unroll
-    for (int d = 1; d < 64; d <<= 1) c += __shfl_xor(c, d);
-    if ((threadIdx.x & 63u) == 0u) part[threadIdx.x >> 6] = c;
-    __syncthreads();
-    if (threadIdx.x == 0) blk_cnt[p * n_blocks + b] = part[0] + part[1] + part[2] + part[3];
+    const unsigned char* m = marks + (uint64_t)p * marks_per_col;
+    uint32_t mk[BM_COUNT_SUB], c[BM_COUNT_SUB];
+#pragma unroll
+    for (uint32_t j = 0; j < BM_COUNT_SUB; j++) {
+        const uint32_t g = (b0 + j) * 256u + threadIdx.x;
+        mk[j] = g < marks_per_col ? (uint32_t)m[g] : 0u;
+    }
+#pragma unroll
+    for (uint32_t j = 0; j < BM_COUNT_SUB; j++) {
+        c[j] = 0;
+        if (mk[j]) {
+#pragma unroll
+            for (uint32_t i = 0; i < 4; i++) {
+                const uint32_t x = ((b0 + j) * 256u + threadIdx.x) * 4u + i;
+                if (x < n_words) c[j] += __popcll(w[x]);
+            }
+        }
+    }
+#pragma unroll
+    for (uint32_t j = 0; j < BM_COUNT_SUB; j++) {
+#pragma unroll
+        for (int d = 1; d < 64; d <<= 1) c[j] += __shfl_xor(c[j], d);
+        if ((threadIdx.x & 63u) == 0u) part[j][threadIdx.x >> 6] = c[j];
+    }
+    __syncthreads();
+    if (threadIdx.x < BM_COUNT_SUB && b0 + threadIdx.x < n_blocks)
+        blk_cnt[p * n_blocks + b0 + threadIdx.x] = part[threadIdx.x][0] + part[threadIdx.x][1] + part[threadIdx.x][2] + part[threadIdx.x][3];
 }
 
 __global__ void __launch_bounds__(256) bitmap_scan_kernel(uint32_t* blk_cnt, uint32_t n_blocks, uint32_t* col_total) {
@@ -472,54 +487,59 @@
     __syncthreads();
 }
 
-__global__ void __launch_bounds__(256) bitmap_scatter_kernel(unsigned long long* bm, uint64_t words_per_col, uint32_t n_words,
-                                                             uint32_t n_blocks, const uint32_t* blk_off, const uint32_t* col_total,
-                                                             const unsigned long long* blk_mask, uint32_t n_pheno, uint32_t* surv_off,
+__global__ void __launch_bounds__(256) bitmap_scatter_kernel(unsigned long long* bm, unsigned char* marks, uint64_t words_per_col,
+                                                             uint64_t marks_per_col, uint32_t n_words, uint32_t n_blocks, const uint32_t* blk_off,
+                                                             const uint32_t* col_total, uint32_t n_pheno, uint32_t* surv_off,
                                                              uint32_t* surv_cnt, uint32_t* key_count, uint32_t* tile_pref, uint32_t* keys,
                                                              uint32_t key_cap, uint32_t row_bits, bool nibble_transposed) {
     __shared__ uint32_t part[4];
     __shared__ uint32_t basep[4];
     const uint32_t p = blockIdx.y, b = blockIdx.x;
-    if (p == 0u && b == 0u) bitmap_bases_block(col_total, n_pheno, key_cap, surv_off, surv_cnt, key_count, tile_pref);
+    const uint32_t lane = threadIdx.x & 63u, wave = threadIdx.x >> 6;
+    const uint32_t g = b * 256u + threadIdx.x;
+    unsigned char* m = marks + (uint64_t)p * marks_per_col + g;
+    const bool mine = g < marks_per_col && *m != 0;
     const uint32_t my_off = blk_off[p * n_blocks + b];
     const uint32_t next_off = b + 1u < n_blocks ? blk_off[p * n_blocks + b + 1u] : col_total[p];
-    if (next_off == my_off) return;
-    const uint32_t lane = threadIdx.x & 63u, wave = threadIdx.x >> 6;
-    uint32_t col_base;
-    {
-        uint32_t v = 0;
-        for (uint32_t q = threadIdx.x; q < p; q += 256u) v += col_total[q];
-#pragma unroll
-        for (int d = 1; d < 64; d <<= 1) v += __shfl_xor(v, d);
-        if (lane == 0u) basep[wave] = v;
-        __syncthreads();
-        col_base = basep[0] + basep[1] + basep[2] + basep[3];
-    }
-    const bool mine = (blk_mask[((uint64_t)p * n_blocks + b) * 4u + wave] >> lane) & 1ull;
+    uint32_t before = 0;
+    for (uint32_t q = threadIdx.x; q < p; q += 256u) before += col_total[q];
     unsigned long long* w = bm + (uint64_t)p * words_per_col;
     unsigned long long x[4] = {0ull, 0ull, 0ull, 0ull};
-    uint32_t c = 0;
     if (mine) {
+        *m = 0;
 #pragma unroll
         for (int i = 0; i < 4; i++) {
-            const uint32_t idx = b * BM_WORDS + threadIdx.x * 4u + i;
+            const uint32_t idx = g * 4u + i;
             if (idx < n_words) {
                 x[i] = w[idx];
                 if (x[i]) w[idx] = 0ull;
             }
-            c += __popcll(x[i]);
-        }
-        if (nibble_transposed) {
-#pragma unroll
-            for (int i = 0; i < 4; i++) {
-                if (!x[i]) continue;
-                unsigned long long y = 0;
-#pragma unroll
-                for (int kg = 0; kg < 4; kg++)
-#pragma unroll
-                    for (int rt = 0; rt < 4; rt++) y |= ((x[i] >> (4 * (4 * kg + rt))) & 0xFull) << (4 * (4 * rt + kg));
-                x[i] = y;
-            }
+        }
+    }
+    if (p == 0u && b == 0u) bitmap_bases_block(col_total, n_pheno, key_cap, surv_off, surv_cnt, key_count, tile_pref);
+    if (next_off == my_off) return;
+    uint32_t col_base;
+    {
+        uint32_t v = before;
+#pragma unroll
+        for (int d = 1; d < 64; d <<= 1) v += __shfl_xor(v, d);
+        if (lane == 0u) basep[wave] = v;
+        __syncthreads();
+        col_base = basep[0] + basep[1] + basep[2] + basep[3];
+    }
+    uint32_t c = 0;
+#pragma unroll
+    for (int i = 0; i < 4; i++) c += __popcll(x[i]);
+    if (nibble_transposed && c) {
+#pragma unroll
+        for (int i = 0; i < 4; i++) {
+            if (!x[i]) continue;
+            unsigned long long y = 0;
+#pragma unroll
+            for (int kg = 0; kg < 4; kg++)
+#pragma unroll
+                for (int rt = 0; rt < 4; rt++) y |= ((x[i] >> (4 * (4 * kg + rt))) & 0xFull) << (4 * (4 * rt + kg));
+            x[i] = y;
         }
     }
     uint32_t incl = c;
@@ -535,7 +555,7 @@
 #pragma unroll
     for (int i = 0; i < 4; i++) {
         unsigned long long v = x[i];
-        const uint32_t row0 = (b * BM_WORDS + threadIdx.x * 4u + i) * 64u;
+        const uint32_t row0 = (g * 4u + i) * 64u;
         while (v) {
             const uint32_t bit = __ffsll((long long)v) - 1u;
             v &= v - 1ull;
@@ -546,15 +566,18 @@
 }
 
 hipError_t launch_bitmap_keys(unsigned long long* bitmap, uint64_t words_per_col, uint64_t n_rows, uint32_t n_pheno, uint32_t* blk_scratch,
-                              unsigned long long* blk_mask, uint32_t* keys_sorted, uint32_t key_cap, uint32_t row_bits, uint32_t* surv_off,
+                              unsigned char* marks, uint32_t* keys_sorted, uint32_t key_cap, uint32_t row_bits, uint32_t* surv_off,
                               uint32_t* surv_cnt, uint32_t* key_count, uint32_t* tile_pref, bool nibble_transposed, hipStream_t st) {
+    if (!marks) return hipErrorInvalidValue;
     const uint32_t n_words = (uint32_t)((n_rows + 63) / 64);
     const uint32_t n_blocks = (n_words + BM_WORDS - 1) / BM_WORDS;
-    hipLaunchKernelGGL(bitmap_count_kernel, dim3(n_blocks, n_pheno), dim3(256), 0, st, bitmap, words_per_col, n_words, n_blocks, blk_scratch, blk_mask);
+    const uint64_t marks_per_col = bitmap_marks_per_col(words_per_col);
+    launch_mid(bitmap_count_kernel, dim3((n_blocks + BM_COUNT_SUB - 1) / BM_COUNT_SUB, n_pheno), dim3(256), 0, st, bitmap, marks, words_per_col,
+               marks_per_col, n_words, n_blocks, blk_scratch);
     uint32_t* col_total = blk_scratch + (size_t)n_pheno * n_blocks;
-    hipLaunchKernelGGL(bitmap_scan_kernel, dim3(n_pheno), dim3(256), 0, st, blk_scratch, n_blocks, col_total);
-    hipLaunchKernelGGL(bitmap_scatter_kernel, dim3(n_blocks, n_pheno), dim3(256), 0, st, bitmap, words_per_col, n_words, n_blocks, blk_scratch,
-                       col_total, blk_mask, n_pheno, surv_off, surv_cnt, key_count, tile_pref, keys_sorted, key_cap, row_bits, nibble_transposed);
+    launch_mid(bitmap_scan_kernel, dim3(n_pheno), dim3(256), 0, st, blk_scratch, n_blocks, col_total);
+    launch_mid(bitmap_scatter_kernel, dim3(n_blocks, n_pheno), dim3(256), 0, st, bitmap, marks, words_per_col, marks_per_col, n_words, n_blocks,
+               blk_scratch, col_total, n_pheno, surv_off, surv_cnt, key_count, tile_pref, keys_sorted, key_cap, row_bits, nibble_transposed);
     return hipGetLastError();
 }
 
@@ -679,9 +702,8 @@
         if (e != hipSuccess) return e;
     }
     if (last)
-        launch_last(narrow_staged_kernel<NP>, dim3(n_blocks), dim3(256), lds, st, a, rows_per_block, stage_bytes);
-    else
-        hipLaunchKernelGGL((narrow_staged_kernel<NP>), dim3(n_blocks), dim3(256), lds, st, a, rows_per_block, stage_bytes);
+        return launch_last(narrow_staged_kernel<NP>, dim3(n_blocks), dim3(256), lds, st, a, rows_per_block, stage_bytes);
+    launch_mid(narrow_staged_kernel<NP>, dim3(n_blocks), dim3(256), lds, st, a, rows_per_block, stage_bytes);
     return hipGetLastError();
 }
 
@@ -735,8 +757,7 @@
         hipError_t e = hipFuncSetAttribute((const void*)narrow_kernel, hipFuncAttributeMaxDynamicSharedMemorySize, (int)lds);
         if (e != hipSuccess) return e;
     }
-    launch_last(narrow_kernel, dim3(n_blocks2), dim3(256), lds, st, a2, rows_per_block);
-    return hipGetLastError();
-}
-
-}
+    return launch_last(narrow_kernel, dim3(n_blocks2), dim3(256), lds, st, a2, rows_per_block);
+}
+
+}
```

Result: no change. 529.2 billion (-0.2%).
